# HJakeCunningham/ASVGP

Measured on AMD Instinct MI355X. Metric: Mpoints/s per ELBO+grad step, N=10M 1D Matern-3/2 M=2048, higher is better.
Workload: dtype f64

## Files before the change

### asvgp_amd/_lib.py

```python
import ctypes
import os

import torch

HERE = os.path.dirname(os.path.abspath(__file__))
LIB_PATH = os.path.join(HERE, "libasvgp_hip.so")

_c = ctypes
_P, _I, _L, _D, _Z = _c.c_void_p, _c.c_int, _c.c_int64, _c.c_double, _c.c_size_t

SIGNATURES = {
    "asvgp_version": (_I, []),
    "asvgp_last_error_string": (_c.c_char_p, []),
    "asvgp_status_name": (_c.c_char_p, [_I]),
    "asvgp_phi_workspace_bytes": (_Z, [_L, _I, _L]),
    "asvgp_create": (_I, [_c.POINTER(_P)]),
    "asvgp_destroy": (_I, [_P]),
    "asvgp_phi_accumulate_1d": (_I, [_P, _P, _P, _L, _L, _P, _L, _D, _I, _L, _P, _P, _Z, _P]),
    "asvgp_phi_weighted_workspace_bytes": (_Z, [_L, _I, _L]),
    "asvgp_phi_accumulate_1d_weighted": (_I, [_P, _P, _P, _P, _L, _L, _P, _L, _D, _I, _L, _P, _P, _P, _Z, _P]),
    "asvgp_set_weight_sums": (_I, [_P, _D, _D, _D]),
    "asvgp_phi_accumulate_kron2d_weighted": (_I, [_P, _P, _P, _L, _P, _L, _D, _L, _P, _L, _D, _L, _I, _P, _P, _P]),
    "asvgp_phi_accumulate_kron2d_sorted_weighted": (_I, [_P, _P, _P, _L, _P, _P, _L, _D, _L, _P, _L, _D, _L, _I, _P, _P, _P]),
    "asvgp_set_phi_algorithm": (_I, [_P, _I]),
    "asvgp_phi_last_algorithm": (_I, [_P]),
    "asvgp_set_phi_input_order": (_I, [_P, _I]),
    "asvgp_phi_last_input_order": (_I, [_P]),
    "asvgp_stream_probe": (_I, [_P, _P, _L, _P, _P]),
    "asvgp_debug_reload_env": (_I, []),
    "asvgp_set_deferred_forward_pass": (_I, [_P, _I]),
    "asvgp_prior_publish": (_I, [_P]),
    "asvgp_host_mantissa_bits": (_I, []),
    "asvgp_prior_interior_kuu_host": (_I, [_P, _I, _L, _I, _P, _P, _c.POINTER(_L), _c.POINTER(_L), _P]),
    "asvgp_result_mirror": (_I, [_P, _I, _c.POINTER(_P)]),
    "asvgp_result_mirror_read": (_I, [_P, _c.c_uint64, _P, _D]),
    "asvgp_elbo_grad_ahead_1d": (_I, [_P, _P, _P, _I, _L, _L, _I, _L, _P, _P, _P, _Z, _P]),
    "asvgp_elbo_publish_theta": (_I, [_P, _D, _D, _D]),
    "asvgp_elbo_grad_host_1d": (_I, [_P, _P, _P, _I, _D, _D, _D, _L, _L, _I, _L, _P, _P, _P, _Z, _P, _P, _D]),
    "asvgp_result_mirror_pending": (_c.c_uint64, [_P]),
    "asvgp_set_phi_workgroups": (_I, [_P, _I]),
    "asvgp_set_phi_deferred_reduce": (_I, [_P, _I]),
    "asvgp_phi_reduce_1d": (_I, [_P, _P]),
    "asvgp_phi_launch_plan_host": (_I, [_I, _I, _I, _I, _L, _L, _L, _I, _L, _D, _I, _I, _D, _D, _I, _P]),
    "asvgp_phi_index_1d": (_I, [_P, _L, _P, _L, _D, _P, _P]),
    "asvgp_phi_evaluate_1d": (_I, [_P, _L, _P, _L, _D, _I, _I, _P, _P, _P]),
    "asvgp_matern_coeffs": (_I, [_I, _D, _D, _c.POINTER(_D), _c.POINTER(_D), _c.POINTER(_I)]),
    "asvgp_kuu_assemble": (_I, [_P, _I, _c.POINTER(_D), _c.POINTER(_D), _L, _I, _P, _P, _P]),
    "asvgp_cholesky_band": (_I, [_P, _P, _L, _I, _P, _P]),
    "asvgp_inverse_from_cholesky_band": (_I, [_P, _P, _L, _I, _P]),
    "asvgp_solve_triang_mat": (_I, [_P, _P, _P, _L, _I, _L, _I, _P]),
    "asvgp_product_band_band": (_I, [_P, _P, _P, _L, _I, _I, _I, _I, _I, _I, _P]),
    "asvgp_transpose_band": (_I, [_P, _P, _L, _I, _I, _P]),
    "asvgp_symmetrise_band": (_I, [_P, _P, _L, _I, _P]),
    "asvgp_unpack_banded_matrix_to_dense": (_I, [_P, _P, _L, _I, _I, _P]),
    "asvgp_pack_dense_matrix_to_banded": (_I, [_P, _P, _L, _I, _I, _P]),
    "asvgp_band_trace_sym": (_I, [_P, _P, _L, _I, _P, _P]),
    "asvgp_cholesky_band_vjp": (_I, [_P, _P, _P, _P, _L, _I, _P]),
    "asvgp_inverse_from_cholesky_band_vjp": (_I, [_P, _P, _P, _P, _P, _L, _I, _P]),
    "asvgp_band_outer_product": (_I, [_P, _P, _L, _L, _I, _D, _P, _P]),
    "asvgp_band_launch_plan_host": (_I, [_I, _L, _I, _I, _I, _P]),
    "asvgp_elbo_workspace_bytes": (_Z, [_L, _I, _L]),
    "asvgp_set_band_algorithm": (_I, [_P, _I]),
    "asvgp_prior_plan_1d": (_I, [_P, _P, _I, _L, _I, _c.POINTER(_I)]),
    "asvgp_prior_table_doubles": (_Z, [_P, _I, _L, _I]),
    "asvgp_prior_forward_host": (_I, [_P, _I, _L, _I, _P, _P, _P, _Z, _P]),
    "asvgp_set_prior_forward": (_I, [_P, _I]),
    "asvgp_prior_forward_device": (_I, [_P, _P, _P, _P, _Z, _P]),
    "asvgp_prior_forward_stamps": (_I, [_P, _P, _P, _P, _P]),
    "asvgp_prior_plan_image_host": (_I, [_P, _I, _L, _I, _P, _P, _P, _P]),
    "asvgp_elbo_launch_plan_host": (_I, [_I, _I, _I, _I, _L, _I, _L, _I, _I, _I, _I, _I, _I, _I, _I, _I, _P]),
    "asvgp_elbo_grad_1d": (_I, [_P, _P, _P, _I, _D, _D, _D, _L, _L, _I, _L, _P, _P, _P, _Z, _P]),
    "asvgp_kuu_inverse_band_1d": (_I, [_P, _P, _I, _D, _D, _L, _I, _P, _P, _P, _P, _P, _P, _P, _Z, _P]),
    "asvgp_elbo_chain_sync": (_I, [_P, _I]),
    "asvgp_elbo_prior_chain_1d": (_I, [_P, _P, _I, _D, _D, _D, _L, _I, _L, _P, _P, _Z, _P]),
    "asvgp_elbo_data_chain_1d": (_I, [_P, _P, _P, _I, _D, _D, _D, _L, _L, _I, _L, _P, _P, _P, _Z, _P]),
    "asvgp_posterior_prepare_1d": (_I, [_P, _P, _P, _I, _D, _D, _D, _L, _I, _L, _P, _P, _P, _P, _Z, _P]),
    "asvgp_posterior_prepare_loo_1d": (_I, [_P, _P, _P, _I, _D, _D, _D, _L, _I, _L, _P, _P, _P, _P, _P, _Z, _P]),
    "asvgp_loo_workspace_bytes": (_Z, [_L, _I, _L]),
    "asvgp_loo_1d": (_I, [_P, _P, _P, _P, _L, _L, _P, _L, _D, _I, _L, _P, _P, _P, _D, _D, _P, _P, _P, _P, _P, _Z, _P]),
    "asvgp_score_workspace_bytes": (_Z, [_L, _I, _L]),
    "asvgp_score_1d": (_I, [_P, _P, _P, _P, _L, _L, _P, _L, _D, _I, _L, _P, _P, _D, _D, _P, _P, _P, _P, _P, _Z, _P]),
    "asvgp_weight_grad_workspace_bytes": (_Z, [_L, _I, _L, _L]),
    "asvgp_weight_grad_1d": (_I, [_P, _P, _P, _P, _L, _L, _P, _L, _D, _I, _L, _P, _P, _P, _D, _D, _P, _L, _P, _P, _P, _Z, _P]),
    "asvgp_predict_1d": (_I, [_P, _L, _P, _L, _D, _I, _L, _P, _P, _D, _L, _P, _P, _P]),
    "asvgp_predict_1d_h": (_I, [_P, _P, _L, _P, _L, _D, _I, _L, _P, _P, _D, _L, _P, _P, _P]),
    "asvgp_posterior_cov_workspace_bytes": (_Z, [_L, _I, _L]),
    "asvgp_posterior_cov_prepare_1d": (_I, [_P, _P, _P, _I, _D, _D, _D, _L, _I, _L, _P, _P, _P, _P, _P, _Z, _P]),
    "asvgp_predict_cov_1d": (_I, [_P, _P, _L, _P, _L, _P, _L, _D, _I, _L, _P, _I, _D, _D, _P, _L, _P]),
    "asvgp_predict_deriv_1d": (_I, [_P, _P, _L, _P, _L, _D, _I, _L, _P, _P, _I, _D, _D, _L, _P, _P, _P]),
    "asvgp_predict_cov_deriv_1d": (_I, [_P, _P, _L, _P, _L, _P, _L, _D, _I, _L, _P, _I, _D, _D, _I, _I, _P, _L, _P]),
    "asvgp_predict_grad_kron2d": (_I, [_P, _L, _P, _L, _D, _L, _P, _L, _D, _L, _I, _P, _P, _P, _P, _P, _L, _I, _L, _L, _L, _L,
                                       _I, _D, _D, _I, _D, _D, _P, _P, _P]),
    "asvgp_kron_dense_inverse": (_I, [_P, _P, _P, _L, _L, _I, _L, _L, _L, _L, _P, _P]),
    "asvgp_predict_cov_kron2d": (_I, [_P, _P, _L, _P, _L, _P, _L, _D, _L, _P, _L, _D, _L, _I, _P, _P, _P, _I, _D, _D, _I, _D, _D, _P, _L, _P]),
    "asvgp_predict_cov_additive": (_I, [_P, _P, _L, _P, _L, _I, _P, _c.POINTER(_L), _c.POINTER(_D), _c.POINTER(_L), _I,
                                         _c.POINTER(_I), _c.POINTER(_D), _c.POINTER(_D), _P, _P, _L, _P]),
    "asvgp_predict_components_additive": (_I, [_P, _P, _L, _I, _P, _c.POINTER(_L), _c.POINTER(_D), _c.POINTER(_L), _I, _c.POINTER(_I),
                                                _c.POINTER(_D), _c.POINTER(_D), _I, _P, _P, _P, _P, _P]),
    "asvgp_profile_enable": (_I, [_P, _I]),
    "asvgp_profile_read": (_I, [_P, _c.POINTER(_D), _c.POINTER(_L)]),
    "asvgp_kron_stats_doubles": (_Z, [_L, _L, _I]),
    "asvgp_phi_accumulate_kron2d": (_I, [_P, _P, _L, _P, _L, _D, _L, _P, _L, _D, _L, _I, _P, _P]),
    "asvgp_kron_evaluate_2d": (_I, [_P, _L, _P, _L, _D, _P, _L, _D, _L, _I, _P, _P, _P]),
    "asvgp_kron_assemble": (_I, [_P, _P, _P, _P, _P, _I, _L, _L, _D, _P, _P, _P]),
    "asvgp_blockband_cholesky": (_I, [_P, _L, _L, _P, _P, _P, _P]),
    "asvgp_blockband_backsolve": (_I, [_P, _L, _L, _P, _P]),
    "asvgp_predict_kron2d": (_I, [_P, _L, _P, _L, _D, _L, _P, _L, _D, _L, _I, _P, _P, _P, _P, _P, _P]),
    "asvgp_kron_cell_index": (_I, [_P, _L, _P, _L, _D, _P, _L, _D, _P, _P]),
    "asvgp_phi_accumulate_kron2d_sorted": (_I, [_P, _P, _L, _P, _P, _L, _D, _L, _P, _L, _D, _L, _I, _P, _P]),
    "asvgp_phi_accumulate_kron2d_sorted_f32": (_I, [_P, _P, _L, _P, _P, _L, _D, _L, _P, _L, _D, _L, _I, _P, _P]),
    "asvgp_kron_phi_launch_plan_host": (_I, [_I, _I, _I, _L, _L, _L, _L, _L, _I, _I, _L, _I, _P]),
    "asvgp_blockband_to_blocks": (_I, [_P, _L, _L, _L, _P, _P, _P]),
    "asvgp_kron_grad_terms": (_I, [_P, _P, _L, _P, _P, _P, _P, _P, _P, _P, _P, _P, _P, _I, _L, _L, _P, _P]),
    "asvgp_predict_kron2d_var": (_I, [_P, _L, _P, _L, _D, _P, _L, _D, _L, _I, _P, _P, _L, _P, _P]),
    "asvgp_kron_assemble_twisted": (_I, [_P, _P, _P, _P, _P, _I, _L, _L, _D, _L, _L, _L, _L, _L, _P, _P, _P, _P]),
    "asvgp_kron_grad_terms_twisted": (_I, [_P, _P, _L, _L, _L, _L, _L, _P, _P, _P, _P, _P, _P, _P, _P, _P, _P, _I, _L, _L, _P, _P]),
    "asvgp_predict_kron2d_var_twisted": (_I, [_P, _L, _P, _L, _D, _P, _L, _D, _L, _L, _I, _P, _P, _L, _L, _L, _L, _L, _P, _P]),
    "asvgp_phi_cross_workspace_bytes": (_Z, [_L, _L]),
    "asvgp_phi_cross_2d": (_I, [_P, _P, _L, _P, _L, _D, _L, _P, _L, _D, _L, _I, _P, _P, _Z, _P]),
}


class AsvgpError(RuntimeError):
    pass


_lib = None


def get_lib():
    global _lib
    if _lib is not None:
        return _lib
    if not os.path.exists(LIB_PATH):
        raise AsvgpError("HIP extension %s is missing: run `python -m asvgp_amd.build` (hipcc, gfx950). "
                         "asvgp_amd has no CPU fallback." % LIB_PATH)
    lib = ctypes.CDLL(LIB_PATH)
    for name, (res, args) in SIGNATURES.items():
        fn = getattr(lib, name, None)
        if fn is None:
            raise AsvgpError("libasvgp_hip.so does not export %s" % name)
        fn.restype = res
        fn.argtypes = args
    _lib = lib
    return lib


def check(status, what=""):
    if status != 0:
        lib = get_lib()
        raise AsvgpError("%s failed: %s (%s)" % (what or "asvgp call", lib.asvgp_status_name(status).decode(),
                                                  lib.asvgp_last_error_string().decode()))


class Handle:
    _defaults = {"band": 0, "phi": 0, "prior_forward": 0, "phi_order": 0}
    _live = None

    def __init__(self):
        import weakref
        lib = get_lib()
        h = _P()
        check(lib.asvgp_create(ctypes.byref(h)), "asvgp_create")
        self.ptr = h
        self._lib = lib
        self.band_algorithm = 0
        if Handle._live is None:
            Handle._live = weakref.WeakSet()
        Handle._live.add(self)
        if Handle._defaults["band"]:
            self.set_band_algorithm(Handle._defaults["band"])
        if Handle._defaults["phi"]:
            self.set_phi_algorithm(Handle._defaults["phi"])
        if Handle._defaults["prior_forward"]:
            self.set_prior_forward(Handle._defaults["prior_forward"])
        if Handle._defaults["phi_order"]:
            self.set_phi_input_order(Handle._defaults["phi_order"])

    def set_prior_forward(self, mode):
        check(self._lib.asvgp_set_prior_forward(self.ptr, int(mode)), "set_prior_forward")

    def prior_forward_device(self, coef, dcoef, n_doubles):
        import numpy as np
        coef = np.ascontiguousarray(coef, dtype=np.float64)
        dcoef = np.ascontiguousarray(dcoef, dtype=np.float64)
        tab = np.zeros(int(n_doubles), dtype=np.float64)
        check(self._lib.asvgp_prior_forward_device(self.ptr, coef.ctypes.data, dcoef.ctypes.data, tab.ctypes.data, tab.size, stream_ptr()),
              "prior_forward_device")
        return tab

    def set_band_algorithm(self, algo):
        check(self._lib.asvgp_set_band_algorithm(self.ptr, int(algo)), "set_band_algorithm")
        self.band_algorithm = int(algo)

    def set_phi_algorithm(self, algo):
        check(self._lib.asvgp_set_phi_algorithm(self.ptr, int(algo)), "set_phi_algorithm")

    def set_weight_sums(self, n_pos, sum_w, sum_log_w):
        if n_pos is None:
            n_pos, sum_w, sum_log_w = -1.0, 0.0, 0.0
        check(self._lib.asvgp_set_weight_sums(self.ptr, float(n_pos), float(sum_w), float(sum_log_w)), "set_weight_sums")

    def phi_last_algorithm(self):
        return int(self._lib.asvgp_phi_last_algorithm(self.ptr))

    def set_phi_input_order(self, order):
        check(self._lib.asvgp_set_phi_input_order(self.ptr, int(order)), "set_phi_input_order")

    def phi_last_input_order(self):
        return int(self._lib.asvgp_phi_last_input_order(self.ptr))

    def result_mirror(self, enable=True):
        import numpy as np
        ptr = _P()
        check(self._lib.asvgp_result_mirror(self.ptr, int(bool(enable)), ctypes.byref(ptr)), "result_mirror")
        if not enable or not ptr.value:
            self._mirror = None
            return None
        self._mirror = np.ctypeslib.as_array(ctypes.cast(ptr, ctypes.POINTER(_D)), shape=(16,))
        return self._mirror

    def set_deferred_forward_pass(self, on):
        check(self._lib.asvgp_set_deferred_forward_pass(self.ptr, int(on)), "set_deferred_forward_pass")
# ... 84 lines not shown
```

### asvgp_amd/csrc/bcr_mfma.hpp

```cpp
#pragma once
#include "bcr.hpp"
#include "prior_plan.hpp"

namespace asvgp {

constexpr int BM_THREADS = 1024;
constexpr int BM_B = 4;
constexpr int BM_GAT = 0, BM_GBT = 16, BM_DINV = 32, BM_SD = 48, BM_CAT = 64, BM_CBT = 80, BM_W = 96, BM_DG = 100, BM_REC = 104;

__host__ __device__ inline size_t bcr_mfma_ws_doubles(long nb) { return (size_t)nb * BM_REC + 64; }
__host__ __device__ inline size_t bcr_mfma_lds_doubles(long nb) {
  return (size_t)((nb + 1) / 2 + 1) * 32 + (size_t)nb * 4 + 96 + (size_t)(BM_THREADS / 64) * 4 * 40 + (size_t)(nb / 8 + 2) * 52;
}

__device__ __forceinline__ double bm_mfma(double a, double b, double c) { return __builtin_amdgcn_mfma_f64_4x4x4f64(a, b, c, 0, 0, 0); }

__device__ __forceinline__ double bm_chol_linv(const double (&d)[10], int hi, int lo, double& dprod, int& badj) {
  double l00, i0, l10, l20, l30, l11, i1, l21, l31, l22, i2, l32, l33, i3;
  Num<double>::sqrt_inv(d[0], l00, i0);
  badj = !(d[0] > 0.0) ? 1 : 0;
  l10 = d[1] * i0; l20 = d[3] * i0; l30 = d[6] * i0;
  double s = fma(-l10, l10, d[2]);
  badj = (!(s > 0.0) && !badj) ? 2 : badj;
  Num<double>::sqrt_inv(s, l11, i1);
  l21 = fma(-l20, l10, d[4]) * i1;
  l31 = fma(-l30, l10, d[7]) * i1;
  s = fma(-l21, l21, fma(-l20, l20, d[5]));
  badj = (!(s > 0.0) && !badj) ? 3 : badj;
  Num<double>::sqrt_inv(s, l22, i2);
  l32 = fma(-l31, l21, fma(-l30, l20, d[8])) * i2;
  s = fma(-l32, l32, fma(-l31, l31, fma(-l30, l30, d[9])));
  badj = (!(s > 0.0) && !badj) ? 4 : badj;
  Num<double>::sqrt_inv(s, l33, i3);
  dprod = (l00 * l11) * (l22 * l33);
  const double z0 = (lo == 0) ? i0 : 0.0;
  const double z1 = fma(-l10, z0, (lo == 1) ? 1.0 : 0.0) * i1;
  const double z2 = fma(-l21, z1, fma(-l20, z0, (lo == 2) ? 1.0 : 0.0)) * i2;
  const double z3 = fma(-l32, z2, fma(-l31, z1, fma(-l30, z0, (lo == 3) ? 1.0 : 0.0))) * i3;
  return hi == 0 ? z0 : (hi == 1 ? z1 : (hi == 2 ? z2 : z3));
}

template <typename Src> __device__ __forceinline__ auto bm_src_load(const Src& A, int dd, long col, long M, int) -> decltype(A.load_dc(dd, col, M)) {
  return A.load_dc(dd, col, M);
}
template <typename Src> __device__ __forceinline__ double bm_src_load(const Src& A, int dd, long col, long M, long) {
  return A.load((long)dd * M + col, true);
}
struct BmLog {
  double m; int e;
  __device__ __forceinline__ void mul(double p) {
    m *= p;
    const int hi = __double2hiint(m);
    e += ((hi >> 20) & 0x7ff) - 1023;
    m = __hiloint2double((hi & 0x800fffff) | 0x3ff00000, __double2loint(m));
  }
};

__device__ __forceinline__ unsigned long long bm_wave_xor(unsigned long long x) {
#pragma unroll
  for (int off = 32; off > 0; off >>= 1) x ^= (unsigned long long)__shfl_xor((long long)x, off, 64);
  return x;
}
__device__ __forceinline__ void bm_msg_send(double* box, int n, double v, unsigned long long tag, int lane) {
  unsigned long long* b = reinterpret_cast<unsigned long long*>(box);
  const unsigned long long w = lane < n ? (unsigned long long)__double_as_longlong(v) : 0ull;
  const unsigned long long x = bm_wave_xor(w) ^ tag;
  if (lane < n) __hip_atomic_store(b + lane, w, __ATOMIC_RELAXED, __HIP_MEMORY_SCOPE_AGENT);
  if (lane == n) __hip_atomic_store(b + n, x, __ATOMIC_RELAXED, __HIP_MEMORY_SCOPE_AGENT);
}
__device__ __forceinline__ bool bm_msg_recv(const double* box, int n, double& v, unsigned long long tag, int lane, long spin_limit) {
  const unsigned long long* b = reinterpret_cast<const unsigned long long*>(box);
  for (long spins = 0; spins <= spin_limit; ++spins) {
    const unsigned long long w = lane <= n ? __hip_atomic_load(b + lane, __ATOMIC_RELAXED, __HIP_MEMORY_SCOPE_AGENT) : 0ull;
    const unsigned long long x = bm_wave_xor(lane < n ? w : 0ull) ^ tag;
    const unsigned long long chk = (unsigned long long)__shfl((long long)w, n, 64);
    if (x == chk) { v = __longlong_as_double((long long)w); return true; }
    __builtin_amdgcn_s_sleep(1);
  }
  return false;
}

struct BmSplit {
  int half = -1;
  double* xchg = nullptr;
  long spin_limit = 0;
  int* gave_up = nullptr;
  unsigned long long tag = 0;
};
constexpr int BM_XCHG = 96;

template <typename Src>
__device__ __attribute__((always_inline)) void bcr_mfma_solve(Src A, const double* rhs, int M, double* ws, double* lds, double* Sband, double* x,
                                                              double* logdet, int* info, int rhs_stride = 1, double* stamps = nullptr,
                                                              BmSplit sp = BmSplit{}) {
  constexpr int B = BM_B;
  const int tid = threadIdx.x;
  const int lane = tid & 63, wv = __builtin_amdgcn_readfirstlane(tid >> 6);
  const int r = lane >> 4, q = (lane >> 2) & 3, c = lane & 3;
  const int e = r * 4 + c, et = c * 4 + r;
  const int hi = r > c ? r : c, lo = r > c ? c : r;
  const int nb = (M + B - 1) / B;
  const int nslot = (nb + 1) / 2;
  double* Dl = lds;
  double* El = lds + (size_t)(nslot + 1) * 16;
  double* xs = El + (size_t)(nslot + 1) * 16;
  double* red = xs + (size_t)nb * B;
  double* slab = red + 96 + (size_t)(wv * 4 + q) * 40;
  double* Fl = red + 96 + (size_t)(BM_THREADS / 64) * 4 * 40;
  double* Sl = lds;
  int levels = 0;
  while ((1 << levels) < nb) ++levels;
  const bool split = sp.half >= 0;
  const int top = levels - 1, ht = 1 << (top > 0 ? top : 0);
  double s_other = 0.0;
  int bad_other = 0x7fffffff;
  auto level_share = [&](int l, int ne, int& m0, int& ne_h) {
    m0 = 0; ne_h = ne;
    if (!split) return;
    if (l < top) {
      const int mL = ht >> (l + 1);
      if (sp.half == 0) ne_h = ne < mL ? ne : mL;
      else { m0 = mL; ne_h = ne > mL ? ne - mL : 0; }
    } else {
      ne_h = sp.half == 0 ? ne : 0;
    }
  };
  int bad = 0;
  BmLog ld{1.0, 0};
  unsigned long long t_prev = stamps ? __builtin_amdgcn_s_memtime() : 0ull;
  int nst = 0;
  auto stamp = [&]() {
    if (stamps && tid == 0) { const unsigned long long t = __builtin_amdgcn_s_memtime(); stamps[nst++] = (double)(t - t_prev); t_prev = t; }
  };
  auto rec = [&](int node) -> double* { return ws + (size_t)node * BM_REC; };
  auto bandD = [&](int n, int rr, int cc) -> double {
    const int col = n * B + cc, row = n * B + rr;
    const bool pad = row >= M;
    const double v = bm_src_load(A, rr - cc, pad ? 0 : col, (long)M, 0);
    return pad ? ((rr == cc) ? 1.0 : 0.0) : v;
  };
  auto bandE = [&](int n, int rr, int cc) -> double {
    if (rr > cc) return 0.0;
    const int col = n * B + cc, row = (n + 1) * B + rr;
    const bool pad = row >= M;
    const double v = bm_src_load(A, B + rr - cc, pad ? 0 : col, (long)M, 0);
    return pad ? 0.0 : v;
  };
  if ((nb & 1) && tid < 16 && !(split && sp.half == 0)) {
    const int rr = tid >> 2, cc = tid & 3;
    Dl[(size_t)((nb - 1) >> 1) * 16 + tid] = bandD(nb - 1, rr > cc ? rr : cc, rr > cc ? cc : rr);
  }
  if (split && sp.half == 0 && tid < 16) Dl[(size_t)(ht >> 1) * 16 + tid] = 0.0;
  for (int row = tid; row < nb * B; row += BM_THREADS) {
    const bool sep_left = split && sp.half == 0 && row >= ht * B && row < (ht + 1) * B;
    xs[row] = (row < M && !sep_left) ? rhs[(long)row * rhs_stride] : 0.0;
  }
  __syncthreads();
  stamp();

  constexpr int RMAXR = 4;
  for (int l = 0; l < levels; ++l) {
    const int h = 1 << l;
    const int ne = (nb > h) ? (nb - h + 2 * h - 1) / (2 * h) : 0;
    int m0, ne_h;
    level_share(l, ne, m0, ne_h);
    if (split && l == top) {
      if (sp.half == 1) {
        if (wv == 0) {
          const double v = lane < 16 ? Dl[(size_t)(ht >> 1) * 16 + lane] : (lane < 20 ? xs[ht * B + lane - 16] : 0.0);
          bm_msg_send(sp.xchg, 20, v, sp.tag | 1ull, lane);
        }
        const double mine = (r == 0 && c == 0) ? (log(ld.m) + (double)ld.e * 0.6931471805599453094) : 0.0;
        const double tot = wave_sum_dpp(mine);
        int bm = bad ? bad : 0x7fffffff;
#pragma unroll
        for (int off = 32; off > 0; off >>= 1) { const int o = __shfl_xor(bm, off, 64); bm = o < bm ? o : bm; }
        int* sbad = reinterpret_cast<int*>(red + 32);
        if (lane == 0) { red[wv] = tot; sbad[wv] = bm; }
        __syncthreads();
        if (wv == 0) {
          double sv = 0.0;
          int bmin = 0x7fffffff;
          for (int w2 = 0; w2 < BM_THREADS / 64; ++w2) { sv += red[w2]; bmin = sbad[w2] < bmin ? sbad[w2] : bmin; }
          bm_msg_send(sp.xchg + 24, 2, lane == 0 ? sv : (double)bmin, sp.tag | 2ull, lane);
        }
      } else {
        if (wv == 0) {
          double v = 0.0;
          if (!bm_msg_recv(sp.xchg, 20, v, sp.tag | 1ull, lane, sp.spin_limit)) { if (lane == 0) *sp.gave_up = 1; }
          else {
            if (lane < 16) Dl[(size_t)(ht >> 1) * 16 + lane] += v;
            else if (lane < 20) xs[ht * B + lane - 16] += v;
          }
        }
        __syncthreads();
        if (*sp.gave_up) return;
      }
      stamp();
    }
    double updb[RMAXR], ybu[RMAXR];
    int qv = q, ev = e;
    asm volatile("" : "+v"(qv), "+v"(ev));
    double sl[2][3];
    auto slab_loads = [&](int rd0) __attribute__((always_inline)) {
#pragma unroll
      for (int u = 0; u < 2; ++u) {
#pragma unroll
        for (int t3 = 0; t3 < 3; ++t3) {
          sl[u][t3] = 0.0;
          int m = (rd0 + u) * 64 + wv * 4 + qv;
          m = m0 + (m < ne_h ? m : ne_h - 1);
          const int kk = ev + 16 * t3, dd = kk >> 3, col = m * 2 * B + (kk & 7);
          const bool in = kk < 40 && col + dd < M;
          const double v = bm_src_load(A, in ? dd : 0, in ? col : 0, (long)M, 0);
          sl[u][t3] = in ? v : ((dd == 0) ? 1.0 : 0.0);
        }
      }
    };
#pragma unroll
    for (int rd = 0; rd < RMAXR; ++rd) {
      __builtin_amdgcn_sched_barrier(0);
      if (l == 0 && (rd & 1) == 0) slab_loads(rd);
      updb[rd] = 0.0; ybu[rd] = 0.0;
      if (rd * 64 + wv * 4 >= ne_h) continue;
      const int ml = rd * 64 + wv * 4 + q;
      const bool act = ml < ne_h;
      const int i = h + (m0 + (act ? ml : ne_h - 1)) * 2 * h, a = i - h, b = i + h;
      const bool hasb = b < nb;
      const int bsafe = hasb ? b : a;
      double d[10];
      double ea, eb, da;
      if (l == 0) {
#pragma unroll
        for (int t3 = 0; t3 < 3; ++t3) if (e + 16 * t3 < 40) slab[e + 16 * t3] = sl[rd & 1][t3];
        int kk = 0;
#pragma unroll
        for (int rr = 0; rr < 4; ++rr)
#pragma unroll
          for (int cc = 0; cc <= rr; ++cc) d[kk++] = slab[(rr - cc) * 8 + 4 + cc];
        ea = slab[(4 + lo - hi) * 8 + hi];
        ea = (r <= c) ? ea : 0.0;
        eb = slab[(4 + lo - hi) * 8 + 4 + hi];
        eb = (hasb && c <= r) ? eb : 0.0;
        da = slab[(hi - lo) * 8 + lo];
      } else {
        const double* Di = Dl + (size_t)(i >> 1) * 16;
        int kk = 0;
#pragma unroll
        for (int rr = 0; rr < 4; ++rr)
#pragma unroll
          for (int cc = 0; cc <= rr; ++cc) d[kk++] = Di[rr * 4 + cc];
        ea = El[(size_t)(a >> 1) * 16 + e];
        eb = El[(size_t)(i >> 1) * 16 + et];
        eb = hasb ? eb : 0.0;
        da = Dl[(size_t)(a >> 1) * 16 + e];
      }
      double yv = xs[i * B + r], ya = xs[a * B + r];
      yv = (c == 0) ? yv : 0.0;
      ya = (c == 0) ? ya : 0.0;
      (void)bsafe;
      double dprod;
      int badj;
      const double t = bm_chol_linv(d, hi, lo, dprod, badj);
      if (act && badj && !bad) bad = i * B + badj;
      const double linv = (r >= c) ? t : 0.0;
      const double linvT = (c >= r) ? t : 0.0;
      if (act) ld.mul(dprod);
      const double ua = bm_mfma(linvT, ea, 0.0);
      const double ub = bm_mfma(linvT, eb, 0.0);
      const double zz = bm_mfma(linvT, yv, 0.0);
      const double nua = -ua, nub = -ub;
      const double da_new = bm_mfma(nua, ua, da);
      const double e_new = bm_mfma(nub, ua, 0.0);
      const double ya_new = bm_mfma(nua, zz, ya);
      updb[rd] = bm_mfma(ub, ub, 0.0);
      ybu[rd] = bm_mfma(ub, zz, 0.0);
      updb[rd] = act ? updb[rd] : 0.0;
      ybu[rd] = act ? ybu[rd] : 0.0;
      const double gat = bm_mfma(ua, linv, 0.0);
      const double gbt = bm_mfma(ub, linv, 0.0);
      const double dinv = bm_mfma(linv, linv, 0.0);
      const double w = bm_mfma(linv, zz, 0.0);
      if (act) {
        if (l >= 3) {
          double* R = Fl + (size_t)(i >> 3) * 52;
          R[e] = gat; R[16 + e] = gbt; R[32 + e] = dinv;
          if (c == 0) R[48 + r] = w;
        } else {
          double* R = rec(i);
          R[BM_GAT + e] = gat; R[BM_GBT + e] = gbt; R[BM_DINV + e] = dinv;
          if (c == 0) R[BM_W + r] = w;
        }
        Dl[(size_t)(a >> 1) * 16 + e] = da_new;
        El[(size_t)(a >> 1) * 16 + e] = e_new;
        if (c == 0) xs[a * B + r] = ya_new;
      }
    }
    bcr_lds_barrier();
#pragma unroll
    for (int rd = 0; rd < RMAXR; ++rd) {
      if (rd * 64 + wv * 4 >= ne_h) continue;
      const int ml = rd * 64 + wv * 4 + q;
      const int i = h + (m0 + ml) * 2 * h, b = i + h;
      if (ml < ne_h && b < nb) {
        Dl[(size_t)(b >> 1) * 16 + e] -= updb[rd];
        if (c == 0) xs[b * B + r] -= ybu[rd];
      }
    }
    bcr_lds_barrier();
    stamp();
  }
  if (wv == 0 && !(split && sp.half == 1)) {
    const bool act = q == 0;
    double d[10];
    int kk = 0;
#pragma unroll
    for (int rr = 0; rr < 4; ++rr)
#pragma unroll
      for (int cc = 0; cc <= rr; ++cc) { const double v = Dl[rr * 4 + cc]; d[kk++] = act ? v : ((rr == cc) ? 1.0 : 0.0); }
    const double yv = (act && c == 0) ? xs[r] : 0.0;
    double dprod;
    int badj;
    const double t = bm_chol_linv(d, hi, lo, dprod, badj);
    if (act && badj && !bad) bad = badj;
    const double linv = (r >= c) ? t : 0.0, linvT = (c >= r) ? t : 0.0;
    if (act) ld.mul(dprod);
    const double s00 = bm_mfma(linv, linv, 0.0);
    const double zz = bm_mfma(linvT, yv, 0.0);
    const double x0 = bm_mfma(linv, zz, 0.0);
    if (act) {
      rec(0)[BM_SD + e] = s00;
      Sl[e] = s00;
      if (r >= c && r < M) Sband[(long)(r - c) * M + c] = s00;
      if (c == 0) xs[r] = x0;
    }
  }
  __syncthreads();
  stamp();
  unsigned long long lw = 0ull;
  for (int l = levels - 1; l >= 0; --l) {
    const int h = 1 << l;
    const int ne = (nb > h) ? (nb - h + 2 * h - 1) / (2 * h) : 0;
    int m0, ne_h;
    level_share(l, ne, m0, ne_h);
    if (split && sp.half == 0 && wv == BM_THREADS / 64 - 1) {
      if (l == top - 1 && lane <= 2)
        lw = __hip_atomic_load(reinterpret_cast<const unsigned long long*>(sp.xchg + 24) + lane, __ATOMIC_RELAXED, __HIP_MEMORY_SCOPE_AGENT);
      if (l == 2) {
        const unsigned long long x = bm_wave_xor(lane < 2 ? lw : 0ull) ^ (sp.tag | 2ull);
        const unsigned long long chk = (unsigned long long)__shfl((long long)lw, 2, 64);
        double v = __longlong_as_double((long long)lw);
        bool ok = x == chk;
        if (!ok) ok = bm_msg_recv(sp.xchg + 24, 2, v, sp.tag | 2ull, lane, sp.spin_limit);
        if (!ok) { if (lane == 0) *sp.gave_up = 1; }
        else if (lane < 2) red[48 + lane] = v;
      }
    }
#pragma unroll
    for (int rd = 0; rd < RMAXR; ++rd) {
      __builtin_amdgcn_sched_barrier(0);
      if (rd * 64 + wv * 4 >= ne_h) continue;
      const int ml = rd * 64 + wv * 4 + q;
      const bool act = ml < ne_h;
      const int i = h + (m0 + (act ? ml : ne_h - 1)) * 2 * h, a = i - h, b = i + h;
      const bool hasb = b < nb;
      const int bs = hasb ? b : a;
      const bool e_is_a = ((a / (2 * h)) & 1) != 0;
      double gat, gbt, dinv, w, saa, sbb, sba, sab;
      if (l >= 3) {
        const double* R = Fl + (size_t)(i >> 3) * 52;
        gat = R[e]; gbt = R[16 + e]; dinv = R[32 + e]; w = R[48 + r];
      } else {
        const double* R = rec(i);
        gat = R[BM_GAT + e]; gbt = R[BM_GBT + e]; dinv = R[BM_DINV + e]; w = R[BM_W + r];
      }
      if (l >= 1) {
        const double* Ra = Sl + (size_t)(a >> 2) * 48;
        const double* Rb = Sl + (size_t)(bs >> 2) * 48;
        saa = Ra[e];
        sbb = Rb[e];
        sba = e_is_a ? Ra[32 + e] : Rb[16 + et];
        sab = e_is_a ? Ra[32 + et] : Rb[16 + e];
      } else {
        const double* Ra = rec(a);
        const double* Rb = rec(bs);
        saa = Ra[BM_SD + e];
        sbb = Rb[BM_SD + e];
        sba = e_is_a ? Ra[BM_CBT + e] : Rb[BM_CAT + et];
        sab = e_is_a ? Ra[BM_CBT + et] : Rb[BM_CAT + e];
      }
      sbb = hasb ? sbb : 0.0; sba = hasb ? sba : 0.0; sab = hasb ? sab : 0.0;
      double xa = xs[a * B + r], xb = xs[bs * B + r];
      xa = (c == 0) ? xa : 0.0;
      xb = (hasb && c == 0) ? xb : 0.0;
      w = (c == 0) ? w : 0.0;
      double ncat = bm_mfma(saa, gat, 0.0);
      ncat = bm_mfma(sba, gbt, ncat);
      double ncbt = bm_mfma(sab, gat, 0.0);
      ncbt = bm_mfma(sbb, gbt, ncbt);
      double sii = bm_mfma(ncat, gat, dinv);
      sii = bm_mfma(ncbt, gbt, sii);
      double gx = bm_mfma(gat, xa, 0.0);
      gx = bm_mfma(gbt, xb, gx);
      if (act) {
        if (c == 0) xs[i * B + r] = w - gx;
        if (l >= 2) {
          double* Rw = Sl + (size_t)(i >> 2) * 48;
          Rw[e] = sii; Rw[16 + e] = -ncat; Rw[32 + e] = -ncbt;
        }
        if (l > 0) {
          double* Rw = rec(i);
          Rw[BM_SD + e] = sii; Rw[BM_CAT + e] = -ncat; Rw[BM_CBT + e] = -ncbt;
        }
        if (r >= c && i * B + r < M) Sband[(long)(r - c) * M + i * B + c] = sii;
        if (l == 0) {
          if (c <= r && i * B + c < M) Sband[(long)(B + c - r) * M + a * B + r] = -ncat;
          if (hasb && r <= c && b * B + r < M) Sband[(long)(B + r - c) * M + i * B + c] = -ncbt;
        }
      }
    }
    if (l == 1) __syncthreads(); else bcr_lds_barrier();
    if (split && l == top) {
      double* Rs = Sl + (size_t)(ht >> 2) * 48;
      if (sp.half == 0) {
        if (wv == 0) bm_msg_send(sp.xchg + 32, 52, lane < 48 ? Rs[lane < 48 ? lane : 0] : (lane < 52 ? xs[ht * B + lane - 48] : 0.0), sp.tag | 3ull, lane);
      } else {
        if (wv == 0) {
          double v = 0.0;
          if (!bm_msg_recv(sp.xchg + 32, 52, v, sp.tag | 3ull, lane, sp.spin_limit)) { if (lane == 0) *sp.gave_up = 1; }
          else if (lane < 48) {
            Rs[lane] = v;
            rec(ht)[BM_SD + lane] = v;
            if (lane < 16) {
              const int rr = lane >> 2, cc = lane & 3;
              if (rr >= cc && ht * B + rr < M) Sband[(long)(rr - cc) * M + ht * B + cc] = v;
            }
          } else if (lane < 52) {
            xs[ht * B + lane - 48] = v;
          }
        }
        __syncthreads();
        if (*sp.gave_up) return;
      }
    }
    stamp();
  }
  if (!(split && sp.half == 0))
    for (int col = M - B + tid; col < M; col += BM_THREADS)
      if (col >= 0)
#pragma unroll
        for (int dd = 1; dd <= B; ++dd)
          if (col + dd >= M) Sband[(long)dd * M + col] = 0.0;
  {
    const int row0 = (split && sp.half == 1) ? (ht + 1) * B : 0, row1 = (split && sp.half == 0) ? (ht + 1) * B : M;
    for (int row = row0 + tid; row < row1 && row < M; row += BM_THREADS) x[(long)row * rhs_stride] = xs[row];
  }
  if (!(split && sp.half == 1)) {
    const double mine = (r == 0 && c == 0) ? (log(ld.m) + (double)ld.e * 0.6931471805599453094) : 0.0;
    const double tot = wave_sum_dpp(mine);
    int bm = bad ? bad : 0x7fffffff;
#pragma unroll
    for (int off = 32; off > 0; off >>= 1) { const int o = __shfl_xor(bm, off, 64); bm = o < bm ? o : bm; }
    int* sbad = reinterpret_cast<int*>(red + 32);
    if (lane == 0) { red[wv] = tot; sbad[wv] = bm; }
    __syncthreads();
    if (split && tid == 0) { s_other = red[48]; bad_other = (int)red[49]; }
    if (tid == 0) {
      double s = 0.0;
      int bmin = 0x7fffffff;
      for (int w2 = 0; w2 < BM_THREADS / 64; ++w2) { s += red[w2]; bmin = sbad[w2] < bmin ? sbad[w2] : bmin; }
      s += s_other;
      bmin = bad_other < bmin ? bad_other : bmin;
      __hip_atomic_store(logdet + 0, 2.0 * s, __ATOMIC_RELAXED, __HIP_MEMORY_SCOPE_AGENT);
      __hip_atomic_store(logdet + 1, 0.0, __ATOMIC_RELAXED, __HIP_MEMORY_SCOPE_AGENT);
      __hip_atomic_store(info, (bmin == 0x7fffffff) ? 0 : bmin, __ATOMIC_RELAXED, __HIP_MEMORY_SCOPE_AGENT);
    }
  }
  stamp();
}


__host__ __device__ inline size_t bcr_mfma_pre_ws_doubles(long nb) { return (size_t)nb * 96 + 64; }
__host__ __device__ inline size_t bcr_mfma_pre_lds_doubles(long nb, int n_rec) {
  return PRIOR_TAB_HEADER + (size_t)2 * n_rec * prior_rec_fields(BM_B) + (size_t)(nb / 4 + 2) * 96 + (size_t)(nb + 1) / 2 + 64;
}

struct BmDual { double v, d; };
__device__ __forceinline__ BmDual bm_dmfma(BmDual x, BmDual y, BmDual c) {
  BmDual r;
  r.v = bm_mfma(x.v, y.v, c.v);
  r.d = bm_mfma(x.d, y.v, c.d);
  r.d = bm_mfma(x.v, y.d, r.d);
  return r;
}

__device__ __attribute__((always_inline)) void bcr_mfma_backward_pre(const double* __restrict__ tab, int n_rec, const int* __restrict__ node_rec, int M,
                                                                      double* ws, double* lds, double* Sv, double* Sd, double* logdet, int* info,
                                                                      unsigned long long* done_flag, unsigned long long seq,
                                                                      const unsigned long long* ready_flag = nullptr, long spin_limit = 0, int* gave_up = nullptr) {
  constexpr int B = BM_B, W = prior_rec_fields(B);
  const int tid = threadIdx.x;
  if (ready_flag) {
    if (tid == 0) {
      long spins = 0;
      while (__hip_atomic_load(ready_flag, __ATOMIC_RELAXED, __HIP_MEMORY_SCOPE_SYSTEM) < seq) {
        __builtin_amdgcn_s_sleep(8);
        if (++spins > spin_limit) { *gave_up = 1; break; }
      }
    }
    __syncthreads();
    if (*gave_up) return;
    __builtin_amdgcn_fence(__ATOMIC_ACQUIRE, "");
  }
  const int lane = tid & 63, wv = __builtin_amdgcn_readfirstlane(tid >> 6);
  const int r = lane >> 4, q = (lane >> 2) & 3, c = lane & 3;
  const int e = r * 4 + c, et = c * 4 + r;
  const int nb = (M + B - 1) / B;
  const int n_tab = PRIOR_TAB_HEADER + 2 * n_rec * W;
  double* tl = lds;
  double* Sl = lds + n_tab;
  int* nrl = reinterpret_cast<int*>(Sl + (size_t)(nb / 4 + 2) * 96);
  {
    const double2* src = reinterpret_cast<const double2*>(tab);
    double2* dst = reinterpret_cast<double2*>(tl);
    for (int i2 = tid; i2 < n_tab / 2; i2 += BM_THREADS) dst[i2] = src[i2];
    for (int i2 = tid; i2 < nb; i2 += BM_THREADS) nrl[i2] = node_rec[i2];
  }
  __syncthreads();
  if (done_flag && tid == 0) __hip_atomic_store(done_flag, seq, __ATOMIC_RELAXED, __HIP_MEMORY_SCOPE_SYSTEM);
  const double* tv = tl + PRIOR_TAB_HEADER;
  const double* td = tv + (size_t)n_rec * W;
  int levels = 0;
  while ((1 << levels) < nb) ++levels;
  if (tid < 16) {
    const int r0 = nrl[0];
    const double xv = tv[(size_t)r0 * W + prior_f_UA(B) + tid], xd = td[(size_t)r0 * W + prior_f_UA(B) + tid];
    Sl[tid] = xv; Sl[48 + tid] = xd;
    ws[tid] = xv; ws[48 + tid] = xd;
    const int rr = tid >> 2, cc = tid & 3;
    if (rr >= cc && rr < M) { Sv[(long)(rr - cc) * M + cc] = xv; Sd[(long)(rr - cc) * M + cc] = xd; }
  }
  __syncthreads();
  constexpr int RMAXR = 4;
  for (int l = levels - 1; l >= 0; --l) {
    const int h = 1 << l;
    const int ne = (nb > h) ? (nb - h + 2 * h - 1) / (2 * h) : 0;
#pragma unroll
    for (int rd = 0; rd < RMAXR; ++rd) {
      __builtin_amdgcn_sched_barrier(0);
      if (rd * 64 + wv * 4 >= ne) continue;
      const int m = rd * 64 + wv * 4 + q;
      const bool act = m < ne;
      const int i = h + (act ? m : ne - 1) * 2 * h, a = i - h, b = i + h;
      const bool hasb = b < nb;
      const int bs = hasb ? b : a;
      const bool e_is_a = ((a / (2 * h)) & 1) != 0;
      const int ri = nrl[i];
      const double* fv = tv + (size_t)ri * W;
      const double* fd = td + (size_t)ri * W;
      const BmDual gat{fv[prior_f_GAT(B) + e], fd[prior_f_GAT(B) + e]};
      const BmDual gbt{fv[prior_f_GBT(B) + e], fd[prior_f_GBT(B) + e]};
      const BmDual dinv{fv[prior_f_DINV(B) + e], fd[prior_f_DINV(B) + e]};
      BmDual saa, sbb, sba, sab;
      if (l >= 1) {
        const double* Ra = Sl + (size_t)(a >> 2) * 96;
        const double* Rb = Sl + (size_t)(bs >> 2) * 96;
        saa = BmDual{Ra[e], Ra[48 + e]};
        sbb = BmDual{Rb[e], Rb[48 + e]};
        sba = e_is_a ? BmDual{Ra[32 + e], Ra[80 + e]} : BmDual{Rb[16 + et], Rb[64 + et]};
        sab = e_is_a ? BmDual{Ra[32 + et], Ra[80 + et]} : BmDual{Rb[16 + e], Rb[64 + e]};
      } else {
        const double* Ga = ws + (size_t)a * 96;
        const double* Gb = ws + (size_t)bs * 96;
        saa = BmDual{Ga[e], Ga[48 + e]};
        sbb = BmDual{Gb[e], Gb[48 + e]};
        sba = e_is_a ? BmDual{Ga[32 + e], Ga[80 + e]} : BmDual{Gb[16 + et], Gb[64 + et]};
        sab = e_is_a ? BmDual{Ga[32 + et], Ga[80 + et]} : BmDual{Gb[16 + e], Gb[64 + e]};
      }
      if (!hasb) { sbb = BmDual{0.0, 0.0}; sba = sbb; sab = sbb; }
      const BmDual zero{0.0, 0.0};
      BmDual ncat = bm_dmfma(saa, gat, zero);
      ncat = bm_dmfma(sba, gbt, ncat);
      BmDual ncbt = bm_dmfma(sab, gat, zero);
      ncbt = bm_dmfma(sbb, gbt, ncbt);
      BmDual sii = bm_dmfma(ncat, gat, dinv);
      sii = bm_dmfma(ncbt, gbt, sii);
      if (act) {
        if (l >= 2) {
          double* Rw = Sl + (size_t)(i >> 2) * 96;
          Rw[e] = sii.v; Rw[16 + e] = -ncat.v; Rw[32 + e] = -ncbt.v;
          Rw[48 + e] = sii.d; Rw[64 + e] = -ncat.d; Rw[80 + e] = -ncbt.d;
        }
        if (l > 0) {
          double* Rw = ws + (size_t)i * 96;
          Rw[e] = sii.v; Rw[16 + e] = -ncat.v; Rw[32 + e] = -ncbt.v;
          Rw[48 + e] = sii.d; Rw[64 + e] = -ncat.d; Rw[80 + e] = -ncbt.d;
        }
        if (r >= c && i * B + r < M) { const long o = (long)(r - c) * M + i * B + c; Sv[o] = sii.v; Sd[o] = sii.d; }
        if (l == 0) {
          if (c <= r && i * B + c < M) { const long o = (long)(B + c - r) * M + a * B + r; Sv[o] = -ncat.v; Sd[o] = -ncat.d; }
          if (hasb && r <= c && b * B + r < M) { const long o = (long)(B + r - c) * M + i * B + c; Sv[o] = -ncbt.v; Sd[o] = -ncbt.d; }
        }
      }
    }
    if (l == 1) __syncthreads(); else bcr_lds_barrier();
  }
  for (int col = M - B + tid; col < M; col += BM_THREADS)
    if (col >= 0)
#pragma unroll
      for (int dd = 1; dd <= B; ++dd)
        if (col + dd >= M) { Sv[(long)dd * M + col] = 0.0; Sd[(long)dd * M + col] = 0.0; }
  if (tid == 0) {
    __hip_atomic_store(logdet + 0, tl[0], __ATOMIC_RELAXED, __HIP_MEMORY_SCOPE_AGENT);
    __hip_atomic_store(logdet + 1, tl[1], __ATOMIC_RELAXED, __HIP_MEMORY_SCOPE_AGENT);
    __hip_atomic_store(info, (int)tl[2], __ATOMIC_RELAXED, __HIP_MEMORY_SCOPE_AGENT);
  }
}

}
```

### asvgp_amd/csrc/elbo.hip

```cpp
#include <stdio.h>
#include <stdlib.h>
#include <time.h>
#include <string.h>

#include <type_traits>

#include "bcr_pre.hpp"
#include "bcr_mfma.hpp"
#include "handle.hpp"

namespace asvgp {


struct Ws {
  double *Kuu, *dK, *P, *LK, *dLK, *LP, *SK, *dSK, *SP, *c, *alpha, *logdets, *fin, *bcrK, *bcrP;
};
static size_t bcr_ws_chain(int planes, int k, bool big) {
  long ns = 1024;
  while ((long)planes * 2 * k * k * ns * 8 + 2 * ns * k * 8 + 1024 > 150 * 1024) ns >>= 1;
  if (big) ns *= 2;
  return (size_t)planes * (7 * k * k + k) * 2 * ns + (big ? (size_t)planes * k * k * ns : 0);
}
static size_t bcr_ws_K(int k, long M) {
  size_t a = bcr_ws_chain(2, k, false), b = bcr_ws_chain(2, k, true), c = bcr_pre_ws_doubles(k, (M + k - 1) / k);
  a = a > b ? a : b;
  return (a > c ? a : c) + 64;
}
static size_t bcr_ws_P(int k) { size_t a = bcr_ws_chain(1, k, false), b = bcr_ws_chain(1, k, true); return (a > b ? a : b) + 64; }
static size_t bcr_ws_total(long M, int k) { return bcr_ws_K(k, M) + bcr_ws_P(k); }
static size_t ws_doubles(long M, int k, long D) {
  return (size_t)9 * (k + 1) * M + (size_t)2 * M * D + 64 + 32 + bcr_ws_total(M, k);
}
static Ws carve(void* ws, long M, int k, long D) {
  double* p = static_cast<double*>(ws);
  size_t E = (size_t)(k + 1) * M;
  Ws w;
  w.Kuu = p; p += E; w.dK = p; p += E; w.P = p; p += E; w.LK = p; p += E; w.dLK = p; p += E;
  w.LP = p; p += E; w.SK = p; p += E; w.dSK = p; p += E; w.SP = p; p += E;
  w.c = p; p += (size_t)M * D; w.alpha = p; p += (size_t)M * D;
  w.logdets = p; p += 64;
  w.fin = p; p += 32;
  w.bcrK = p; p += bcr_ws_K(k, M);
  w.bcrP = p;
  return w;
}

template <int K> struct ElboLauncher {
  static int run(Handle* h, const double* stats, const double* S, int kind, double v, double l, double s, long N, long M, long D,
                 double* out, int* info, void* ws, hipStream_t st, int part);
};
template <int K> struct KuuInvLauncher {
  static int run(Handle* h, const double* S, int kind, double v, double l, long M, double* Kuu, double* dK, double* SK, double* dSK,
                 double* logdet2, int* info, void* ws, hipStream_t st);
};
template <int K> struct PostLauncher {
  static int run(Handle* h, const double* stats, const double* S, int kind, double v, double l, double s, long M, long D,
                 double* alpha, double* W, int* info, void* ws, hipStream_t st, double* Pinv = nullptr);
};
static size_t cov_ws_doubles(long M, int k) { return (size_t)4 * (k + 1) * M + (size_t)2 * M + 8; }
template <int K> struct PostCovLauncher {
  static int run(Handle* h, const double* stats, const double* S, int kind, double v, double l, double s, long M, long D,
                 double* alpha, double* W, double* Wd, int* info, void* ws, hipStream_t st);
};

constexpr int FIN_LDS_DOUBLES = 16 * 14 + 2;
constexpr size_t LDS_BYTES = 160 * 1024;
enum ChainPath { PATH_SWEEPS = 0, PATH_BCR, PATH_BCR_PRIOR, PATH_BCR_DATA, PATH_PLANNED_BCR, PATH_PLANNED_MFMA };
enum ChainForward { FWD_NONE = 0, FWD_HOST_INLINE, FWD_HOST_BEFORE, FWD_DEFERRED, FWD_WORKER, FWD_GPU, FWD_AHEAD };
struct ChainPlanIn {
  int algo;
  bool have_plan; int n_rec;
  bool interior;
  long M, D;
  int part;
  bool fused_fin;
  bool ahead_req, gpu_fwd, fwd_worker, defer_forward;
  bool no_split, plan_first;
};
struct ChainPlan {
  int status; char msg[160];
  int path;
  int part;
  bool nothing;
  bool big;
  size_t lds_bytes;
  int grid, n_helpers, split;
  int fwd;
  bool scale_alpha, scale_c;
};

template <int K, bool TANGENT>
static ChainPlan plan_chains(const ChainPlanIn& in) {
  ChainPlan p{};
  auto refuse = [&p](int status, const char* fmt, size_t bytes = 0) { p.status = status; snprintf(p.msg, sizeof(p.msg), fmt, bytes); return p; };
  const int algo = in.algo;
  const long M = in.M, nb = (M + K - 1) / K;
  if ((algo == 3 || algo == 4) && !in.have_plan) return refuse(ASVGP_ERR_BAD_ARG, "band algorithms 3 and 4 need asvgp_prior_plan_1d for this (M, k, kernel)");
  const bool planned0 = in.have_plan && (algo == 0 || algo == 3 || algo == 4);
  const size_t ldsK = sizeof(double) * (TANGENT ? bcr_lds_doubles<Dual, K, 0>(nb) : bcr_lds_doubles<double, K, 0>(nb));
  const size_t ldsP = sizeof(double) * bcr_lds_doubles<double, K, 1>(nb);
  p.lds_bytes = planned0 ? ldsP : (ldsK > ldsP ? ldsK : ldsP);
  bool fits = p.lds_bytes <= LDS_BYTES - 256;
  constexpr bool HAS_BIG = (K <= 5);
  if (HAS_BIG && !fits) {
    const size_t bK = sizeof(double) * (TANGENT ? bcr_lds_doubles<Dual, K, 0, true>(nb) : bcr_lds_doubles<double, K, 0, true>(nb));
    const size_t bP = sizeof(double) * bcr_lds_doubles<double, K, 1, true>(nb);
    const size_t bb = planned0 ? bP : (bK > bP ? bK : bP);
    if (bb <= LDS_BYTES - 256) { p.big = true; fits = true; p.lds_bytes = bb; }
  }
  const bool use_bcr = (algo == 2 || algo == 3 || algo == 4 || (algo == 0 && fits));
  const bool planned = planned0 && use_bcr;
  p.part = in.part;
  if (in.part != 0 && (!use_bcr || planned)) {
    if (in.part == 1) { p.nothing = true; return p; }
    p.part = 0;
  }
  p.scale_alpha = !TANGENT;
  const char* ahead_only = "launch-ahead exists for the matrix-core launch only (k = 4, D = 1, M <= 2048, planned prior chain)";
  if (planned) {
    bool mfma = false;
    size_t lds_mfma = 0;
    if constexpr (K == BM_B) {
      const size_t lb = sizeof(double) * bcr_mfma_lds_doubles(nb), lk = sizeof(double) * bcr_mfma_pre_lds_doubles(nb, in.n_rec);
      mfma = (algo == 0 || algo == 4) && in.D == 1 && nb <= 512 && TANGENT && in.fused_fin && lb <= LDS_BYTES && lk <= LDS_BYTES && in.interior;
      lds_mfma = lb > lk ? lb : lk;
    }
    if (algo == 4 && !mfma)
      return refuse(ASVGP_ERR_UNSUPPORTED, "band algorithm 4 (matrix-core chains) needs k = 4, D = 1, M <= 2048, Toeplitz static bands and the ELBO + gradient entry point");
    if (in.ahead_req && !mfma) return refuse(ASVGP_ERR_UNSUPPORTED, ahead_only);
    if (!mfma) {
      if (!fits) return refuse(ASVGP_ERR_LDS_CAPACITY, "BCR needs %zu B of LDS", p.lds_bytes);
      p.path = PATH_PLANNED_BCR;
      const size_t lds_pre = sizeof(double) * bcr_pre_lds_doubles(K, in.n_rec);
      if (lds_pre > p.lds_bytes) p.lds_bytes = lds_pre;
      p.n_helpers = (int)((M + 255) / 256 < 6 ? (M + 255) / 256 : 6);
      p.grid = 2 + p.n_helpers;
      p.fwd = in.gpu_fwd ? FWD_GPU : FWD_HOST_BEFORE;
      return p;
    }
    if (in.ahead_req && (in.gpu_fwd || in.plan_first)) return refuse(ASVGP_ERR_UNSUPPORTED, "launch-ahead needs the host forward pass (asvgp_set_prior_forward(h, 0))");
    p.path = PATH_PLANNED_MFMA;
    p.big = false;
    p.lds_bytes = lds_mfma > sizeof(double) * FIN_LDS_DOUBLES ? lds_mfma : sizeof(double) * FIN_LDS_DOUBLES;
    p.split = (nb >= 128 && !in.no_split) ? 1 : 0;
    p.grid = 2 + p.split;
    p.fwd = in.ahead_req ? FWD_AHEAD : in.gpu_fwd ? FWD_GPU : in.plan_first ? FWD_HOST_BEFORE : in.fwd_worker ? FWD_WORKER
          : in.defer_forward ? FWD_DEFERRED : FWD_HOST_INLINE;
    return p;
  }
  if (in.ahead_req) return refuse(ASVGP_ERR_UNSUPPORTED, ahead_only);
  if (!use_bcr) {
    p.path = PATH_SWEEPS; p.big = false; p.lds_bytes = 0; p.grid = 2; p.scale_alpha = p.scale_c = true;
    return p;
  }
  if (!fits) return refuse(ASVGP_ERR_LDS_CAPACITY, "BCR forced but needs %zu B of LDS", p.lds_bytes);
  p.path = p.part == 1 ? PATH_BCR_PRIOR : (p.part == 2 ? PATH_BCR_DATA : PATH_BCR);
  p.grid = p.part == 0 ? 2 : 1;
  if (p.part == 1) p.scale_alpha = false;
  return p;
}

template <class F>
static int for_bandwidth(int k, F&& f) {
  switch (k) {
    case 1: return f(std::integral_constant<int, 1>{});
    case 2: return f(std::integral_constant<int, 2>{});
    case 3: return f(std::integral_constant<int, 3>{});
    case 4: return f(std::integral_constant<int, 4>{});
    case 5: return f(std::integral_constant<int, 5>{});
    case 6: return f(std::integral_constant<int, 6>{});
  }
  return ASVGP_ERR_UNSUPPORTED;
}

#ifdef ASVGP_ELBO_ONLY_K
struct KuuCoefs2 { double c[ASVGP_MAX_KUU_TERMS]; double dc[ASVGP_MAX_KUU_TERMS]; int n; };

constexpr int KI_DKB = 8;
struct KuuInterior { double k[8]; long lo, hi; double bnd[2 * PRIOR_BND_DIAGS * PRIOR_BND]; double dk[8]; double dkb[2 * 5 * KI_DKB]; int dk_tab; };
struct ThetaBox {
  unsigned long long seq;
  double s, alpha_scale, v, l, N, Nw, cw;
  double k[8], dk[8];
  double bnd[2 * PRIOR_BND_DIAGS * PRIOR_BND];
  double dkb[2 * 5 * KI_DKB];
  double dc[ASVGP_MAX_KUU_TERMS];
};
typedef const __attribute__((address_space(3))) double* lds_cdouble_ptr;
struct BandSumToep {
  const double* A; double inv_s;
  lds_cdouble_ptr kl;
  lds_cdouble_ptr bnd;
  long lo, hi;
  __device__ __forceinline__ double load_dc(int dd, long col, long M) const {
#pragma clang fp contract(off)
    const double t2 = A[(long)dd * M + col] * inv_s;
    const bool left = col < lo, right = col >= hi;
    const long bi = left ? (long)dd * PRIOR_BND + col : (right ? (long)(PRIOR_BND_DIAGS + dd) * PRIOR_BND + (col - hi) : 0);
    const double bv = bnd[bi];
    const double kv = kl[dd];
    return t2 + ((left || right) ? bv : kv);
  }
};

static __global__ void elbo_prepare_kernel(const double* __restrict__ S, KuuCoefs2 cf, long E, const double* __restrict__ A,
                                    double s, double* __restrict__ Kuu, double* __restrict__ dK,
                                    double* __restrict__ P) {
#pragma clang fp contract(off)
  long e = (long)blockIdx.x * blockDim.x + threadIdx.x;
  if (e >= E) return;
  double acc = cf.c[0] * S[e];
  double dacc = cf.dc[0] * S[e];
  for (int t = 1; t < cf.n; ++t) {
    double sv = S[(long)t * E + e];
    acc = acc + cf.c[t] * sv;
    dacc = dacc + cf.dc[t] * sv;
  }
  Kuu[e] = acc;
  if (dK) dK[e] = dacc;
  if (P) P[e] = A[e] / s + acc;
}

template <int K, bool TANGENT, bool RHS>
__global__ __launch_bounds__(64) void elbo_factor_kernel(const double* Kuu, const double* dK, const double* P,
                                                         double* LK, double* dLK, double* LP, const double* b,
                                                         double* c, int M, int* info) {
  if (blockIdx.x == 0) {
    if (TANGENT) cholesky_sweep<Dual, K, false>(BandPtr<Dual>{Kuu, dK}, BandOut<Dual>{LK, dLK}, M, nullptr, nullptr, info);
    else cholesky_sweep<double, K, false>(BandPtr<double>{Kuu, nullptr}, BandOut<double>{LK, nullptr}, M, nullptr, nullptr, info);
  } else {
    cholesky_sweep<double, K, RHS>(BandPtr<double>{P, nullptr}, BandOut<double>{LP, nullptr}, M, b, c, info + 1);
  }
}

template <int K, bool TANGENT, bool RHS>
__global__ __launch_bounds__(64) void elbo_inverse_kernel(const double* LK, const double* dLK, const double* LP,
                                                          double* SK, double* dSK, double* SP, const double* c,
                                                          double* alpha, int M) {
  if (blockIdx.x == 0) {
    if (TANGENT) takahashi_sweep<Dual, K, false>(BandPtr<Dual>{LK, dLK}, BandOut<Dual>{SK, dSK}, M, nullptr, nullptr);
    else takahashi_sweep<double, K, false>(BandPtr<double>{LK, nullptr}, BandOut<double>{SK, nullptr}, M, nullptr, nullptr);
  } else {
    takahashi_sweep<double, K, RHS>(BandPtr<double>{LP, nullptr}, BandOut<double>{SP, nullptr}, M, c, alpha);
  }
}

template <int K>
__global__ __launch_bounds__(64) void elbo_trsv_kernel(const double* L, int M, const double* B, double* X, long D,
                                                       int trans, double scale) {
  const long d = blockIdx.x;
  if (trans) trsv_sweep<K, true>(L, M, B + d, X + d, D);
  else trsv_sweep<K, false>(L, M, B + d, X + d, D);
  (void)scale;
}

template <int K, bool BIG>
__device__ __forceinline__ void more_columns(const double* b, double* x, int D, int M, double* wsP, double* lds, int lds_doubles) {
  if (D <= 1) return;
  __syncthreads();
  const int nb = (M + K - 1) / K;
  int chunk = lds_doubles / (nb * K);
  if (chunk < 1) chunk = 1;
  for (int d0 = 1; d0 < D; d0 += chunk) bcr_solve_more<K, BIG>(b, x, D, d0, (D - d0 < chunk) ? D - d0 : chunk, M, wsP, lds);
}

template <int K, bool TANGENT, bool BIG>
__global__ __launch_bounds__(BCR_THREADS) void elbo_bcr_kernel(const double* Kuu, const double* dK, const double* P,
                                                               const double* b, int M, double* wsK, double* wsP,
                                                               double* SK, double* dSK, double* SP, double* x,
                                                               double* logdets, int* info, int do_stamps,
                                                               int first_chain, int D, int lds_doubles) {
  extern __shared__ double lds[];
  double* st = do_stamps ? logdets + 8 : nullptr;
  for (int rep = (do_stamps == 2) ? 0 : 1; rep < 2; ++rep) {
    if (blockIdx.x + first_chain == 0) {
      if (TANGENT) bcr_solve<Dual, K, 0, BandPtr<Dual>, BIG>(BandPtr<Dual>{Kuu, dK}, nullptr, M, wsK, lds, BandOut<Dual>{SK, dSK}, nullptr, logdets, info, st);
      else bcr_solve<double, K, 0, BandPtr<double>, BIG>(BandPtr<double>{Kuu, nullptr}, nullptr, M, wsK, lds, BandOut<double>{SK, nullptr}, nullptr, logdets, info, st);
    } else {
      bcr_solve<double, K, 1, BandPtr<double>, BIG>(BandPtr<double>{P, nullptr}, b, M, wsP, lds, BandOut<double>{SP, nullptr}, x, logdets + 2, info + 1, st ? st + 24 : nullptr, D);
      more_columns<K, BIG>(b, x, D, M, wsP, lds, lds_doubles);
    }
    __syncthreads();
  }
}

template <int K, bool BIG>
__global__ __launch_bounds__(BCR_THREADS) void elbo_bcr_prior_kernel(const double* Kuu, const double* dK, int M, double* wsK,
                                                                     double* SK, double* dSK, double* logdets, int* info,
                                                                     int do_stamps) {
  extern __shared__ double lds[];
  double* st = do_stamps ? logdets + 8 : nullptr;
  bcr_solve<Dual, K, 0, BandPtr<Dual>, BIG>(BandPtr<Dual>{Kuu, dK}, nullptr, M, wsK, lds, BandOut<Dual>{SK, dSK}, nullptr, logdets, info, st);
}

template <int K, bool BIG>
__global__ __launch_bounds__(BCR_THREADS) void elbo_bcr_data_kernel(const double* Kuu, const double* A, const double* b, int M,
                                                                    double* wsP, double* SP, double* x, double* logdets,
                                                                    int* info, int do_stamps, double s, int D, int lds_doubles) {
  extern __shared__ double lds[];
  double* st = do_stamps ? logdets + 8 : nullptr;
  bcr_solve<double, K, 1, BandSumP, BIG>(BandSumP{A, Kuu, 1.0 / s}, b, M, wsP, lds, BandOut<double>{SP, nullptr}, x, logdets + 2, info + 1,
                                         st ? st + 24 : nullptr, D);
  more_columns<K, BIG>(b, x, D, M, wsP, lds, lds_doubles);
}

template <int KT>
__device__ __forceinline__ double quad_col(const double* S, long M, long j, const double* x, long D, long d) {
  double xj = x[j * D + d];
  double a = S[j] * xj * xj;
#pragma unroll
  for (int r = 1; r <= KT; ++r) {
    long jr = (j + r < M) ? j + r : M - 1;
    double sv = (j + r < M) ? S[(long)r * M + j] : 0.0;
    a = fma(2.0 * sv * xj, x[jr * D + d], a);
  }
  return a;
}

struct ElboScalars { double v, l, s, N, Nw, cw; };

template <int KT>
__device__ __forceinline__ void elbo_finalize_body(
    int bid, int nblk, double* part_lds, const double* __restrict__ stats, const double* __restrict__ Kuu, const double* __restrict__ dK,
    const double* __restrict__ LK, const double* __restrict__ LP, const double* __restrict__ SK,
    const double* __restrict__ dSK, const double* __restrict__ SP, const double* __restrict__ c,
    const double* __restrict__ alpha, const double* __restrict__ logdets, long M, long D, ElboScalars th,
    double alpha_scale, double* __restrict__ gacc, unsigned* __restrict__ ticket, unsigned* __restrict__ rearm, double* __restrict__ out) {
  constexpr int k = KT;
  const double* A = stats;
  const double* b = stats + (long)(k + 1) * M;
  const double yy = stats[(long)(k + 1) * M + M * D];
  enum { LOGK, LOGP, TRKA, DTRKA, SKDK, SPDK, SKK, SPK, SPA, CC, AKA, ADKA, AAA, BA, NACC };
  double acc[NACC];
#pragma unroll
  for (int i = 0; i < NACC; ++i) acc[i] = 0.0;
  const long chunk = (M + nblk - 1) / nblk;
  const long j_end = ((long)(bid + 1) * chunk < M) ? (long)(bid + 1) * chunk : M;
  for (long j = (long)bid * chunk + threadIdx.x; j < j_end; j += blockDim.x) {
    if (!logdets) {
      double lk = LK[j], lp = LP[j];
      acc[LOGK] += log(lk * lk);
      acc[LOGP] += log(lp * lp);
    }
#pragma unroll
    for (int r = 0; r <= k; ++r) {
      long o = (long)r * M + j;
      double w = (r == 0) ? 1.0 : 2.0;
      double sk = SK[o], sp = SP[o], a = A[o], kk = Kuu[o], dk = dK[o];
      acc[TRKA] = fma(w * sk, a, acc[TRKA]);
      acc[DTRKA] = fma(w * dSK[o], a, acc[DTRKA]);
      acc[SKDK] = fma(w * sk, dk, acc[SKDK]);
      acc[SPDK] = fma(w * sp, dk, acc[SPDK]);
      acc[SKK] = fma(w * sk, kk, acc[SKK]);
      acc[SPK] = fma(w * sp, kk, acc[SPK]);
      acc[SPA] = fma(w * sp, a, acc[SPA]);
    }
    for (long d = 0; d < D; ++d) {
      if (!logdets) {
        double cv = c[j * D + d];
        acc[CC] = fma(cv, cv, acc[CC]);
      }
      acc[AKA] += quad_col<KT>(Kuu, M, j, alpha, D, d);
      acc[ADKA] += quad_col<KT>(dK, M, j, alpha, D, d);
      acc[AAA] += quad_col<KT>(A, M, j, alpha, D, d);
      acc[BA] = fma(b[j * D + d], alpha[j * D + d], acc[BA]);
    }
  }
  double (*part)[NACC] = reinterpret_cast<double (*)[NACC]>(part_lds);
  const int lane = threadIdx.x & 63, wv = threadIdx.x >> 6, nw = blockDim.x >> 6;
#pragma unroll
  for (int i = 0; i < NACC; ++i) {
    double v = wave_sum_dpp(acc[i]);
    if (lane == 0) part[wv][i] = v;
  }
  __syncthreads();
  double tot[NACC];
  if (threadIdx.x < 64) {
#pragma unroll
    for (int i = 0; i < NACC; ++i) tot[i] = wave_sum_dpp(lane < nw ? part[lane][i] : 0.0);
  }
  int* is_last_p = reinterpret_cast<int*>(part_lds + 16 * NACC);
#define is_last (*is_last_p)
  if (threadIdx.x == 0) {
#pragma unroll
    for (int i = 0; i < NACC; ++i)
      if (tot[i] != 0.0) __hip_atomic_fetch_add(gacc + i, tot[i], __ATOMIC_RELAXED, __HIP_MEMORY_SCOPE_AGENT);
    asm volatile("s_waitcnt vmcnt(0)" ::: "memory");
    unsigned t = __hip_atomic_fetch_add(ticket, 1u, __ATOMIC_RELAXED, __HIP_MEMORY_SCOPE_AGENT);
    is_last = (t == (unsigned)nblk - 1);
  }
  __syncthreads();
  if (!is_last) return;
  if (threadIdx.x == 0) {
#pragma unroll
    for (int i = 0; i < NACC; ++i) tot[i] = __hip_atomic_load(gacc + i, __ATOMIC_RELAXED, __HIP_MEMORY_SCOPE_AGENT);
#pragma unroll
    for (int i = 0; i < NACC; ++i) __hip_atomic_store(gacc + i, 0.0, __ATOMIC_RELAXED, __HIP_MEMORY_SCOPE_AGENT);
    __hip_atomic_store(ticket, 0u, __ATOMIC_RELAXED, __HIP_MEMORY_SCOPE_AGENT);
    if (rearm) __hip_atomic_store(rearm, 0u, __ATOMIC_RELAXED, __HIP_MEMORY_SCOPE_AGENT);
    const double v = th.v, s = th.s, N = th.N, Nw = th.Nw, Dd = (double)D;
    tot[AKA] *= alpha_scale * alpha_scale; tot[ADKA] *= alpha_scale * alpha_scale; tot[AAA] *= alpha_scale * alpha_scale;
    tot[BA] *= alpha_scale;
    if (logdets) {
      tot[LOGK] = logdets[0];
      tot[LOGP] = logdets[2];
      tot[CC] = tot[BA] / s;
    }
    const double two_pi = 6.283185307179586476925286766559;
    double elbo = -0.5 * N * Dd * log(two_pi * s);
    elbo -= 0.5 * Dd * tot[LOGP];
    elbo += 0.5 * Dd * tot[LOGK];
    elbo -= 0.5 * yy / s;
    elbo += 0.5 * tot[CC];
    elbo -= 0.5 * Nw * v / s;
    elbo += 0.5 * tot[TRKA] / s;
    if (th.cw != 0.0) elbo += th.cw;
    double d_l = 0.5 * (Dd * tot[SKDK] - Dd * tot[SPDK] - tot[ADKA] + tot[DTRKA] / s);
    double d_v = 0.5 * (-Dd * tot[SKK] / v + Dd * tot[SPK] / v + tot[AKA] / v + tot[TRKA] / (v * s)) - 0.5 * Nw / s;
    double s2 = s * s;
    double d_s = -0.5 * N * Dd / s + 0.5 * Dd * tot[SPA] / s2 + 0.5 * yy / s2 + 0.5 * tot[AAA] / s2 - tot[BA] / s2 +
                 0.5 * Nw * v / s2 - 0.5 * tot[TRKA] / s2;
    out[0] = elbo; out[1] = d_v; out[2] = d_l; out[3] = d_s;
    out[4] = tot[LOGK]; out[5] = tot[LOGP]; out[6] = tot[TRKA]; out[7] = tot[CC];
  }
#undef is_last
}

template <int KT>
__global__ __launch_bounds__(256) void elbo_finalize_kernel(
    const double* __restrict__ stats, const double* __restrict__ Kuu, const double* __restrict__ dK,
    const double* __restrict__ LK, const double* __restrict__ LP, const double* __restrict__ SK,
    const double* __restrict__ dSK, const double* __restrict__ SP, const double* __restrict__ c,
    const double* __restrict__ alpha, const double* __restrict__ logdets, long M, int k_rt, long D, ElboScalars th,
    double alpha_scale, double* __restrict__ gacc, unsigned* __restrict__ ticket, double* __restrict__ out) {
  __shared__ double part[FIN_LDS_DOUBLES];
  (void)k_rt;
  elbo_finalize_body<KT>((int)blockIdx.x, (int)gridDim.x, part, stats, Kuu, dK, LK, LP, SK, dSK, SP, c, alpha, logdets, M, D, th, alpha_scale,
                         gacc, ticket, nullptr, out);
}

struct FusedFin {
  const double* stats; ElboScalars th; double alpha_scale; double* gacc; unsigned* ticket; unsigned* arrived; unsigned* assembled; double* out;
  long D; int n_helpers; int finalize; int debug_no_assembly; int debug_stamps;
  double* mirror; unsigned long long mirror_seq;
  int split; double* xchg;
};
constexpr int FIN_GACC_PR = 21;
__device__ __forceinline__ void assemble_band_slice(const double* __restrict__ S, const double* __restrict__ coef, const double* __restrict__ dcoef, int n_terms,
                                                    long E, long e, double* __restrict__ Kuu, double* __restrict__ dK) {
#pragma clang fp contract(off)
  double sv[ASVGP_MAX_KUU_TERMS];
#pragma unroll
  for (int t = 0; t < ASVGP_MAX_KUU_TERMS; ++t) sv[t] = (t < n_terms) ? S[(long)t * E + e] : 0.0;
  double acc = coef[0] * sv[0], dacc = dcoef[0] * sv[0];
#pragma unroll
  for (int t = 1; t < ASVGP_MAX_KUU_TERMS; ++t)
    if (t < n_terms) { acc = acc + coef[t] * sv[t]; dacc = dacc + dcoef[t] * sv[t]; }
  Kuu[e] = acc;
  if (dK) dK[e] = dacc;
}
template <int K, bool BIG>
__global__ __launch_bounds__(BCR_THREADS) void elbo_chains_kernel(const double* S_static, KuuCoefs2 cf, double* Kuu, double* dK, const double* A, const double* b, int M,
                                                                  double* wsP, double* SP, double* x, double* logdets, int* info,
                                                                  double s, const double* tab, int n_rec, const int* node_rec,
                                                                  double* wsK, double* SK, double* dSK,
                                                                  unsigned long long* done_flag, unsigned long long seq, int D, int lds_doubles, FusedFin fin) {
  extern __shared__ double lds[];
  const long E = (long)(K + 1) * M;
  __shared__ int gave_up;
  if (threadIdx.x == 0) gave_up = 0;
  __syncthreads();
  if (blockIdx.x == 0) {
    if (threadIdx.x == 0) {
      long spins = 0;
      while (__hip_atomic_load(fin.assembled, __ATOMIC_RELAXED, __HIP_MEMORY_SCOPE_AGENT) < (unsigned)fin.n_helpers) {
        __builtin_amdgcn_s_sleep(2);
        if (++spins > (1L << 25)) { gave_up = 1; break; }
      }
      if (!gave_up) __hip_atomic_store(fin.assembled, 0u, __ATOMIC_RELAXED, __HIP_MEMORY_SCOPE_AGENT);
    }
    __syncthreads();
    if (gave_up) { if (threadIdx.x == 0) atomicExch(info + 1, -1); return; }
    __builtin_amdgcn_fence(__ATOMIC_ACQUIRE, "agent");
    bcr_solve<double, K, 1, BandSumP, BIG>(BandSumP{A, Kuu, 1.0 / s}, b, M, wsP, lds, BandOut<double>{SP, nullptr}, x, logdets + 2, info + 1, nullptr, D);
    more_columns<K, BIG>(b, x, D, M, wsP, lds, lds_doubles);
  } else if (blockIdx.x == 1) {
    bcr_backward_pre<K>(tab, n_rec, node_rec, M, wsK, lds, BandOut<Dual>{SK, dSK}, logdets, info, done_flag, seq);
  } else {
    for (long e = (long)(blockIdx.x - 2) * blockDim.x + threadIdx.x; e < E; e += (long)fin.n_helpers * blockDim.x)
      assemble_band_slice(S_static, cf.c, cf.dc, cf.n, E, e, Kuu, dK);
    __syncthreads();
    if (threadIdx.x == 0) {
      __threadfence();
      __hip_atomic_fetch_add(fin.assembled, 1u, __ATOMIC_RELEASE, __HIP_MEMORY_SCOPE_AGENT);
    }
  }
  if (!fin.finalize) return;
  if (blockIdx.x < 2) {
    __syncthreads();
    if (threadIdx.x == 0) {
      __threadfence();
      __hip_atomic_fetch_add(fin.arrived, 1u, __ATOMIC_RELEASE, __HIP_MEMORY_SCOPE_AGENT);
    }
    return;
  }
  if (threadIdx.x == 0) {
    long spins = 0;
    while (__hip_atomic_load(fin.arrived, __ATOMIC_RELAXED, __HIP_MEMORY_SCOPE_AGENT) < 2u) {
      __builtin_amdgcn_s_sleep(8);
      if (++spins > (1L << 25)) { gave_up = 1; break; }
    }
  }
  __syncthreads();
  if (gave_up) { if (threadIdx.x == 0) atomicExch(info + 1, -1); return; }
  __builtin_amdgcn_fence(__ATOMIC_ACQUIRE, "agent");
  elbo_finalize_body<K>((int)blockIdx.x - 2, fin.n_helpers, lds, fin.stats, Kuu, dK, nullptr, nullptr, SK, dSK, SP, nullptr, x, logdets, (long)M, fin.D,
                        fin.th, fin.alpha_scale, fin.gacc, fin.ticket, fin.arrived, fin.out);
}

template <int K>
__global__ __launch_bounds__(BM_THREADS) void elbo_chains_mfma_kernel(KuuInterior ki, const double* S_static, KuuCoefs2 cf, double* Kuu, double* dK, const double* A, const double* b, int M,
                                                                      double* wsP, double* SP, double* x, double* logdets, int* info,
                                                                      double s, const double* tab, int n_rec, const int* node_rec,
                                                                      double* wsK, double* SK, double* dSK,
                                                                      unsigned long long* done_flag, unsigned long long seq,
                                                                      const unsigned long long* ready_flag, long spin_limit, FusedFin fin, const ThetaBox* box) {
  extern __shared__ double lds[];
  static_assert(K == BM_B, "matrix-core chains: bandwidth 4");
  const long E = (long)(K + 1) * M;
  const unsigned long long t_start = fin.debug_stamps ? __builtin_amdgcn_s_memrealtime() : 0ull;
  auto rstamp = [&](int slot) {
    if (fin.debug_stamps && threadIdx.x == 0 && blockIdx.x <= 2)
      logdets[(slot < 4 ? 8 + 4 * (int)blockIdx.x : 24) + slot] = (slot == 0) ? (double)(t_start & 0xffffffffull) : (double)((__builtin_amdgcn_s_memrealtime() - t_start) & 0xffffffffull);
  };
  rstamp(0);
  __shared__ int gave_up, kuu_ok;
  __shared__ double kuu_pref[4];
  if (threadIdx.x == 0) { gave_up = 0; kuu_ok = 0; }
  __syncthreads();
  double s_v = s, asc_v = fin.alpha_scale;
  ElboScalars th_v = fin.th;
  if (box) {
    if (threadIdx.x == 0) {
      long spins = 0;
      for (;;) {
        const unsigned long long got = __hip_atomic_load(&box->seq, __ATOMIC_RELAXED, __HIP_MEMORY_SCOPE_SYSTEM);
        if (got == seq) break;
        if (got == ~0ull || ++spins > spin_limit) { gave_up = 1; break; }
        __builtin_amdgcn_s_sleep(2);
      }
    }
    __syncthreads();
    if (gave_up) { if (threadIdx.x == 0) atomicExch(info + 1, -1); return; }
    s_v = box->s; asc_v = box->alpha_scale;
    th_v.v = box->v; th_v.l = box->l; th_v.s = box->s; th_v.N = box->N; th_v.Nw = box->Nw; th_v.cw = box->cw;
  }
  const double* stats = fin.stats;
  enum { LOGK, LOGP, TRKA, DTRKA, SKDK, SPDK, SKK, SPK, SPA, CC, AKA, ADKA, AAA, BA, NACC };
  double acc[NACC];
#pragma unroll
  for (int i = 0; i < NACC; ++i) acc[i] = 0.0;
  const bool isP = blockIdx.x == 0 || (fin.split && blockIdx.x == 2);
  const bool isPR = fin.split && blockIdx.x == 2;
  __shared__ double kdl[16];
  __shared__ double bnd[2 * PRIOR_BND_DIAGS * PRIOR_BND], dkb[2 * 5 * KI_DKB];
  {
    if (isP) rstamp(1);
    if (threadIdx.x == 0) {
      if (box) {
#pragma unroll
        for (int i = 0; i < 5; ++i) { kdl[i] = box->k[i]; kdl[8 + i] = box->dk[i]; }
      } else {
        kdl[0] = ki.k[0]; kdl[1] = ki.k[1]; kdl[2] = ki.k[2]; kdl[3] = ki.k[3]; kdl[4] = ki.k[4];
        kdl[8] = ki.dk[0]; kdl[9] = ki.dk[1]; kdl[10] = ki.dk[2]; kdl[11] = ki.dk[3]; kdl[12] = ki.dk[4];
      }
    }
    {
      const double* bnd_g = box ? box->bnd : reinterpret_cast<const double*>((const char*)__builtin_amdgcn_kernarg_segment_ptr() + offsetof(KuuInterior, bnd));
      const double* dkb_g = box ? box->dkb : reinterpret_cast<const double*>((const char*)__builtin_amdgcn_kernarg_segment_ptr() + offsetof(KuuInterior, dkb));
      if (threadIdx.x < 2 * PRIOR_BND_DIAGS * PRIOR_BND) bnd[threadIdx.x] = bnd_g[threadIdx.x];
      else if (threadIdx.x < 2 * PRIOR_BND_DIAGS * PRIOR_BND + 2 * 5 * KI_DKB) dkb[threadIdx.x - 2 * PRIOR_BND_DIAGS * PRIOR_BND] = dkb_g[threadIdx.x - 2 * PRIOR_BND_DIAGS * PRIOR_BND];
    }
    __syncthreads();
  }
  if (isP) {
    BmSplit bsp;
    if (fin.split) { bsp.half = isPR ? 1 : 0; bsp.xchg = fin.xchg; bsp.spin_limit = spin_limit; bsp.gave_up = &gave_up; bsp.tag = seq << 8; }
    bcr_mfma_solve<BandSumToep>(BandSumToep{A, 1.0 / s_v, (lds_cdouble_ptr)kdl, (lds_cdouble_ptr)bnd, ki.lo, ki.hi}, b, M, wsP, lds, SP, x, logdets + 2, info + 1, 1,
                                fin.debug_stamps ? (isPR ? fin.xchg + 128 : logdets + 32) : (double*)nullptr, bsp);
    rstamp(3);
    __syncthreads();
    if (gave_up) { if (threadIdx.x == 0) atomicExch(info + 1, -1); return; }
    rstamp(4);
    if (fin.finalize) {
      const double* xs_l = lds + (size_t)2 * ((((M + K - 1) / K) + 1) / 2 + 1) * 16;
      static_assert(BM_THREADS == 1024, "two columns per thread");
      int nbl = (M + K - 1) / K, lv = 0;
      while ((1 << lv) < nbl) ++lv;
      const long jsep = (long)(1 << (lv > 0 ? lv - 1 : 0)) * K;
      const long j0 = isPR ? jsep : 0, j1 = (fin.split && !isPR) ? jsep : (long)M;
      unsigned long long kw = 0ull;
      const bool kuu_reader = !isPR && (threadIdx.x >> 6) == 1;
      if (kuu_reader && (threadIdx.x & 63) <= 4)
        kw = __hip_atomic_load(reinterpret_cast<const unsigned long long*>(fin.gacc + 8) + (threadIdx.x & 63), __ATOMIC_RELAXED, __HIP_MEMORY_SCOPE_AGENT);
      double sp[2][K + 1], av[2][K + 1], bj[2];
#pragma unroll
      for (int cI = 0; cI < 2; ++cI) {
        const long j = j0 + threadIdx.x + cI * BM_THREADS, jc = j < j1 ? j : j1 - 1;
#pragma unroll
        for (int r = 0; r <= K; ++r) { sp[cI][r] = SP[(long)r * M + jc]; av[cI][r] = stats[(long)r * M + jc]; }
        bj[cI] = stats[(long)(K + 1) * M + jc];
      }
#pragma unroll
      for (int cI = 0; cI < 2; ++cI) {
        const long j = j0 + threadIdx.x + cI * BM_THREADS;
        if (j >= j1) continue;
        const bool left = j < ki.lo, right = j >= ki.hi;
        const double xj = xs_l[j];
#pragma unroll
        for (int r = 0; r <= K; ++r) {
          const long o = (long)r * M + j;
          const double w2 = (r == 0) ? 1.0 : 2.0;
          double kv = kdl[r], dkv = kdl[8 + r];
          if (left || right) {
            kv = bnd[left ? (long)r * PRIOR_BND + j : (long)(PRIOR_BND_DIAGS + r) * PRIOR_BND + (j - ki.hi)];
            if (ki.dk_tab) {
              dkv = dkb[left ? (long)r * KI_DKB + j : (long)(5 + r) * KI_DKB + (j - ki.hi)];
            } else {
              dkv = 0.0;
              for (int t = 0; t < cf.n; ++t) dkv = fma(box ? box->dc[t] : cf.dc[t], S_static[(long)t * E + o], dkv);
            }
          }
          const double xx = (j + r < M) ? w2 * xj * xs_l[j + r] : 0.0;
          acc[SPDK] = fma(w2 * sp[cI][r], dkv, acc[SPDK]);
          acc[SPK] = fma(w2 * sp[cI][r], kv, acc[SPK]);
          acc[SPA] = fma(w2 * sp[cI][r], av[cI][r], acc[SPA]);
          acc[AKA] = fma(kv, xx, acc[AKA]);
          acc[ADKA] = fma(dkv, xx, acc[ADKA]);
          acc[AAA] = fma(av[cI][r], xx, acc[AAA]);
        }
        acc[BA] = fma(bj[cI], xj, acc[BA]);
      }
      if (kuu_reader) {
        const int ln = threadIdx.x & 63;
        const unsigned long long x = bm_wave_xor(ln < 4 ? kw : 0ull) ^ ((seq << 8) | 4ull);
        const unsigned long long chk = (unsigned long long)__shfl((long long)kw, 4, 64);
        if (x == chk) { if (ln < 4) kuu_pref[ln] = __longlong_as_double((long long)kw); if (ln == 0) kuu_ok = 1; }
      }
    }
  } else {
    if (fin.debug_no_assembly) {
      if (threadIdx.x == 0) { for (long sp_ = 0; sp_ < spin_limit; ++sp_) __builtin_amdgcn_s_sleep(8); atomicExch(info + 1, -1); }
      return;
    }
    bcr_mfma_backward_pre(tab, n_rec, node_rec, M, wsK, lds, SK, dSK, logdets, info, done_flag, seq, ready_flag,
                          spin_limit < (1L << 20) ? spin_limit : (1L << 20), &gave_up);
    if (gave_up) { if (threadIdx.x == 0) atomicExch(info + 1, -1); return; }
    rstamp(1);
    if (fin.finalize) {
      __syncthreads();
      double sk[2][K + 1], dsk[2][K + 1], av[2][K + 1];
#pragma unroll
      for (int cI = 0; cI < 2; ++cI) {
        const long j = (long)threadIdx.x + cI * BM_THREADS, jc = j < M ? j : M - 1;
#pragma unroll
        for (int r = 0; r <= K; ++r) { sk[cI][r] = SK[(long)r * M + jc]; dsk[cI][r] = dSK[(long)r * M + jc]; av[cI][r] = stats[(long)r * M + jc]; }
      }
#pragma unroll
      for (int cI = 0; cI < 2; ++cI) {
        const long j = (long)threadIdx.x + cI * BM_THREADS;
        if (j >= M) continue;
        const bool left = j < ki.lo, right = j >= ki.hi;
#pragma unroll
        for (int r = 0; r <= K; ++r) {
          const long o = (long)r * M + j;
          const double w2 = (r == 0) ? 1.0 : 2.0;
          double kv = kdl[r], dkv = kdl[8 + r];
          if (left || right) {
            kv = bnd[left ? (long)r * PRIOR_BND + j : (long)(PRIOR_BND_DIAGS + r) * PRIOR_BND + (j - ki.hi)];
            if (ki.dk_tab) {
              dkv = dkb[left ? (long)r * KI_DKB + j : (long)(5 + r) * KI_DKB + (j - ki.hi)];
            } else {
              dkv = 0.0;
              for (int t = 0; t < cf.n; ++t) dkv = fma(box ? box->dc[t] : cf.dc[t], S_static[(long)t * E + o], dkv);
            }
          }
          acc[TRKA] = fma(w2 * sk[cI][r], av[cI][r], acc[TRKA]);
          acc[DTRKA] = fma(w2 * dsk[cI][r], av[cI][r], acc[DTRKA]);
          acc[SKDK] = fma(w2 * sk[cI][r], dkv, acc[SKDK]);
          acc[SKK] = fma(w2 * sk[cI][r], kv, acc[SKK]);
        }
      }
    }
  }
  if (!fin.finalize) { rstamp(2); return; }
  if (isP) rstamp(5);
  double* part0 = lds;
  const int lane = threadIdx.x & 63;
  double mine[8];
  mine[0] = isP ? acc[SPDK] : acc[TRKA];
  mine[1] = isP ? acc[SPK] : acc[DTRKA];
  mine[2] = isP ? acc[SPA] : acc[SKDK];
  mine[3] = isP ? acc[AKA] : acc[SKK];
  mine[4] = acc[ADKA]; mine[5] = acc[AAA]; mine[6] = acc[BA]; mine[7] = 0.0;
  const int nmine = isP ? 7 : 4;
  __syncthreads();
  const bool b0 = (lane & 1) != 0, b1 = (lane & 2) != 0, b2 = (lane & 4) != 0;
  double s4[4], s2[2];
#pragma unroll
  for (int i = 0; i < 4; ++i) { const double keep = b0 ? mine[4 + i] : mine[i], send = b0 ? mine[i] : mine[4 + i]; s4[i] = keep + dpp_move_f64<0xB1>(send); }
#pragma unroll
  for (int i = 0; i < 2; ++i) { const double keep = b1 ? s4[2 + i] : s4[i], send = b1 ? s4[i] : s4[2 + i]; s2[i] = keep + dpp_move_f64<0x4E>(send); }
  double s1 = (b2 ? s2[1] : s2[0]) + dpp_xor4_f64(b2 ? s2[0] : s2[1], b2);
  s1 += dpp_move_f64<0x128>(s1); s1 += __shfl_xor(s1, 16, 64); s1 += __shfl_xor(s1, 32, 64);
  const int wv = threadIdx.x >> 6;
  if (lane < 8) part0[wv * 8 + lane] = s1;
  __syncthreads();
  if (threadIdx.x >= 64) return;
  double t2 = part0[(2 * (lane >> 3)) * 8 + (lane & 7)] + part0[(2 * (lane >> 3) + 1) * 8 + (lane & 7)];
  t2 += __shfl_xor(t2, 8, 64); t2 += __shfl_xor(t2, 16, 64); t2 += __shfl_xor(t2, 32, 64);
  double red[7];
  red[0] = __shfl(t2, 0, 64); red[1] = __shfl(t2, 4, 64); red[2] = __shfl(t2, 2, 64); red[3] = __shfl(t2, 6, 64);
  red[4] = __shfl(t2, 1, 64); red[5] = __shfl(t2, 5, 64); red[6] = __shfl(t2, 3, 64);
  (void)nmine;
  double tot[NACC];
#pragma unroll
  for (int i = 0; i < NACC; ++i) tot[i] = 0.0;
  if (isP && threadIdx.x == 0) rstamp(6);
  const unsigned long long mtag = seq << 8;
  double* box_kuu = fin.gacc + 8;
  double* box_pr = fin.gacc + FIN_GACC_PR;
  if (!isP || isPR) {
    double v = red[0];
#pragma unroll
    for (int i = 1; i < 7; ++i) v = (lane == i) ? red[i] : v;
    bm_msg_send(isPR ? box_pr : box_kuu, nmine, v, mtag | (isPR ? 5ull : 4ull), lane);
    if (threadIdx.x == 0) rstamp(2);
    return;
  }
  double kuu_v = 0.0, pr_v = 0.0;
  {
    bool ok = true;
    if (kuu_ok) kuu_v = lane < 4 ? kuu_pref[lane] : 0.0;
    else ok = bm_msg_recv(box_kuu, 4, kuu_v, mtag | 4ull, lane, spin_limit);
    if (ok && fin.split) ok = bm_msg_recv(box_pr, 7, pr_v, mtag | 5ull, lane, spin_limit);
    if (!ok) { if (lane == 0) atomicExch(info + 1, -1); return; }
  }
  {
    const int pidx[7] = {SPDK, SPK, SPA, AKA, ADKA, AAA, BA};
#pragma unroll
    for (int i = 0; i < 7; ++i) tot[pidx[i]] = red[i] + (fin.split ? __shfl(pr_v, i, 64) : 0.0);
  }
  tot[TRKA] = __shfl(kuu_v, 0, 64); tot[DTRKA] = __shfl(kuu_v, 1, 64); tot[SKDK] = __shfl(kuu_v, 2, 64); tot[SKK] = __shfl(kuu_v, 3, 64);
  if (threadIdx.x != 0) return;
#pragma unroll
  for (int i = 0; i < 14; ++i) __hip_atomic_store(fin.gacc + i, 0.0, __ATOMIC_RELAXED, __HIP_MEMORY_SCOPE_AGENT);
  {
    const double v = th_v.v, sn = th_v.s, N = th_v.N, Nw = th_v.Nw;
    const double yy = stats[(long)(K + 1) * M + M];
    const double asc = asc_v;
    tot[AKA] *= asc * asc; tot[ADKA] *= asc * asc; tot[AAA] *= asc * asc; tot[BA] *= asc;
    tot[LOGK] = __hip_atomic_load(logdets + 0, __ATOMIC_RELAXED, __HIP_MEMORY_SCOPE_AGENT);
    tot[LOGP] = __hip_atomic_load(logdets + 2, __ATOMIC_RELAXED, __HIP_MEMORY_SCOPE_AGENT);
    tot[CC] = tot[BA] / sn;
    const double two_pi = 6.283185307179586476925286766559;
    double elbo = -0.5 * N * log(two_pi * sn);
    elbo -= 0.5 * tot[LOGP];
    elbo += 0.5 * tot[LOGK];
    elbo -= 0.5 * yy / sn;
    elbo += 0.5 * tot[CC];
    elbo -= 0.5 * Nw * v / sn;
    elbo += 0.5 * tot[TRKA] / sn;
    if (th_v.cw != 0.0) elbo += th_v.cw;
    const double d_l = 0.5 * (tot[SKDK] - tot[SPDK] - tot[ADKA] + tot[DTRKA] / sn);
    const double d_v = 0.5 * (-tot[SKK] / v + tot[SPK] / v + tot[AKA] / v + tot[TRKA] / (v * sn)) - 0.5 * Nw / sn;
    const double s2 = sn * sn;
    const double d_s = -0.5 * N / sn + 0.5 * tot[SPA] / s2 + 0.5 * yy / s2 + 0.5 * tot[AAA] / s2 - tot[BA] / s2 + 0.5 * Nw * v / s2 - 0.5 * tot[TRKA] / s2;
    double* out = fin.out;
    out[0] = elbo; out[1] = d_v; out[2] = d_l; out[3] = d_s;
    out[4] = tot[LOGK]; out[5] = tot[LOGP]; out[6] = tot[TRKA]; out[7] = tot[CC];
    if (fin.mirror) {
      double* m = fin.mirror;
      const double mv[10] = {elbo, d_v, d_l, d_s, tot[LOGK], tot[LOGP], tot[TRKA], tot[CC],
                             (double)__hip_atomic_load(info, __ATOMIC_RELAXED, __HIP_MEMORY_SCOPE_AGENT),
                             (double)__hip_atomic_load(info + 1, __ATOMIC_RELAXED, __HIP_MEMORY_SCOPE_AGENT)};
      double sum = (double)fin.mirror_seq;
#pragma unroll
      for (int i = 0; i < 10; ++i) { __hip_atomic_store(m + i, mv[i], __ATOMIC_RELAXED, __HIP_MEMORY_SCOPE_SYSTEM); sum += mv[i]; }
      __hip_atomic_store(m + 11, sum, __ATOMIC_RELAXED, __HIP_MEMORY_SCOPE_SYSTEM);
      __hip_atomic_store(m + 10, (double)fin.mirror_seq, __ATOMIC_RELAXED, __HIP_MEMORY_SCOPE_SYSTEM);
    }
  }
  rstamp(2);
}

static __global__ void scale_sub_kernel(const double* __restrict__ a, const double* __restrict__ b, double* __restrict__ o,
                                 long n) {
  long i = (long)blockIdx.x * blockDim.x + threadIdx.x;
  if (i < n) o[i] = a[i] - b[i];
}
static __global__ void scale_kernel(double* __restrict__ x, double f, long n) {
  long i = (long)blockIdx.x * blockDim.x + threadIdx.x;
  if (i < n) x[i] = x[i] * f;
}

static double now_us() { timespec ts; clock_gettime(CLOCK_MONOTONIC, &ts); return ts.tv_sec * 1e6 + ts.tv_nsec * 1e-3; }

struct ChainCall {
  Handle* h; const double *S, *A, *b; KuuCoefs2 cf; int kind; double s; long M, D; Ws w; int* info; hipStream_t st; const FusedFin* fin;
  double t_enter;
};
static void scale_after(const ChainCall& c, const ChainPlan& p) {
  const long n = c.M * c.D;
  if (p.scale_c) hipLaunchKernelGGL(scale_kernel, dim3((unsigned)((n + 255) / 256)), dim3(256), 0, c.st, c.w.c, 1.0 / c.s, n);
  if (p.scale_alpha) hipLaunchKernelGGL(scale_kernel, dim3((unsigned)((n + 255) / 256)), dim3(256), 0, c.st, c.w.alpha, 1.0 / c.s, n);
}
static void set_pending_forward(Handle* h, const KuuCoefs2& cf, const TableSlot& slot) {
  for (int t = 0; t < ASVGP_MAX_KUU_TERMS; ++t) { h->fwd.coef[t] = cf.c[t]; h->fwd.dcoef[t] = cf.dc[t]; }
  h->fwd.tab = slot.tab; h->fwd.slot = slot.slot; h->fwd.seq = slot.seq;
}
static FusedFin chain_fin(const ChainCall& c, const ChainPlan& p) {
  FusedFin ff{};
  if (c.fin) { ff = *c.fin; ff.finalize = 1; }
  ff.n_helpers = p.n_helpers;
  ff.split = p.split;
  ff.xchg = p.split ? c.w.LP : nullptr;
  ff.assembled = reinterpret_cast<unsigned*>(c.w.fin + 20);
  ff.debug_no_assembly = debug_env().no_assembly;
  ff.debug_stamps = debug_env().chain_stamps;
  return ff;
}
static void interior_dkuu(const PriorPlan* plan, const double* dc, double* dk, double* dkb) {
  double bnd2[2 * PRIOR_BND_DIAGS * PRIOR_BND];
  long lo2 = 0, hi2 = 0;
  prior_plan_interior_kuu(plan, dc, dk, &lo2, &hi2, bnd2);
  for (int sd = 0; sd < 2; ++sd)
    for (int d = 0; d <= BM_B; ++d)
      for (int cI = 0; cI < KI_DKB; ++cI)
        dkb[(sd * 5 + d) * KI_DKB + cI] = bnd2[(size_t)(sd * PRIOR_BND_DIAGS + d) * PRIOR_BND + cI];
}
static int grant_lds(const void* kern, size_t lds_bytes) {
  const hipError_t e = hipFuncSetAttribute(kern, hipFuncAttributeMaxDynamicSharedMemorySize, (int)lds_bytes);
  if (e == hipSuccess) return ASVGP_OK;
  set_error("hipFuncSetAttribute: %s", hipGetErrorString(e));
  return ASVGP_ERR_LDS_CAPACITY;
}

template <int K>
static int launch_planned_mfma(const ChainCall& c, const ChainPlan& p) {
  Handle* h = c.h;
  const Ws& w = c.w;
  const int n_rec = prior_plan_nrec(h->plan);
  const bool host_times = debug_env().host_times != 0;
  KuuInterior ki;
  prior_plan_interior_kuu(h->plan, c.cf.c, ki.k, &ki.lo, &ki.hi, ki.bnd);
  interior_dkuu(h->plan, c.cf.dc, ki.dk, ki.dkb);
  ki.dk_tab = (ki.lo <= KI_DKB && c.M - ki.hi <= KI_DKB) ? 1 : 0;
  const double t_acq0 = host_times ? now_us() : 0.0;
  TableSlot slot(h);
  const double t_acq1 = host_times ? now_us() : 0.0;
  const double* tab_k = h->tab_dev + (size_t)slot.slot * h->slot_doubles;
  const unsigned long long* ready = h->ready_dev + slot.slot;
  if (p.fwd == FWD_GPU) {
    double* t = nullptr;
    const int rc = handle_prior_dd_forward(h, c.cf.c, c.cf.dc, slot.slot, c.st, &t, nullptr, slot.seq, &ready);
    if (rc) return rc;
    tab_k = t;
  }
  FusedFin ff = chain_fin(c, p);
  const long spin_limit = debug_env().spin_limit;
  auto kern = elbo_chains_mfma_kernel<K>;
  static size_t lds_granted[16] = {0};
  size_t& granted = lds_granted[h->device & 15];
  if (p.lds_bytes > granted) {
    const int rc = grant_lds(reinterpret_cast<const void*>(kern), p.lds_bytes);
    if (rc) return rc;
    granted = p.lds_bytes;
  }
  const double t0 = host_times ? now_us() : 0.0;
  const ThetaBox* box_k = nullptr;
  if (p.fwd == FWD_HOST_BEFORE) {
    (void)prior_plan_eval(h->plan, c.cf.c, c.cf.dc, slot.tab);
    ready = nullptr;
  } else if (p.fwd == FWD_AHEAD) {
    static_assert(sizeof(ThetaBox) <= BOX_BYTES, "theta box");
    if (!h->box_host) {
      if (hipHostMalloc(&h->box_host, BOX_BYTES * TAB_SLOTS, hipHostMallocMapped | hipHostMallocPortable | hipHostMallocCoherent) != hipSuccess ||
          hipHostGetDevicePointer(&h->box_dev, h->box_host, 0) != hipSuccess) {
        if (h->box_host) { (void)hipHostFree(h->box_host); h->box_host = nullptr; }
        set_error("launch-ahead: pinned allocation failed: %s", hipGetErrorString(hipGetLastError()));
        return ASVGP_ERR_HIP;
      }
      memset(h->box_host, 0, BOX_BYTES * TAB_SLOTS);
    }
    ThetaBox* bh = reinterpret_cast<ThetaBox*>(static_cast<char*>(h->box_host) + (size_t)slot.slot * BOX_BYTES);
    __atomic_store_n(&bh->seq, 0ull, __ATOMIC_RELEASE);
    box_k = reinterpret_cast<const ThetaBox*>(static_cast<const char*>(h->box_dev) + (size_t)slot.slot * BOX_BYTES);
  }
  if (h->mirror_dev) { ff.mirror = h->mirror_dev; ff.mirror_seq = ++h->mirror_seq; h->mirror_pending = ff.mirror_seq; }
  if (p.fwd == FWD_WORKER) {
    set_pending_forward(h, c.cf, slot);
    handle_post_forward(h);
  }
  hipLaunchKernelGGL(kern, dim3(p.grid), dim3(BM_THREADS), p.lds_bytes, c.st, ki, c.S, c.cf, w.Kuu, w.dK, c.A, c.b, (int)c.M, w.bcrP, w.SP, w.alpha,
                     w.logdets, c.info, c.s, tab_k, n_rec, h->node_rec_dev, w.bcrK, w.SK, w.dSK, h->done_dev + slot.slot, slot.seq, ready, spin_limit, ff,
                     box_k);
  switch (p.fwd) {
    case FWD_AHEAD: {
      const int rc = slot.launched(check_launch("elbo chains (matrix cores, launched ahead of theta)"));
      if (rc == ASVGP_OK) h->ahead = Handle::PendingAhead{true, slot.slot, slot.seq, slot.tab, c.kind, ff.th.N, ff.th.Nw, ff.th.cw};
      return rc;
    }
    case FWD_GPU: return slot.launched(check_launch("elbo chains (matrix cores, forward pass on the GPU)"));
    case FWD_WORKER: return slot.launched(check_launch("elbo chains (matrix cores, forward pass on the worker thread)"));
    case FWD_DEFERRED:
      h->fwd.valid = true;
      set_pending_forward(h, c.cf, slot);
      return slot.launched(check_launch("elbo chains (matrix cores, forward pass deferred)"));
    default: break;
  }
  const double t1 = host_times ? now_us() : 0.0;
  if (p.fwd == FWD_HOST_INLINE) (void)prior_plan_eval(h->plan, c.cf.c, c.cf.dc, slot.tab);
  if (host_times) {
    static double acc_launch = 0.0, acc_plan = 0.0, acc_pre = 0.0, acc_acq = 0.0, acc_a = 0.0;
    static long calls = 0;
    const bool plan_first = p.fwd == FWD_HOST_BEFORE;
    const double t2 = now_us();
    acc_acq += t_acq1 - t_acq0; acc_a += t_acq0 - c.t_enter;
    acc_pre += t0 - c.t_enter; acc_launch += t1 - t0; acc_plan += t2 - t1;
    if (++calls % 200 == 0) {
      fprintf(stderr, "[entry -> acquire %.1f us, table acquire %.1f us] ", acc_a / 200, acc_acq / 200);
      fprintf(stderr, "[asvgp host times, mean of 200 calls] entry -> launch call %.1f us | launch call (%s) %.1f us | %s %.1f us\n", acc_pre / 200,
              plan_first ? "forward pass + hipLaunchKernel" : "hipLaunchKernel", acc_launch / 200, plan_first ? "-" : "forward pass", acc_plan / 200);
      acc_a = acc_acq = acc_launch = acc_plan = acc_pre = 0.0;
    }
  }
  __atomic_store_n(h->ready_host + slot.slot, slot.seq, __ATOMIC_RELEASE);
  return slot.launched(check_launch("elbo chains (planned prior)"));
}

template <int K, bool TANGENT>
static int launch_planned_bcr(const ChainCall& c, const ChainPlan& p) {
  Handle* h = c.h;
  const Ws& w = c.w;
  constexpr bool HAS_BIG = (K <= 5);
  const int n_rec = prior_plan_nrec(h->plan);
  TableSlot slot(h);
  const double* tab_k = h->tab_dev + (size_t)slot.slot * h->slot_doubles;
  if (p.fwd == FWD_GPU) {
    double* t = nullptr;
    const int rc = handle_prior_dd_forward(h, c.cf.c, c.cf.dc, slot.slot, c.st, &t);
    if (rc) return rc;
    tab_k = t;
  } else {
    (void)prior_plan_eval(h->plan, c.cf.c, c.cf.dc, slot.tab);
    __atomic_store_n(h->ready_host + slot.slot, slot.seq, __ATOMIC_RELEASE);
  }
  const FusedFin ff = chain_fin(c, p);
  auto kern = p.big ? elbo_chains_kernel<K, HAS_BIG> : elbo_chains_kernel<K, false>;
  const int rc = grant_lds(reinterpret_cast<const void*>(kern), p.lds_bytes);
  if (rc) return rc;
  hipLaunchKernelGGL(kern, dim3(p.grid), dim3(BCR_THREADS), p.lds_bytes, c.st, c.S, c.cf, w.Kuu, TANGENT ? w.dK : (double*)nullptr, c.A, c.b,
                     (int)c.M, w.bcrP, w.SP, w.alpha, w.logdets, c.info, c.s, tab_k, n_rec, h->node_rec_dev, w.bcrK, w.SK, w.dSK,
                     h->done_dev + slot.slot, slot.seq, (int)c.D, (int)(p.lds_bytes / sizeof(double)), ff);
  scale_after(c, p);
  return slot.launched(check_launch("elbo chains (planned prior)"));
}

template <int K, bool TANGENT>
static int launch_bcr(const ChainCall& c, const ChainPlan& p) {
  const Ws& w = c.w;
  constexpr bool HAS_BIG = (K <= 5);
  const long E = (long)(K + 1) * c.M;
  hipLaunchKernelGGL(elbo_prepare_kernel, dim3((unsigned)((E + 255) / 256)), dim3(256), 0, c.st, c.S, c.cf, E, c.A, c.s, w.Kuu, w.dK, w.P);
  auto kern = p.big ? elbo_bcr_kernel<K, TANGENT, HAS_BIG> : elbo_bcr_kernel<K, TANGENT, false>;
  const int rc = grant_lds(reinterpret_cast<const void*>(kern), p.lds_bytes);
  if (rc) return rc;
  hipLaunchKernelGGL(kern, dim3(p.grid), dim3(BCR_THREADS), p.lds_bytes, c.st, w.Kuu, w.dK, w.P, c.b, (int)c.M, w.bcrK, w.bcrP, w.SK, w.dSK, w.SP,
                     w.alpha, w.logdets, c.info, debug_env().bcr_stamps, 0, (int)c.D, (int)(p.lds_bytes / sizeof(double)));
  scale_after(c, p);
  return check_launch("elbo chains");
}
template <int K>
static int launch_bcr_prior(const ChainCall& c, const ChainPlan& p) {
  Handle* h = c.h;
  const Ws& w = c.w;
  constexpr bool HAS_BIG = (K <= 5);
  const long E = (long)(K + 1) * c.M;
  hipLaunchKernelGGL(elbo_prepare_kernel, dim3((unsigned)((E + 255) / 256)), dim3(256), 0, c.st, c.S, c.cf, E, c.A, c.s, w.Kuu, w.dK, (double*)nullptr);
  if (h->sync_on) (void)hipEventRecord(h->evK, c.st);
  auto kern = p.big ? elbo_bcr_prior_kernel<K, HAS_BIG> : elbo_bcr_prior_kernel<K, false>;
  const int rc = grant_lds(reinterpret_cast<const void*>(kern), p.lds_bytes);
  if (rc) return rc;
  hipLaunchKernelGGL(kern, dim3(p.grid), dim3(BCR_THREADS), p.lds_bytes, c.st, w.Kuu, w.dK, (int)c.M, w.bcrK, w.SK, w.dSK, w.logdets, c.info,
                     debug_env().bcr_stamps);
  if (h->sync_on) (void)hipEventRecord(h->evP, c.st);
  return check_launch("elbo prior chain");
}
template <int K>
static int launch_bcr_data(const ChainCall& c, const ChainPlan& p) {
  Handle* h = c.h;
  const Ws& w = c.w;
  constexpr bool HAS_BIG = (K <= 5);
  if (h->sync_on) (void)hipStreamWaitEvent(c.st, h->evK, 0);
  auto kern = p.big ? elbo_bcr_data_kernel<K, HAS_BIG> : elbo_bcr_data_kernel<K, false>;
  const int rc = grant_lds(reinterpret_cast<const void*>(kern), p.lds_bytes);
  if (rc) return rc;
  hipLaunchKernelGGL(kern, dim3(p.grid), dim3(BCR_THREADS), p.lds_bytes, c.st, w.Kuu, c.A, c.b, (int)c.M, w.bcrP, w.SP, w.alpha, w.logdets, c.info,
                     debug_env().bcr_stamps, c.s, (int)c.D, (int)(p.lds_bytes / sizeof(double)));
  scale_after(c, p);
  return check_launch("elbo chains");
}

template <int K, bool TANGENT>
static int launch_sweeps(const ChainCall& c, const ChainPlan& p) {
  const Ws& w = c.w;
  const long E = (long)(K + 1) * c.M, D = c.D;
  const int M = (int)c.M;
  hipLaunchKernelGGL(elbo_prepare_kernel, dim3((unsigned)((E + 255) / 256)), dim3(256), 0, c.st, c.S, c.cf, E, c.A, c.s, w.Kuu, w.dK, w.P);
  if (D == 1) {
    hipLaunchKernelGGL((elbo_factor_kernel<K, TANGENT, true>), dim3(p.grid), dim3(64), 0, c.st, w.Kuu, w.dK, w.P, w.LK, w.dLK, w.LP, c.b, w.c, M, c.info);
    hipLaunchKernelGGL((elbo_inverse_kernel<K, TANGENT, true>), dim3(p.grid), dim3(64), 0, c.st, w.LK, w.dLK, w.LP, w.SK, w.dSK, w.SP, w.c, w.alpha, M);
  } else {
    hipLaunchKernelGGL((elbo_factor_kernel<K, TANGENT, false>), dim3(p.grid), dim3(64), 0, c.st, w.Kuu, w.dK, w.P, w.LK, w.dLK, w.LP, c.b, w.c, M, c.info);
    hipLaunchKernelGGL(elbo_trsv_kernel<K>, dim3((unsigned)D), dim3(64), 0, c.st, w.LP, M, c.b, w.c, D, 0, 1.0);
    hipLaunchKernelGGL((elbo_inverse_kernel<K, TANGENT, false>), dim3(p.grid), dim3(64), 0, c.st, w.LK, w.dLK, w.LP, w.SK, w.dSK, w.SP, w.c, w.alpha, M);
    hipLaunchKernelGGL(elbo_trsv_kernel<K>, dim3((unsigned)D), dim3(64), 0, c.st, w.LP, M, w.c, w.alpha, D, 1, 1.0);
  }
  scale_after(c, p);
  return check_launch("elbo chains");
}

template <int K, bool TANGENT>
static int run_chains(Handle* h, const double* stats, const double* S, int kind, double v, double l, double s, long M, long D,
                      Ws w, int* info, hipStream_t st, ChainPlan& p, int part = 0, const FusedFin* fin = nullptr) {
  ChainCall c{h, S, stats, stats ? stats + (long)(K + 1) * M : nullptr, {}, kind, s, M, D, w, info, st, fin, debug_env().host_times ? now_us() : 0.0};
  for (int t = 0; t < ASVGP_MAX_KUU_TERMS; ++t) c.cf.c[t] = c.cf.dc[t] = 0.0;
  const int rc = asvgp_matern_coeffs(kind, v, l, c.cf.c, c.cf.dc, &c.cf.n);
  if (rc) return rc;
  const bool have_plan = h->plan && prior_plan_M(h->plan) == M && prior_plan_k(h->plan) == K && prior_plan_terms(h->plan) == c.cf.n;
  p = plan_chains<K, TANGENT>(ChainPlanIn{h->band_algo, have_plan, have_plan ? prior_plan_nrec(h->plan) : 0, have_plan && prior_plan_interior(h->plan),
                                          M, D, part, fin != nullptr, h->ahead_req, h->prior_forward_gpu, h->fwd_worker, h->defer_forward,
                                          debug_env().no_split != 0, debug_env().plan_first != 0});
  if (p.status) { set_error("%s", p.msg); return p.status; }
  if (p.nothing) return ASVGP_OK;
  switch (p.path) {
    case PATH_PLANNED_MFMA: if constexpr (K == BM_B) return launch_planned_mfma<K>(c, p); break;
    case PATH_PLANNED_BCR: return launch_planned_bcr<K, TANGENT>(c, p);
    case PATH_BCR: return launch_bcr<K, TANGENT>(c, p);
    case PATH_BCR_PRIOR: if constexpr (TANGENT) return launch_bcr_prior<K>(c, p); break;
    case PATH_BCR_DATA: return launch_bcr_data<K>(c, p);
    case PATH_SWEEPS: return launch_sweeps<K, TANGENT>(c, p);
  }
  set_error("elbo chains: no launcher for this plan in this unit");
  return ASVGP_ERR_UNSUPPORTED;
}

template <int K>
int ElboLauncher<K>::run(Handle* h, const double* stats, const double* S, int kind, double v, double l, double s, long N, long M, long D,
                         double* out, int* info, void* ws, hipStream_t st, int part) {
  {
    Ws w = carve(ws, M, K, D);
    ChainPlan p;
    h->mirror_pending = 0;
    ElboScalars th{v, l, s, (double)N, (double)N, 0.0};
    if (h->w_set) { th.N = h->w_npos; th.Nw = h->w_sum; th.cw = 0.5 * (double)D * h->w_sumlog; }
    const int fin_blocks = (int)((M + 255) / 256 < 64 ? (M + 255) / 256 : 64);
    static_assert(BCR_THREADS == 256, "the fused finalize shares the chain kernel's workgroup size");
    const FusedFin ff{stats, th, 1.0 / s, w.fin, reinterpret_cast<unsigned*>(w.fin + 16), reinterpret_cast<unsigned*>(w.fin + 18), nullptr, out, D, 0, 0};
    int rc = run_chains<K, true>(h, stats, S, kind, v, l, s, M, D, w, info, st, p, part, part == 1 ? nullptr : &ff);
    if (rc || (part == 1)) return rc;
    if (p.path == PATH_PLANNED_BCR || p.path == PATH_PLANNED_MFMA) return check_launch("elbo_grad_1d (fused)");
    const bool bcr = p.path != PATH_SWEEPS;
    if (h->sync_on && p.path == PATH_BCR_DATA && h->evP) (void)hipStreamWaitEvent(st, h->evP, 0);
    hipLaunchKernelGGL(elbo_finalize_kernel<K>, dim3(fin_blocks), dim3(256), 0, st, stats, w.Kuu, w.dK, w.LK, w.LP, w.SK,
                       w.dSK, w.SP, w.c, w.alpha, bcr ? w.logdets : (const double*)nullptr, M, K, D, th,
                       bcr ? 1.0 / s : 1.0, w.fin, reinterpret_cast<unsigned*>(w.fin + 16), out);
    return check_launch("elbo_grad_1d");
  }
}
template <int K>
int PostLauncher<K>::run(Handle* h, const double* stats, const double* S, int kind, double v, double l, double s, long M, long D,
                         double* alpha, double* W, int* info, void* ws, hipStream_t st, double* Pinv) {
  {
    Ws w = carve(ws, M, K, D);
    ChainPlan p;
    int rc = run_chains<K, false>(h, stats, S, kind, v, l, s, M, D, w, info, st, p);
    if (rc) return rc;
    long E = (long)(K + 1) * M;
    hipLaunchKernelGGL(scale_sub_kernel, dim3((unsigned)((E + 255) / 256)), dim3(256), 0, st, w.SP, w.SK, W, E);
    hipError_t e = hipMemcpyAsync(alpha, w.alpha, sizeof(double) * M * D, hipMemcpyDeviceToDevice, st);
    if (e == hipSuccess && Pinv) e = hipMemcpyAsync(Pinv, w.SP, sizeof(double) * E, hipMemcpyDeviceToDevice, st);
    if (e != hipSuccess) { set_error("hipMemcpyAsync: %s", hipGetErrorString(e)); return ASVGP_ERR_HIP; }
    return check_launch(Pinv ? "posterior_prepare_loo_1d" : "posterior_prepare_1d");
  }
}

#if !defined(ASVGP_ELBO_PART) || ASVGP_ELBO_PART == 2
static __global__ void cov_recip_kernel(const double* __restrict__ LK, const double* __restrict__ LP, long M, double* __restrict__ rK,
                                        double* __restrict__ rP, const int* __restrict__ finfo, int* __restrict__ info) {
  const long j = (long)blockIdx.x * blockDim.x + threadIdx.x;
  if (j < M) { rK[j] = 1.0 / LK[j]; rP[j] = 1.0 / LP[j]; }
  if (j < 2 && info[j] == 0 && finfo[j] != 0) info[j] = finfo[j];
}

constexpr int COV_CH = 64;
template <int K>
__global__ __launch_bounds__(64) void cov_rows_kernel(const double* __restrict__ LK, const double* __restrict__ LP, const double* __restrict__ rK,
                                                      const double* __restrict__ rP, const double* __restrict__ SK, const double* __restrict__ SP,
                                                      const double* __restrict__ Wb, int M, double* __restrict__ Wd) {
  constexpr int NV = 2 * K + 2;
  __shared__ double tab[COV_CH][NV];
  const int lane = threadIdx.x;
  const int i0 = blockIdx.x * COV_CH;
  const int i = i0 + lane;
  const bool live = i < M;
  const int jtop = (i0 + COV_CH - 1 < M - 1) ? i0 + COV_CH - 1 : M - 1;
  double wk[K], wp[K];
#pragma unroll
  for (int l = 0; l < K; ++l) wk[l] = wp[l] = 0.0;
  double nxt[NV];
  auto fetch = [&](int jhi) {
    const int j = jhi - lane;
    if (j >= 0) {
#pragma unroll
      for (int l = 1; l <= K; ++l) { nxt[l - 1] = LK[(long)l * M + j]; nxt[K + l - 1] = LP[(long)l * M + j]; }
      nxt[2 * K] = rK[j];
      nxt[2 * K + 1] = rP[j];
    }
  };
  fetch(jtop);
  for (int jhi = jtop; jhi >= 0; jhi -= COV_CH) {
#pragma unroll
    for (int v = 0; v < NV; ++v) tab[lane][v] = nxt[v];
    __syncthreads();
    if (jhi - COV_CH >= 0) fetch(jhi - COV_CH);
    const int nj = jhi + 1 < COV_CH ? jhi + 1 : COV_CH;
    for (int c = 0; c < nj; ++c) {
      const int j = jhi - c;
      const int d = i - j;
      double sk = 0.0, sp = 0.0;
      if (live && d > K) {
        double ak = 0.0, ap = 0.0;
#pragma unroll
        for (int l = K; l >= 1; --l) { ak = fma(tab[c][l - 1], wk[l - 1], ak); ap = fma(tab[c][K + l - 1], wp[l - 1], ap); }
        sk = -ak * tab[c][2 * K];
        sp = -ap * tab[c][2 * K + 1];
        Wd[(long)j * M + i] = sp - sk;
      } else if (live && d >= 0) {
        sk = SK[(long)d * M + j];
        sp = SP[(long)d * M + j];
        Wd[(long)j * M + i] = Wb[(long)d * M + j];
      }
#pragma unroll
      for (int l = K - 1; l >= 1; --l) { wk[l] = wk[l - 1]; wp[l] = wp[l - 1]; }
      wk[0] = sk;
      wp[0] = sp;
    }
    __syncthreads();
  }
}

static __global__ __launch_bounds__(256) void cov_mirror_kernel(double* __restrict__ Wd, int M) {
  const int bi = blockIdx.y, bj = blockIdx.x;
  if (bj > bi) return;
  __shared__ double t[64][65];
  const int tx = threadIdx.x & 63, ty = threadIdx.x >> 6;
  for (int r = ty; r < 64; r += 4) {
    const int j = bj * 64 + r, i = bi * 64 + tx;
    if (i < M && j <= i) t[r][tx] = Wd[(long)j * M + i];
  }
  __syncthreads();
  for (int r = ty; r < 64; r += 4) {
    const int i = bi * 64 + r, j = bj * 64 + tx;
    if (i < M && j < i) Wd[(long)i * M + j] = t[tx][r];
  }
}

template <int K>
int PostCovLauncher<K>::run(Handle* h, const double* stats, const double* S, int kind, double v, double l, double s, long M, long D,
                            double* alpha, double* W, double* Wd, int* info, void* ws, hipStream_t st) {
  int rc = PostLauncher<K>::run(h, stats, S, kind, v, l, s, M, D, alpha, W, info, ws, st);
  if (rc) return rc;
  const Ws w = carve(ws, M, K, D);
  const long E = (long)(K + 1) * M;
  double* c = static_cast<double*>(ws) + ws_doubles(M, K, D);
  double *Kb = c, *Pb = c + E, *LKb = c + 2 * E, *LPb = c + 3 * E, *rK = c + 4 * E, *rP = rK + M;
  int* finfo = reinterpret_cast<int*>(rP + M);
  KuuCoefs2 cf;
  for (int t = 0; t < ASVGP_MAX_KUU_TERMS; ++t) cf.c[t] = cf.dc[t] = 0.0;
  rc = asvgp_matern_coeffs(kind, v, l, cf.c, cf.dc, &cf.n);
  if (rc) return rc;
  hipLaunchKernelGGL(elbo_prepare_kernel, dim3((unsigned)((E + 255) / 256)), dim3(256), 0, st, S, cf, E, stats, s, Kb, (double*)nullptr, Pb);
  rc = asvgp_cholesky_band(Kb, LKb, M, K, finfo, st);
  if (rc) return rc;
  rc = asvgp_cholesky_band(Pb, LPb, M, K, finfo + 1, st);
// ... 169 lines not shown
    if (m[10] == want) {
      double r[12];
      for (int i = 0; i < 12; ++i) r[i] = m[i];
      double sum = want;
      for (int i = 0; i < 10; ++i) sum += r[i];
      if (r[10] == want && (sum == r[11] || r[11] != r[11])) {
        for (int i = 0; i < 10; ++i) result10[i] = r[i];
        return ASVGP_OK;
      }
    }
    __builtin_ia32_pause();
    if ((spins & 1023) == 1023) {
      struct timespec t1;
      clock_gettime(CLOCK_MONOTONIC, &t1);
      if ((double)(t1.tv_sec - t0.tv_sec) + 1e-9 * (double)(t1.tv_nsec - t0.tv_nsec) > timeout_seconds) return 1;
    }
  }
}
extern "C" int asvgp_elbo_grad_ahead_1d(asvgp_handle_t handle, const double* stats, const double* static_bands, int kind, int64_t N, int64_t M,
                                        int k, int64_t D, double* out, int* info, void* workspace, size_t workspace_bytes, asvgp_stream_t stream) {
  Handle* h = as_handle(handle);
  if (h->ahead.valid) { set_error("elbo_grad_ahead_1d: the previous launch still waits for its theta (asvgp_elbo_publish_theta)"); return ASVGP_ERR_BAD_ARG; }
  if (!h->mirror_host) { const double* p = nullptr; const int rcm = asvgp_result_mirror(handle, 1, &p); if (rcm) return rcm; }
  h->ahead_req = true;
  const int rc = asvgp_elbo_grad_1d(handle, stats, static_bands, kind, 1.0, 1.0, 1.0, N, M, k, D, out, info, workspace, workspace_bytes, stream);
  h->ahead_req = false;
  return rc;
}
extern "C" int asvgp_elbo_publish_theta(asvgp_handle_t handle, double variance, double lengthscale, double noise_variance) {
  if (!(variance > 0.0) || !(lengthscale > 0.0) || !(noise_variance > 0.0)) { set_error("elbo_publish_theta: bad argument"); return ASVGP_ERR_BAD_ARG; }
  return elbo_publish_theta(as_handle(handle), variance, lengthscale, noise_variance, false);
}
extern "C" int asvgp_elbo_grad_host_1d(asvgp_handle_t handle, const double* stats, const double* static_bands, int kind, double variance,
                                       double lengthscale, double noise_variance, int64_t N, int64_t M, int k, int64_t D,
                                       double* out, int* info, void* workspace, size_t workspace_bytes, asvgp_stream_t stream,
                                       double* result10, double timeout_seconds) {
  Handle* h = as_handle(handle);
  if (!h->mirror_host) { const double* p = nullptr; const int rcm = asvgp_result_mirror(handle, 1, &p); if (rcm) return rcm; }
  const int rc = asvgp_elbo_grad_1d(handle, stats, static_bands, kind, variance, lengthscale, noise_variance, N, M, k, D, out, info, workspace,
                                    workspace_bytes, stream);
  if (rc) return rc;
  return asvgp_result_mirror_read(handle, h->mirror_pending, result10, timeout_seconds);
}

extern "C" int asvgp_elbo_prior_chain_1d(asvgp_handle_t handle, const double* static_bands, int kind, double variance, double lengthscale,
                                         double noise_variance, int64_t M, int k, int64_t D, int* info, void* workspace,
                                         size_t workspace_bytes, asvgp_stream_t stream) {
  int rc = elbo_args_ok(static_bands, static_bands, static_bands, M, k, D, variance, lengthscale, noise_variance, workspace,
                        workspace_bytes, info, "elbo_prior_chain_1d");
  if (rc) return rc;
  Handle* h = as_handle(handle);
  hipStream_t st = as_stream(stream);
  return for_bandwidth(k, [&](auto kk) {
    return ElboLauncher<decltype(kk)::value>::run(h, nullptr, static_bands, kind, variance, lengthscale, noise_variance, 0, (long)M, (long)D, nullptr, info, workspace, st, 1);
  });
}

extern "C" int asvgp_elbo_data_chain_1d(asvgp_handle_t handle, const double* stats, const double* static_bands, int kind, double variance,
                                        double lengthscale, double noise_variance, int64_t N, int64_t M, int k, int64_t D,
                                        double* out, int* info, void* workspace, size_t workspace_bytes,
                                        asvgp_stream_t stream) {
  int rc = elbo_args_ok(stats, static_bands, out, M, k, D, variance, lengthscale, noise_variance, workspace,
                        workspace_bytes, info, "elbo_data_chain_1d");
  if (rc) return rc;
  Handle* h = as_handle(handle);
  { const int rcf = handle_flush_phi_reduce(h, stats, as_stream(stream)); if (rcf) return rcf; }
  hipStream_t st = as_stream(stream);
  return for_bandwidth(k, [&](auto kk) {
    return ElboLauncher<decltype(kk)::value>::run(h, stats, static_bands, kind, variance, lengthscale, noise_variance, (long)N, (long)M, (long)D, out, info, workspace, st, 2);
  });
}

extern "C" int asvgp_kuu_inverse_band_1d(asvgp_handle_t handle, const double* static_bands, int kind, double variance, double lengthscale,
                                         int64_t M, int k, double* Kuu, double* dKuu_dl, double* S, double* dS_dl, double* logdet2, int* info,
                                         void* workspace, size_t workspace_bytes, asvgp_stream_t stream) {
  if (!static_bands || !Kuu || !dKuu_dl || !S || !dS_dl || !logdet2 || !info || M < 1 || !(variance > 0.0) || !(lengthscale > 0.0)) {
    set_error("kuu_inverse_band_1d: bad argument");
    return ASVGP_ERR_BAD_ARG;
  }
  if (k < 1 || k > ASVGP_MAX_ORDER) { set_error("kuu_inverse_band_1d: bandwidth %d outside 1..%d", k, (int)ASVGP_MAX_ORDER); return ASVGP_ERR_UNSUPPORTED; }
  if (!workspace || workspace_bytes < asvgp_elbo_workspace_bytes(M, k, 1)) { set_error("kuu_inverse_band_1d: workspace too small"); return ASVGP_ERR_WORKSPACE; }
  Handle* h = as_handle(handle);
  hipStream_t st = as_stream(stream);
  return for_bandwidth(k, [&](auto kk) {
    return KuuInvLauncher<decltype(kk)::value>::run(h, static_bands, kind, variance, lengthscale, (long)M, Kuu, dKuu_dl, S, dS_dl, logdet2, info, workspace, st);
  });
}

extern "C" int asvgp_posterior_prepare_1d(asvgp_handle_t handle, const double* stats, const double* static_bands, int kind, double variance,
                                          double lengthscale, double noise_variance, int64_t M, int k, int64_t D,
                                          double* alpha, double* W, int* info, void* workspace, size_t workspace_bytes,
                                          asvgp_stream_t stream) {
  int rc = elbo_args_ok(stats, static_bands, alpha, M, k, D, variance, lengthscale, noise_variance, workspace,
                        workspace_bytes, info, "posterior_prepare_1d");
  if (rc) return rc;
  if (!W) { set_error("posterior_prepare_1d: bad argument"); return ASVGP_ERR_BAD_ARG; }
  Handle* h = as_handle(handle);
  { const int rcf = handle_flush_phi_reduce(h, stats, as_stream(stream)); if (rcf) return rcf; }
  hipStream_t st = as_stream(stream);
  return for_bandwidth(k, [&](auto kk) {
    return PostLauncher<decltype(kk)::value>::run(h, stats, static_bands, kind, variance, lengthscale, noise_variance, (long)M, (long)D, alpha, W, info, workspace, st);
  });
}

extern "C" int asvgp_posterior_prepare_loo_1d(asvgp_handle_t handle, const double* stats, const double* static_bands, int kind, double variance,
                                              double lengthscale, double noise_variance, int64_t M, int k, int64_t D,
                                              double* alpha, double* W, double* Pinv_band, int* info, void* workspace, size_t workspace_bytes,
                                              asvgp_stream_t stream) {
  int rc = elbo_args_ok(stats, static_bands, alpha, M, k, D, variance, lengthscale, noise_variance, workspace,
                        workspace_bytes, info, "posterior_prepare_loo_1d");
  if (rc) return rc;
  if (!W || !Pinv_band) { set_error("posterior_prepare_loo_1d: bad argument"); return ASVGP_ERR_BAD_ARG; }
  Handle* h = as_handle(handle);
  { const int rcf = handle_flush_phi_reduce(h, stats, as_stream(stream)); if (rcf) return rcf; }
  hipStream_t st = as_stream(stream);
  return for_bandwidth(k, [&](auto kk) {
    return PostLauncher<decltype(kk)::value>::run(h, stats, static_bands, kind, variance, lengthscale, noise_variance, (long)M, (long)D, alpha, W, info, workspace, st, Pinv_band);
  });
}

extern "C" size_t asvgp_posterior_cov_workspace_bytes(int64_t M, int k, int64_t D) {
  if (M < 1 || k < 1 || k > ASVGP_MAX_ORDER || D < 1) return 0;
  return sizeof(double) * (ws_doubles(M, k, D) + cov_ws_doubles(M, k));
}

extern "C" int asvgp_posterior_cov_prepare_1d(asvgp_handle_t handle, const double* stats, const double* static_bands, int kind, double variance,
                                              double lengthscale, double noise_variance, int64_t M, int k, int64_t D,
                                              double* alpha, double* W, double* W_dense, int* info, void* workspace, size_t workspace_bytes,
                                              asvgp_stream_t stream) {
  int rc = elbo_args_ok(stats, static_bands, alpha, M, k, D, variance, lengthscale, noise_variance, workspace,
                        workspace_bytes, info, "posterior_cov_prepare_1d");
  if (rc) return rc;
  if (!W || !W_dense) { set_error("posterior_cov_prepare_1d: bad argument"); return ASVGP_ERR_BAD_ARG; }
  if (workspace_bytes < asvgp_posterior_cov_workspace_bytes(M, k, D)) {
    set_error("posterior_cov_prepare_1d: workspace too small (asvgp_posterior_cov_workspace_bytes)");
    return ASVGP_ERR_WORKSPACE;
  }
  Handle* h = as_handle(handle);
  { const int rcf = handle_flush_phi_reduce(h, stats, as_stream(stream)); if (rcf) return rcf; }
  hipStream_t st = as_stream(stream);
  return for_bandwidth(k, [&](auto kk) {
    return PostCovLauncher<decltype(kk)::value>::run(h, stats, static_bands, kind, variance, lengthscale, noise_variance, (long)M, (long)D, alpha, W, W_dense, info, workspace, st);
  });
}

extern "C" int asvgp_elbo_launch_plan_host(int band_algorithm, int have_plan, int n_rec, int interior, int64_t M, int k, int64_t D, int part, int tangent,
                                           int fused_finalize, int ahead, int prior_forward_gpu, int forward_worker, int defer_forward, int no_split,
                                           int plan_first, int64_t* plan12_host) {
  if (!plan12_host || M < 1 || D < 1 || part < 0 || part > 2 || band_algorithm < 0 || band_algorithm > 4) {
    set_error("elbo_launch_plan_host: bad argument");
    return ASVGP_ERR_BAD_ARG;
  }
  const ChainPlanIn in{band_algorithm, have_plan != 0, n_rec, interior != 0, (long)M, (long)D, part, fused_finalize != 0, ahead != 0,
                       prior_forward_gpu != 0, forward_worker != 0, defer_forward != 0, no_split != 0, plan_first != 0};
  ChainPlan p{};
  p.status = ASVGP_ERR_UNSUPPORTED;
  snprintf(p.msg, sizeof(p.msg), "elbo_launch_plan_host: bandwidth %d outside 1..%d", k, (int)ASVGP_MAX_ORDER);
  (void)for_bandwidth(k, [&](auto kk) {
    p = tangent ? plan_chains<decltype(kk)::value, true>(in) : plan_chains<decltype(kk)::value, false>(in);
    return 0;
  });
  const int64_t f[12] = {p.status, p.path, p.part, p.nothing, p.big, (int64_t)p.lds_bytes, p.grid, p.n_helpers, p.split, p.fwd, p.scale_alpha, p.scale_c};
  for (int i = 0; i < 12; ++i) plan12_host[i] = f[i];
  if (p.status) set_error("%s", p.msg);
  return p.status;
}

#endif
```

### asvgp_amd/csrc/handle.hip

```cpp
#include <sched.h>
#include <stdlib.h>
#include <string.h>
#include <time.h>

#include <condition_variable>
#include <mutex>
#include <thread>
#include <vector>

#include "handle.hpp"

namespace asvgp {

static DebugEnv g_dbg;
static std::once_flag g_dbg_once;
static void debug_env_load() {
  g_dbg.no_assembly = getenv("ASVGP_DEBUG_NO_ASSEMBLY") ? 1 : 0;
  g_dbg.chain_stamps = getenv("ASVGP_CHAIN_STAMPS") ? 1 : 0;
  g_dbg.spin_limit = getenv("ASVGP_SPIN_LIMIT") ? atol(getenv("ASVGP_SPIN_LIMIT")) : (1L << 25);
  g_dbg.host_times = getenv("ASVGP_HOST_TIMES") ? 1 : 0;
  g_dbg.plan_first = getenv("ASVGP_PLAN_FIRST") ? 1 : 0;
  g_dbg.bcr_stamps = getenv("ASVGP_BCR_STAMPS") ? atoi(getenv("ASVGP_BCR_STAMPS")) : 0;
  g_dbg.no_split = getenv("ASVGP_NO_SPLIT") ? atoi(getenv("ASVGP_NO_SPLIT")) : 0;
}
const DebugEnv& debug_env() {
  std::call_once(g_dbg_once, debug_env_load);
  return g_dbg;
}

static Handle* g_default = nullptr;
static std::mutex g_default_mu;

Handle* as_handle(asvgp_handle_t h) {
  if (h) return reinterpret_cast<Handle*>(h);
  std::lock_guard<std::mutex> lk(g_default_mu);
  if (!g_default) {
    g_default = new Handle;
    (void)hipGetDevice(&g_default->device);
  }
  return g_default;
}

static void handle_quiesce(Handle* h) {
  if (h->ahead.valid) (void)elbo_publish_theta(h, 1.0, 1.0, 1.0, true);
  handle_publish_forward(h);
  bool need_sync = false;
  struct timespec t0;
  clock_gettime(CLOCK_MONOTONIC, &t0);
  auto expired = [&]() { struct timespec t1; clock_gettime(CLOCK_MONOTONIC, &t1); return (t1.tv_sec - t0.tv_sec) > 2; };
  if (h->done_host && h->seq > 0) {
    volatile unsigned long long* flag = h->done_host + (h->seq % TAB_SLOTS);
    while (*flag < h->seq) { sched_yield(); if (expired()) { need_sync = true; break; } }
  }
  if (!need_sync && h->mirror_host && h->mirror_pending) {
    volatile double* m = h->mirror_host + 10;
    while (*m != (double)h->mirror_pending) { sched_yield(); if (expired()) { need_sync = true; break; } }
  }
  if (need_sync) (void)hipDeviceSynchronize();
}

static void plan_release(Handle* h) {
  handle_quiesce(h);
  if (h->plan) { prior_plan_destroy(h->plan); h->plan = nullptr; }
  handle_prior_dd_release(h);
  if (h->node_rec_dev) { (void)hipFree(h->node_rec_dev); h->node_rec_dev = nullptr; }
  if (h->tab_host) { (void)hipHostFree(h->tab_host); h->tab_host = nullptr; h->tab_dev = nullptr; }
  if (h->done_host) { (void)hipHostFree(h->done_host); h->done_host = nullptr; h->done_dev = nullptr; }
  if (h->ready_host) { (void)hipHostFree(h->ready_host); h->ready_host = nullptr; h->ready_dev = nullptr; }
  h->slot_doubles = 0;
}

static void worker_wait_idle(Handle* h) {
  while (__atomic_load_n(&h->wstate, __ATOMIC_ACQUIRE) == 1) sched_yield();
}
struct WorkerPark {
  std::mutex mu;
  std::condition_variable cv;
  int parked = 0;
};
static WorkerPark* park_of(Handle* h) { return static_cast<WorkerPark*>(h->worker_park); }
static void worker_main(Handle* h) {
  long idle = 0;
  WorkerPark* pk = park_of(h);
  for (;;) {
    const int st = __atomic_load_n(&h->wstate, __ATOMIC_ACQUIRE);
    if (st == 2) return;
    if (st == 1) {
      if (h->plan) (void)prior_plan_eval(h->plan, h->fwd.coef, h->fwd.dcoef, h->fwd.tab);
      __atomic_store_n(h->ready_host + h->fwd.slot, h->fwd.seq, __ATOMIC_RELEASE);
      __atomic_store_n(&h->wstate, 0, __ATOMIC_RELEASE);
      idle = 0;
    } else if (++idle > 200000) {
      std::unique_lock<std::mutex> lk(pk->mu);
      pk->parked = 1;
      pk->cv.wait(lk, [&] { return __atomic_load_n(&h->wstate, __ATOMIC_ACQUIRE) != 0; });
      pk->parked = 0;
      idle = 0;
    } else {
      __builtin_ia32_pause();
    }
  }
}
static void worker_signal(Handle* h, int state) {
  WorkerPark* pk = park_of(h);
  __atomic_store_n(&h->wstate, state, __ATOMIC_SEQ_CST);
  bool wake;
  { std::lock_guard<std::mutex> lk(pk->mu); wake = pk->parked != 0; }
  if (wake) pk->cv.notify_one();
}
void handle_post_forward(Handle* h) {
  if (!h->worker) {
    h->worker_park = new WorkerPark;
    h->worker = new std::thread(worker_main, h);
  }
  worker_signal(h, 1);
}
static void worker_stop(Handle* h) {
  if (!h->worker) return;
  worker_wait_idle(h);
  worker_signal(h, 2);
  std::thread* t = static_cast<std::thread*>(h->worker);
  t->join();
  delete t;
  delete park_of(h);
  h->worker_park = nullptr;
  h->worker = nullptr;
  h->wstate = 0;
}

void handle_publish_forward(Handle* h) {
  if (h->worker) worker_wait_idle(h);
  if (!h->fwd.valid) return;
  h->fwd.valid = false;
  if (h->plan) (void)prior_plan_eval(h->plan, h->fwd.coef, h->fwd.dcoef, h->fwd.tab);
  __atomic_store_n(h->ready_host + h->fwd.slot, h->fwd.seq, __ATOMIC_RELEASE);
}

double* handle_table_acquire(Handle* h, unsigned long long* seq_out, int* slot_out) {
  handle_publish_forward(h);
  const unsigned long long seq = ++h->seq;
  const int slot = (int)(seq % TAB_SLOTS);
  if (seq > TAB_SLOTS) {
    const unsigned long long need = seq - TAB_SLOTS;
    volatile unsigned long long* flag = h->done_host + slot;
    struct timespec t0;
    clock_gettime(CLOCK_MONOTONIC, &t0);
    while (*flag < need) {
      sched_yield();
      struct timespec t1;
      clock_gettime(CLOCK_MONOTONIC, &t1);
      if ((t1.tv_sec - t0.tv_sec) > 2) { (void)hipDeviceSynchronize(); break; }
    }
  }
  *seq_out = seq;
  *slot_out = slot;
  return h->tab_host + (size_t)slot * h->slot_doubles;
}

bool handle_mesh_is_linspace(Handle* h, const double* mesh_dev, long n_mesh, hipStream_t st, double* step_out, double* first_out, double* last_out) {
  for (int i = 0; i < h->n_mesh_seen; ++i)
    if (h->mesh_seen[i].ptr == mesh_dev && h->mesh_seen[i].n == n_mesh) {
      *step_out = h->mesh_seen[i].step;
      if (first_out) *first_out = h->mesh_seen[i].first;
      if (last_out) *last_out = h->mesh_seen[i].last;
      return h->mesh_seen[i].regular != 0;
    }
  std::vector<double> m((size_t)n_mesh);
  bool regular = false;
  double step = 0.0, first = 0.0, last = 0.0;
  if (n_mesh >= 2 && hipMemcpyAsync(m.data(), mesh_dev, sizeof(double) * (size_t)n_mesh, hipMemcpyDeviceToHost, st) == hipSuccess &&
      hipStreamSynchronize(st) == hipSuccess) {
    const double m0 = m[0];
    first = m0; last = m[n_mesh - 1];
    step = (m[n_mesh - 1] - m0) / (double)(n_mesh - 1);
    regular = step > 0.0 && step == step;
    for (long i = 0; i < n_mesh - 1 && regular; ++i) {
// ... 271 lines not shown
```

### asvgp_amd/csrc/handle.hpp

```cpp
#pragma once
#include "asvgp_common.hpp"
#include "prior_plan.hpp"

namespace asvgp {

constexpr int PROF_RING = 1024;
constexpr int TAB_SLOTS = 16;

struct Handle {
  unsigned magic = 0x41535647u;
  int device = 0;
  int phi_algo = 0, phi_blocks = 0;
  int phi_last = 0;
  bool phi_defer = false;
  struct PendingReduce { const double* partials; int G, M, K; double* stats; bool valid; const int* ranges; } pend = {nullptr, 0, 0, 0, nullptr, false, nullptr};
  int band_algo = 0;
  bool sync_on = false;
  hipEvent_t evK = nullptr, evP = nullptr;
  bool prof_on = false, prof_made = false;
  int prof_every = 1;
  long prof_calls = 0, prof_n = 0;
  hipEvent_t prof_ev[PROF_RING][2];
  PriorPlan* plan = nullptr;
  int* node_rec_dev = nullptr;
  double* tab_host = nullptr;
  double* tab_dev = nullptr;
  unsigned long long* done_host = nullptr;
  unsigned long long* done_dev = nullptr;
  unsigned long long* ready_host = nullptr;
  unsigned long long* ready_dev = nullptr;
  size_t slot_doubles = 0;
  unsigned long long seq = 0;
  int plan_terms = 0;
  bool defer_forward = false;
  bool fwd_worker = false;
  void* worker = nullptr;
  void* worker_park = nullptr;
  int wstate = 0;
  struct PendingForward { bool valid; double coef[ASVGP_MAX_KUU_TERMS], dcoef[ASVGP_MAX_KUU_TERMS]; double* tab; int slot; unsigned long long seq; } fwd = {false, {0}, {0}, nullptr, 0, 0};
  bool prior_forward_gpu = false;
  int* dd_img_i = nullptr;
  int dd_n_img = 0;
  double* dd_img_d = nullptr;
  double* dd_tab = nullptr;
  hipStream_t dd_stream = nullptr;
  unsigned long long* dd_ready = nullptr;
  double* mirror_host = nullptr;
  double* mirror_dev = nullptr;
  unsigned long long mirror_seq = 0;
  unsigned long long mirror_pending = 0;
  struct MeshSeen { const double* ptr; long n; int regular; double step, first, last; };
  MeshSeen mesh_seen[8];
  int n_mesh_seen = 0;
  int phi_order = 0;
  struct OrderSeen { const double* ptr; long n; int series; };
  OrderSeen order_seen[8];
  int n_order_seen = 0;
  int* order_dev = nullptr;
  int phi_last_series = 0;
  bool ahead_req = false;
  void* box_host = nullptr;
  void* box_dev = nullptr;
  struct PendingAhead { bool valid; int slot; unsigned long long seq; double* tab; int kind; double N, Nw, cw; } ahead = {false, 0, 0, nullptr, 0, 0.0, 0.0, 0.0};
  bool w_set = false;
  double w_npos = 0.0, w_sum = 0.0, w_sumlog = 0.0;
};
constexpr size_t BOX_BYTES = 4096;

struct DebugEnv { int no_assembly; int chain_stamps; long spin_limit; int host_times; int plan_first; int bcr_stamps; int no_split; };
const DebugEnv& debug_env();

Handle* as_handle(asvgp_handle_t h);

bool handle_mesh_is_linspace(Handle* h, const double* mesh_dev, long n_mesh, hipStream_t st, double* step_out, double* first_out, double* last_out);

int handle_flush_phi_reduce(Handle* h, const double* stats, hipStream_t st);

void handle_publish_forward(Handle* h);
void handle_post_forward(Handle* h);

int handle_prior_dd_prepare(Handle* h);
void handle_prior_dd_release(Handle* h);
int handle_prior_dd_forward(Handle* h, const double* coef, const double* dcoef, int slot, hipStream_t st, double** tab_out, unsigned long long* stamps = nullptr,
                            unsigned long long seq = 0, const unsigned long long** ready_out = nullptr);

int elbo_publish_theta(Handle* h, double v, double l, double s, bool withdraw);

double* handle_table_acquire(Handle* h, unsigned long long* seq_out, int* slot_out);
struct TableSlot {
  Handle* h; unsigned long long seq = 0; int slot = 0; double* tab; bool owned = true;
  explicit TableSlot(Handle* hh) : h(hh) { tab = handle_table_acquire(h, &seq, &slot); }
  TableSlot(const TableSlot&) = delete;
  TableSlot& operator=(const TableSlot&) = delete;
  int launched(int rc) { if (rc == ASVGP_OK) owned = false; return rc; }
  ~TableSlot() {
    if (!owned) return;
    __atomic_store_n(h->ready_host + slot, seq, __ATOMIC_RELEASE);
    __atomic_store_n(h->done_host + slot, seq, __ATOMIC_RELEASE);
  }
};

}
```

### asvgp_amd/csrc/phi_launch.hpp

```cpp
#pragma once
#include <type_traits>

namespace asvgp {

constexpr size_t PHI_LDS_MAX = 160 * 1024;

struct PhiGrid { int G; long ppb; };
static PhiGrid phi_grid(long N, int blocks, long unit, long round) {
  const long nblk = (N + unit - 1) / unit;
  const long gmax = (blocks > 0 && blocks < PHI_MAX_BLOCKS) ? blocks : PHI_MAX_BLOCKS;
  const int G = (int)(nblk < 1 ? 1 : (nblk > gmax ? gmax : nblk));
  return PhiGrid{G, ((N + G - 1) / G + round - 1) / round * round};
}

static int phi_s0(long ppb) {
  int lg = 1;
  for (long c = 2; c < ppb; c <<= 1) ++lg;
  return 62 - lg < 50 ? 62 - lg : 50;
}

static int phi_max_cols(int K, long n_mesh, bool fx) {
  long avail = (long)PHI_LDS_BUDGET - (long)n_mesh * 8 - 16 * 8;
  if (avail <= 0) return 0;
  return (int)(avail / (8 * (K + 2 + (fx ? 1 : 0))));
}
static size_t phi_band_lds_bytes(int K, bool fx, int ncols, long n_mesh) { return sizeof(double) * ((size_t)(K + 2 + (fx ? 1 : 0)) * ncols + n_mesh + 16); }

static int phi_reduce_split(int G) { return G >= 64 ? 16 : (G >= 8 ? 4 : 1); }
static void enqueue_phi_reduce(hipStream_t st, const double* partials, int G, int ncols, int K, int cell0, long M, long D, int dcol, int do_band,
                               double* stats, const int* ranges) {
  const int E1 = (K + 2) * ncols + 1;
  hipLaunchKernelGGL(phi_reduce_kernel, dim3((E1 + 255) / 256, phi_reduce_split(G)), dim3(256), 0, st, partials, G, ncols, K, cell0, M, D, dcol, do_band, stats, ranges);
}

template <class Kern, class... Args>
static int phi_launch(Handle* h, hipStream_t st, Kern kern, int G, int threads, size_t lds_bytes, Args... args) {
  hipError_t e = hipFuncSetAttribute(reinterpret_cast<const void*>(kern), hipFuncAttributeMaxDynamicSharedMemorySize, (int)lds_bytes);
  if (e != hipSuccess) { set_error("hipFuncSetAttribute(%zu B LDS): %s", lds_bytes, hipGetErrorString(e)); return ASVGP_ERR_LDS_CAPACITY; }
  const bool prof = h->prof_on && h->prof_n < PROF_RING && (h->prof_calls++ % h->prof_every == 0);
  if (prof) (void)hipEventRecord(h->prof_ev[h->prof_n][0], st);
  hipLaunchKernelGGL(kern, dim3((unsigned)G), dim3(threads), lds_bytes, st, args...);
  if (prof) { (void)hipEventRecord(h->prof_ev[h->prof_n][1], st); ++h->prof_n; }
  return ASVGP_OK;
}

template <class F>
static int for_phi_order(int order, F&& f) {
  switch (order) {
    case 1: return f(std::integral_constant<int, 1>{});
    case 2: return f(std::integral_constant<int, 2>{});
    case 3: return f(std::integral_constant<int, 3>{});
    case 4: return f(std::integral_constant<int, 4>{});
    case 5: return f(std::integral_constant<int, 5>{});
    case 6: return f(std::integral_constant<int, 6>{});
  }
  return ASVGP_ERR_UNSUPPORTED;
}

enum PhiNeed { PHI_NEED_NOTHING = 0, PHI_NEED_MESH, PHI_NEED_ORDER };
struct PhiInputs {
  long N, D, M, n_mesh; double delta;
  bool weighted;
  int algo, blocks; bool defer;
  bool aligned16;
  int mesh_regular; double mesh_first, mesh_last, mesh_step;
  int series;
};
struct PhiPlan {
  int status; char msg[256];
  int need;
  int kernel;
  int series;
  int shape;
  size_t lds_bytes;
  int G; long ppb;
  int s0;
  int cells_per_chunk, chunks;
  int launches, reduces, reduce_y;
  bool defer;
  bool asked_mesh, asked_order;
};

static double phi_knot_margin(const PhiInputs& in) {
  const double amax = fabs(in.mesh_first) > fabs(in.mesh_last) ? fabs(in.mesh_first) : fabs(in.mesh_last);
  return 16.0 * 2.220446049250313e-16 * amax / in.delta + 1e-12;
}

template <int K>
static PhiPlan plan_phi(const PhiInputs& in) {
  PhiPlan p{};
  p.s0 = -1;
  auto refuse = [&p](int status, const char* fmt, auto... a) { p.status = status; snprintf(p.msg, sizeof(p.msg), fmt, a...); return p; };
  auto ask = [&p](int fact) { p.need = fact; return p; };
  auto whole = [&](int kernel, int series, int shape, size_t lds, PhiGrid g, bool fixed_point, bool may_defer) {
    p.kernel = kernel; p.series = series; p.shape = shape; p.lds_bytes = lds; p.G = g.G; p.ppb = g.ppb;
    if (fixed_point) p.s0 = phi_s0(g.ppb);
    p.cells_per_chunk = (int)in.n_mesh - 1; p.chunks = 1; p.launches = 1;
    p.defer = may_defer && in.defer;
    p.reduces = p.defer ? 0 : 1; p.reduce_y = phi_reduce_split(g.G);
    return p;
  };
  const int algo = in.algo;
  const int ncells = (int)in.n_mesh - 1;
  const char* entry = in.weighted ? "phi_accumulate_1d_weighted" : "phi_accumulate_1d";
  if (in.weighted && (algo == 3 || algo == 5))
    return refuse(ASVGP_ERR_UNSUPPORTED, "%s: phi algorithm %d accumulates in fixed point, whose scales are bounds on the unweighted products - it has no weighted form (0 or 1)", entry, algo);
  const bool streams = in.D == 1 && in.aligned16;

  if (algo == 0 || algo == 6) {
    bool applies = streams && in.N >= 2 && in.M <= PS_NCELL;
    if (applies) {
      if (in.mesh_regular < 0) return ask(PHI_NEED_MESH);
      p.asked_mesh = true;
      applies = in.mesh_regular != 0 && phi_knot_margin(in) < 0.125;
    }
    if (applies && !in.weighted) {
      if (in.series < 0) return ask(PHI_NEED_ORDER);
      p.asked_order = true;
    }
    if (applies) {
      constexpr int TP = ps_tile_points<K>(), TPS = TP < 4 ? TP : 4, TPW = psw_tile_points<K>();
      static_assert(psw_lds_bytes<K, TPW>() <= PHI_LDS_MAX && ps_epilogue_bytes<K>() <= PHI_LDS_MAX, "weighted register-moment kernel: LDS plan exceeds 160 KB");
      struct { int kernel, series, tp; size_t lds; bool tried; } inst[3] = {
          {16, 0, TPW, psw_lds_bytes<K, TPW>(), in.weighted},
          {6, 1, TPS, ps_lds_bytes<K, TPS, 1>(), !in.weighted && in.series > 0},
          {6, 0, TP, ps_lds_bytes<K, TP, 0>(), !in.weighted}};
      for (const auto& i : inst) {
        if (!i.tried) continue;
        const size_t lds = i.lds > ps_epilogue_bytes<K>() ? i.lds : ps_epilogue_bytes<K>();
        const PhiGrid g = phi_grid(in.N, in.blocks, (long)i.tp * PS_THREADS, i.series ? 128 : 2);
        if (lds > PHI_LDS_MAX || g.ppb > 0x3fffffffL) continue;
        return whole(i.kernel, i.series, i.tp, lds, g, false, !in.weighted);
      }
    }
    if (algo == 6)
      return in.weighted ? refuse(ASVGP_ERR_UNSUPPORTED, "%s: phi algorithm 6 (register moments) needs D == 1, N >= 2, M <= 2048, 16-byte aligned x / y / w and a mesh that is an exact linspace", entry)
                         : refuse(ASVGP_ERR_UNSUPPORTED, "%s", "phi algorithm 6 (tile sort) needs D == 1, N >= 2, M <= 2048, 16-byte aligned x / y and a mesh that is an exact linspace");
  }

  if (!in.weighted && (algo == 0 || algo == 5)) {
    if (streams && in.N >= 1) {
      if (in.mesh_regular < 0) return ask(PHI_NEED_MESH);
      p.asked_mesh = true;
      const size_t lds[3] = {mq_lds_bytes<K, 512>(in.M), mq_lds_bytes<K, 1024>(in.M), mq_lds_bytes<K, 2048>(in.M)};
      for (int i = 0; i < 3; ++i)
        if (ncells <= (512 << i) && lds[i] <= PHI_LDS_BUDGET)
          return whole(5, 0, 512 << i, lds[i], phi_grid(in.N, in.blocks, 2 * MQ_THREADS, 2 * MQ_THREADS), true, true);
    }
    if (algo == 5) return refuse(ASVGP_ERR_UNSUPPORTED, "%s", "phi algorithm 5 (centred moments) needs D == 1, 16-byte aligned x / y and M small enough for the LDS split");
  }

  const bool fx = !in.weighted && algo != 1;
  const int maxc = phi_max_cols(K, in.n_mesh, fx);
  if (maxc < 2 * K + 2) return refuse(ASVGP_ERR_LDS_CAPACITY, "%s: mesh table (%ld knots) leaves no LDS for the band", entry, in.n_mesh);
  p.kernel = in.weighted ? 11 : (fx ? 3 : 1);
  p.cells_per_chunk = (in.M <= maxc) ? ncells : (maxc - K);
  p.chunks = (ncells + p.cells_per_chunk - 1) / p.cells_per_chunk;
  p.lds_bytes = phi_band_lds_bytes(K, fx, p.cells_per_chunk + K, in.n_mesh);
  const PhiGrid g = in.weighted ? phi_grid(in.N, in.blocks, PW_THREADS, 64) : phi_grid(in.N, in.blocks, 2 * PHI_THREADS, 2 * PHI_THREADS);
  p.G = g.G; p.ppb = g.ppb;
  if (fx) p.s0 = phi_s0(g.ppb);
  p.launches = p.reduces = (int)(p.chunks * in.D);
  p.reduce_y = phi_reduce_split(g.G);
  return p;
}

static bool handle_phi_is_series(Handle* h, const double* x, long N, double m0, double inv_delta, long n_mesh, hipStream_t st) {
  if (h->phi_order == 1) return false;
  if (h->phi_order == 2) return true;
  for (int i = 0; i < h->n_order_seen; ++i)
    if (h->order_seen[i].ptr == x && h->order_seen[i].n == N) return h->order_seen[i].series != 0;
  int series = 0;
  const int nprobe = 512;
  if (N >= 128L * nprobe) {
    if (!h->order_dev && hipMalloc(&h->order_dev, sizeof(int)) != hipSuccess) h->order_dev = nullptr;
    int cnt = 0;
    if (h->order_dev && hipMemsetAsync(h->order_dev, 0, sizeof(int), st) == hipSuccess) {
      hipLaunchKernelGGL(phi_order_probe_kernel, dim3(nprobe), dim3(64), 0, st, x, N, N / nprobe, nprobe, m0, inv_delta, (int)n_mesh, h->order_dev);
      if (hipMemcpyAsync(&cnt, h->order_dev, sizeof(int), hipMemcpyDeviceToHost, st) == hipSuccess && hipStreamSynchronize(st) == hipSuccess)
        series = cnt * 10 >= nprobe * 9 ? 1 : 0;
    }
  }
  if (h->n_order_seen < 8) h->order_seen[h->n_order_seen++] = Handle::OrderSeen{x, N, series};
  return series != 0;
}

struct PhiCall {
  PhiInputs in;
  const double* x; const double* y; const double* w; const double* mesh;
  double* stats; double* wstats;
  double* ws;
// ... 199 lines not shown
```

### include/asvgp_hip.h

```cpp
#ifndef ASVGP_HIP_H
#define ASVGP_HIP_H

#include <stddef.h>
#include <stdint.h>

#ifdef __cplusplus
extern "C" {
#endif

typedef void* asvgp_stream_t;
typedef struct asvgp_handle_s* asvgp_handle_t;

typedef enum {
  ASVGP_OK = 0,
  ASVGP_ERR_BAD_ARG = -1,
  ASVGP_ERR_UNSUPPORTED = -2,
  ASVGP_ERR_LDS_CAPACITY = -3,
  ASVGP_ERR_WORKSPACE = -4,
  ASVGP_ERR_HIP = -5
} asvgp_status;

enum { ASVGP_MATERN12 = 0, ASVGP_MATERN32 = 1, ASVGP_MATERN52 = 2 };
enum { ASVGP_MAX_ORDER = 6, ASVGP_MAX_BANDWIDTH = 8, ASVGP_MAX_KUU_TERMS = 9 };

int asvgp_version(void);
const char* asvgp_last_error_string(void);
const char* asvgp_status_name(int status);

int asvgp_create(asvgp_handle_t* handle_out);
int asvgp_destroy(asvgp_handle_t handle);

size_t asvgp_phi_workspace_bytes(int64_t M, int order, int64_t D);
int asvgp_phi_accumulate_1d(asvgp_handle_t handle, const double* x, const double* y, int64_t N, int64_t D,
                            const double* mesh, int64_t n_mesh, double delta, int order, int64_t M,
                            double* stats, void* workspace, size_t workspace_bytes, asvgp_stream_t stream);

int asvgp_set_phi_algorithm(asvgp_handle_t handle, int algo);
int asvgp_prior_interior_kuu_host(const double* static_bands_host, int n_terms, int64_t M, int k, const double* coef_host,
                                  double* kuu_diag8, int64_t* lo, int64_t* hi, double* bnd256);
int asvgp_host_mantissa_bits(void);
int asvgp_debug_reload_env(void);
int asvgp_set_deferred_forward_pass(asvgp_handle_t handle, int on);
int asvgp_prior_publish(asvgp_handle_t handle);
int asvgp_result_mirror(asvgp_handle_t handle, int enable, const double** host_ptr);
uint64_t asvgp_result_mirror_pending(asvgp_handle_t handle);
int asvgp_result_mirror_read(asvgp_handle_t handle, uint64_t token, double* result10, double timeout_seconds);
int asvgp_elbo_grad_ahead_1d(asvgp_handle_t handle, const double* stats, const double* static_bands, int kind, int64_t N, int64_t M, int k,
                             int64_t D, double* out, int* info, void* workspace, size_t workspace_bytes, asvgp_stream_t stream);
int asvgp_elbo_publish_theta(asvgp_handle_t handle, double variance, double lengthscale, double noise_variance);
int asvgp_elbo_grad_host_1d(asvgp_handle_t handle, const double* stats, const double* static_bands, int kind, double variance,
                            double lengthscale, double noise_variance, int64_t N, int64_t M, int k, int64_t D,
                            double* out, int* info, void* workspace, size_t workspace_bytes, asvgp_stream_t stream,
                            double* result10, double timeout_seconds);
int asvgp_phi_last_algorithm(asvgp_handle_t handle);
int asvgp_set_phi_input_order(asvgp_handle_t handle, int order);
int asvgp_phi_last_input_order(asvgp_handle_t handle);
int asvgp_stream_probe(const double* x, const double* y, int64_t N, double* sink, asvgp_stream_t stream);
int asvgp_set_phi_workgroups(asvgp_handle_t handle, int n);
int asvgp_set_phi_deferred_reduce(asvgp_handle_t handle, int on);
int asvgp_phi_reduce_1d(asvgp_handle_t handle, asvgp_stream_t stream);
int asvgp_phi_launch_plan_host(int phi_algorithm, int phi_workgroups, int deferred_reduce, int weighted, int64_t N, int64_t D, int64_t M, int order,
                               int64_t n_mesh, double delta, int aligned16, int mesh_regular, double mesh_first, double mesh_last, int series,
                               int64_t* plan16_host);

size_t asvgp_phi_weighted_workspace_bytes(int64_t M, int order, int64_t D);
int asvgp_phi_accumulate_1d_weighted(asvgp_handle_t handle, const double* x, const double* y, const double* w, int64_t N, int64_t D,
                                     const double* mesh, int64_t n_mesh, double delta, int order, int64_t M, double* stats,
                                     double* wstats, void* workspace, size_t workspace_bytes, asvgp_stream_t stream);
int asvgp_set_weight_sums(asvgp_handle_t handle, double n_pos, double sum_w, double sum_log_w);

int asvgp_phi_index_1d(const double* x, int64_t N, const double* mesh, int64_t n_mesh, double delta,
                       int64_t* idx, asvgp_stream_t stream);

int asvgp_phi_evaluate_1d(const double* x, int64_t N, const double* mesh, int64_t n_mesh, double delta,
                          int order, int deriv, int64_t* rows, double* data, asvgp_stream_t stream);

int asvgp_matern_coeffs(int kind, double variance, double lengthscale, double* coef_host, double* dcoef_dl_host,
                        int* n_terms_host);
int asvgp_kuu_assemble(const double* static_bands, int n_terms, const double* coef_host,
                       const double* dcoef_dl_host, int64_t M, int k, double* Kuu, double* dKuu_dl,
                       asvgp_stream_t stream);

int asvgp_cholesky_band(const double* K, double* L, int64_t M, int k, int* info, asvgp_stream_t stream);
int asvgp_inverse_from_cholesky_band(const double* L, double* S, int64_t M, int k, asvgp_stream_t stream);
int asvgp_solve_triang_mat(const double* L, const double* B, double* X, int64_t M, int k, int64_t D,
                           int transpose_left, asvgp_stream_t stream);
int asvgp_product_band_band(const double* left, const double* right, double* out, int64_t M,
                            int left_lower, int left_upper, int right_lower, int right_upper,
                            int result_lower, int result_upper, asvgp_stream_t stream);
int asvgp_transpose_band(const double* in, double* out, int64_t M, int lower, int upper, asvgp_stream_t stream);
int asvgp_symmetrise_band(const double* in, double* out, int64_t M, int lower, asvgp_stream_t stream);
int asvgp_unpack_banded_matrix_to_dense(const double* band, double* dense, int64_t M, int lower, int upper,
                                        asvgp_stream_t stream);
int asvgp_pack_dense_matrix_to_banded(const double* dense, double* band, int64_t M, int lower, int upper,
                                      asvgp_stream_t stream);
int asvgp_band_trace_sym(const double* S, const double* A, int64_t M, int k, double* out, asvgp_stream_t stream);

int asvgp_cholesky_band_vjp(const double* L, const double* Lbar, double* Kbar, double* work, int64_t M, int k, asvgp_stream_t stream);
int asvgp_inverse_from_cholesky_band_vjp(const double* L, const double* S, const double* Sbar, double* Lbar, double* work, int64_t M,
                                         int k, asvgp_stream_t stream);
int asvgp_band_outer_product(const double* U, const double* V, int64_t M, int64_t D, int k, double sign, double* out, asvgp_stream_t stream);
int asvgp_band_launch_plan_host(int op, int64_t M, int k, int lds, int seg_blocks, int64_t* plan8);

size_t asvgp_elbo_workspace_bytes(int64_t M, int k, int64_t D);
int asvgp_set_band_algorithm(asvgp_handle_t handle, int algo);
int asvgp_prior_plan_1d(asvgp_handle_t handle, const double* static_bands_host, int n_terms, int64_t M, int k, int* planned);
size_t asvgp_prior_table_doubles(const double* static_bands_host, int n_terms, int64_t M, int k);
int asvgp_prior_forward_host(const double* static_bands_host, int n_terms, int64_t M, int k, const double* coef_host,
                             const double* dcoef_dl_host, double* table_host, size_t table_doubles, int* node_rec_host);
int asvgp_set_prior_forward(asvgp_handle_t handle, int mode);
int asvgp_prior_forward_device(asvgp_handle_t handle, const double* coef_host, const double* dcoef_dl_host, double* table_host,
                               size_t table_doubles, void* stream);
int asvgp_prior_plan_image_host(const double* static_bands_host, int n_terms, int64_t M, int k, int* ints, size_t* n_ints,
                                double* doubles, size_t* n_doubles);
int asvgp_elbo_launch_plan_host(int band_algorithm, int have_plan, int n_rec, int interior, int64_t M, int k, int64_t D, int part, int tangent,
                                int fused_finalize, int ahead, int prior_forward_gpu, int forward_worker, int defer_forward, int no_split,
                                int plan_first, int64_t* plan12_host);
int asvgp_prior_forward_stamps(asvgp_handle_t handle, const double* coef_host, const double* dcoef_dl_host, uint64_t* out64, void* stream);
int asvgp_elbo_grad_1d(asvgp_handle_t handle, const double* stats, const double* static_bands, int kind, double variance,
                       double lengthscale, double noise_variance, int64_t N, int64_t M, int k, int64_t D,
                       double* out, int* info, void* workspace, size_t workspace_bytes, asvgp_stream_t stream);

int asvgp_kuu_inverse_band_1d(asvgp_handle_t handle, const double* static_bands, int kind, double variance, double lengthscale,
                              int64_t M, int k, double* Kuu, double* dKuu_dl, double* S, double* dS_dl, double* logdet2, int* info,
                              void* workspace, size_t workspace_bytes, asvgp_stream_t stream);

int asvgp_elbo_chain_sync(asvgp_handle_t handle, int enable);
int asvgp_elbo_prior_chain_1d(asvgp_handle_t handle, const double* static_bands, int kind, double variance, double lengthscale,
                              double noise_variance, int64_t M, int k, int64_t D, int* info, void* workspace,
                              size_t workspace_bytes, asvgp_stream_t stream);
int asvgp_elbo_data_chain_1d(asvgp_handle_t handle, const double* stats, const double* static_bands, int kind, double variance,
                             double lengthscale, double noise_variance, int64_t N, int64_t M, int k, int64_t D,
                             double* out, int* info, void* workspace, size_t workspace_bytes, asvgp_stream_t stream);

int asvgp_posterior_prepare_1d(asvgp_handle_t handle, const double* stats, const double* static_bands, int kind, double variance,
                               double lengthscale, double noise_variance, int64_t M, int k, int64_t D,
                               double* alpha, double* W, int* info, void* workspace, size_t workspace_bytes,
                               asvgp_stream_t stream);
int asvgp_predict_1d(const double* xnew, int64_t n, const double* mesh, int64_t n_mesh, double delta, int order,
                     int64_t M, const double* alpha, const double* W, double variance, int64_t D, double* mean,
                     double* var, asvgp_stream_t stream);
int asvgp_predict_1d_h(asvgp_handle_t handle, const double* xnew, int64_t n, const double* mesh, int64_t n_mesh, double delta, int order,
                       int64_t M, const double* alpha, const double* W, double variance, int64_t D, double* mean,
                       double* var, asvgp_stream_t stream);

size_t asvgp_posterior_cov_workspace_bytes(int64_t M, int k, int64_t D);
int asvgp_posterior_cov_prepare_1d(asvgp_handle_t handle, const double* stats, const double* static_bands, int kind, double variance,
                                   double lengthscale, double noise_variance, int64_t M, int k, int64_t D,
                                   double* alpha, double* W, double* W_dense, int* info, void* workspace, size_t workspace_bytes,
                                   asvgp_stream_t stream);
int asvgp_predict_cov_1d(asvgp_handle_t handle, const double* x1, int64_t n1, const double* x2, int64_t n2, const double* mesh,
                         int64_t n_mesh, double delta, int order, int64_t M, const double* W_dense, int kind, double variance,
                         double lengthscale, double* cov, int64_t ldc, asvgp_stream_t stream);

int asvgp_predict_deriv_1d(asvgp_handle_t handle, const double* xnew, int64_t n, const double* mesh, int64_t n_mesh, double delta,
                           int order, int64_t M, const double* alpha, const double* W, int kind, double variance, double lengthscale,
                           int64_t D, double* mean, double* var, asvgp_stream_t stream);
int asvgp_predict_cov_deriv_1d(asvgp_handle_t handle, const double* x1, int64_t n1, const double* x2, int64_t n2, const double* mesh,
                               int64_t n_mesh, double delta, int order, int64_t M, const double* W_dense, int kind, double variance,
                               double lengthscale, int p, int q, double* cov, int64_t ldc, asvgp_stream_t stream);

int asvgp_posterior_prepare_loo_1d(asvgp_handle_t handle, const double* stats, const double* static_bands, int kind, double variance,
                                   double lengthscale, double noise_variance, int64_t M, int k, int64_t D,
                                   double* alpha, double* W, double* Pinv_band, int* info, void* workspace, size_t workspace_bytes,
                                   asvgp_stream_t stream);
size_t asvgp_loo_workspace_bytes(int64_t M, int order, int64_t D);
int asvgp_loo_1d(asvgp_handle_t handle, const double* x, const double* y, const double* w, int64_t N, int64_t D, const double* mesh,
                 int64_t n_mesh, double delta, int order, int64_t M, const double* alpha, const double* W, const double* Pinv_band,
                 double variance, double noise_variance, double* mean, double* var, double* logdens, double* scores,
                 void* workspace, size_t workspace_bytes, asvgp_stream_t stream);

size_t asvgp_score_workspace_bytes(int64_t M, int order, int64_t D);
int asvgp_score_1d(asvgp_handle_t handle, const double* x, const double* y, const double* w, int64_t N, int64_t D, const double* mesh,
                   int64_t n_mesh, double delta, int order, int64_t M, const double* alpha, const double* W, double variance,
                   double noise_variance, double* mean, double* var, double* logdens, double* scores, void* workspace,
                   size_t workspace_bytes, asvgp_stream_t stream);

size_t asvgp_weight_grad_workspace_bytes(int64_t M, int order, int64_t D, int64_t G);
int asvgp_weight_grad_1d(asvgp_handle_t handle, const double* x, const double* y, const double* w, int64_t N, int64_t D,
                         const double* mesh, int64_t n_mesh, double delta, int order, int64_t M, const double* alpha, const double* W,
                         const double* Pinv_band, double variance, double noise_variance, const int32_t* groups, int64_t G, double* grad,
                         double* gsum, void* workspace, size_t workspace_bytes, asvgp_stream_t stream);

size_t asvgp_kron_stats_doubles(int64_t m1, int64_t m2, int k);
int asvgp_phi_accumulate_kron2d(const double* X, const double* y, int64_t N, const double* mesh1, int64_t n_mesh1,
                                double delta1, int64_t m1, const double* mesh2, int64_t n_mesh2, double delta2,
                                int64_t m2, int order, double* stats, asvgp_stream_t stream);
int asvgp_kron_evaluate_2d(const double* X, int64_t N, const double* mesh1, int64_t n_mesh1, double delta1,
                           const double* mesh2, int64_t n_mesh2, double delta2, int64_t m2, int order, int64_t* rows,
                           double* data, asvgp_stream_t stream);
int asvgp_kron_assemble(const double* K1, const double* K2, const double* S1, const double* S2, const double* Ablk, int k,
                        int64_t m1, int64_t m2, double noise_variance, double* Pb, double* trace_out,
                        asvgp_stream_t stream);
int asvgp_blockband_cholesky(double* Pb, int64_t M, int64_t bw, double* rhs, double* logdet, int* info,
                             asvgp_stream_t stream);
int asvgp_blockband_backsolve(const double* Lb, int64_t M, int64_t bw, double* x, asvgp_stream_t stream);
int asvgp_predict_kron2d(const double* Xnew, int64_t n, const double* mesh1, int64_t n_mesh1, double delta1, int64_t m1,
                         const double* mesh2, int64_t n_mesh2, double delta2, int64_t m2, int order, const double* alpha,
                         const double* S1, const double* S2, double* mean, double* qk, asvgp_stream_t stream);

int asvgp_kron_cell_index(const double* X, int64_t N, const double* mesh1, int64_t n_mesh1, double delta1,
                          const double* mesh2, int64_t n_mesh2, double delta2, int* cell, asvgp_stream_t stream);
int asvgp_phi_accumulate_kron2d_sorted(const double* Xs, const double* ys, int64_t N, const int64_t* cell_start,
                                       const double* mesh1, int64_t n_mesh1, double delta1, int64_t m1,
                                       const double* mesh2, int64_t n_mesh2, double delta2, int64_t m2, int order,
                                       double* stats, asvgp_stream_t stream);
int asvgp_phi_accumulate_kron2d_sorted_f32(const float* Xs, const float* ys, int64_t N, const int64_t* cell_start,
                                           const double* mesh1, int64_t n_mesh1, double delta1, int64_t m1,
                                           const double* mesh2, int64_t n_mesh2, double delta2, int64_t m2, int order,
                                           double* stats, asvgp_stream_t stream);
int asvgp_phi_accumulate_kron2d_weighted(const double* X, const double* y, const double* w, int64_t N, const double* mesh1, int64_t n_mesh1,
                                         double delta1, int64_t m1, const double* mesh2, int64_t n_mesh2, double delta2,
                                         int64_t m2, int order, double* stats, double* wstats, asvgp_stream_t stream);
int asvgp_phi_accumulate_kron2d_sorted_weighted(const double* Xs, const double* ys, const double* ws, int64_t N, const int64_t* cell_start,
                                                const double* mesh1, int64_t n_mesh1, double delta1, int64_t m1,
                                                const double* mesh2, int64_t n_mesh2, double delta2, int64_t m2, int order,
                                                double* stats, double* wstats, asvgp_stream_t stream);
int asvgp_kron_phi_launch_plan_host(int sorted, int weighted, int f32, int64_t N, int64_t m1, int64_t m2, int64_t n_mesh1, int64_t n_mesh2,
                                    int order, int atomics, int64_t grid, int staging, int64_t* plan12);

int asvgp_blockband_to_blocks(const double* Lb, int64_t M, int64_t bw, int64_t Bb, double* diag, double* sub,
                              asvgp_stream_t stream);
int asvgp_kron_grad_terms(const double* SigD, const double* SigS, int64_t Bb, const double* alpha, const double* Ablk,
                          const double* K1, const double* K2, const double* dK1, const double* dK2, const double* S1,
                          const double* S2, const double* Z1, const double* Z2, int k, int64_t m1, int64_t m2,
                          double* out11, asvgp_stream_t stream);
int asvgp_predict_kron2d_var(const double* Xnew, int64_t n, const double* mesh1, int64_t n_mesh1, double delta1,
                             const double* mesh2, int64_t n_mesh2, double delta2, int64_t m2, int order,
                             const double* SigD, const double* SigS, int64_t Bb, double* qp, asvgp_stream_t stream);
int asvgp_kron_assemble_twisted(const double* K1, const double* K2, const double* S1, const double* S2, const double* Ablk, int k,
                                int64_t m1, int64_t m2, double noise_variance, int64_t Bb, int64_t nb, int64_t top_end, int64_t padt,
                                int64_t padb, double* Pt, double* Pr, double* trace_out, asvgp_stream_t stream);
int asvgp_kron_grad_terms_twisted(const double* SigD, const double* SigS, int64_t Bb, int64_t nb, int64_t top_end, int64_t padt,
                                  int64_t padb, const double* alpha, const double* Ablk, const double* K1, const double* K2,
                                  const double* dK1, const double* dK2, const double* S1, const double* S2, const double* Z1,
                                  const double* Z2, int k, int64_t m1, int64_t m2, double* out11, asvgp_stream_t stream);
int asvgp_predict_kron2d_var_twisted(const double* Xnew, int64_t n, const double* mesh1, int64_t n_mesh1, double delta1,
                                     const double* mesh2, int64_t n_mesh2, double delta2, int64_t m1, int64_t m2, int order,
                                     const double* SigD, const double* SigS, int64_t Bb, int64_t nb, int64_t top_end, int64_t padt,
                                     int64_t padb, double* qp, asvgp_stream_t stream);
int asvgp_predict_grad_kron2d(const double* X, int64_t n, const double* mesh1, int64_t n_mesh1, double delta1, int64_t m1,
                              const double* mesh2, int64_t n_mesh2, double delta2, int64_t m2, int order, const double* alpha,
                              const double* S1, const double* S2, const double* SigD, const double* SigS, int64_t Bb, int twisted,
                              int64_t nb, int64_t top_end, int64_t padt, int64_t padb, int kind1, double variance1,
                              double lengthscale1, int kind2, double variance2, double lengthscale2, double* mean2, double* cov3,
                              asvgp_stream_t stream);

int asvgp_kron_dense_inverse(const double* G, const double* SigD, const double* SigS, int64_t M, int64_t Bb, int twisted, int64_t nb,
                             int64_t top_end, int64_t padt, int64_t padb, double* Sigma, asvgp_stream_t stream);
int asvgp_predict_cov_kron2d(asvgp_handle_t handle, const double* x1, int64_t n1, const double* x2, int64_t n2, const double* mesh1,
                             int64_t n_mesh1, double delta1, int64_t m1, const double* mesh2, int64_t n_mesh2, double delta2, int64_t m2,
                             int order, const double* Sigma, const double* K1inv, const double* K2inv, int kind1, double variance1,
                             double lengthscale1, int kind2, double variance2, double lengthscale2, double* cov, int64_t ldc,
                             asvgp_stream_t stream);

size_t asvgp_phi_cross_workspace_bytes(int64_t m_i, int64_t m_j);
int asvgp_phi_cross_2d(const double* x_i, const double* x_j, int64_t N, const double* mesh_i, int64_t n_mesh_i,
                       double delta_i, int64_t m_i, const double* mesh_j, int64_t n_mesh_j, double delta_j, int64_t m_j,
                       int order, double* out, void* workspace, size_t workspace_bytes, asvgp_stream_t stream);

enum { ASVGP_ADDITIVE_COV_MAX_D = 16 };
int asvgp_predict_cov_additive(asvgp_handle_t handle, const double* x1, int64_t n1, const double* x2, int64_t n2, int d,
                               const double* meshes, const int64_t* n_mesh, const double* delta, const int64_t* m, int order,
                               const int* kind, const double* variance, const double* lengthscale, const double* W, double* cov,
                               int64_t ldc, asvgp_stream_t stream);

int asvgp_predict_components_additive(asvgp_handle_t handle, const double* X, int64_t n, int d, const double* meshes,
                                      const int64_t* n_mesh, const double* delta, const int64_t* m, int order, const int* kind,
                                      const double* variance, const double* lengthscale, int deriv, const double* alpha,
                                      const double* W, double* mean, double* cov, asvgp_stream_t stream);
// ... 9 lines not shown
```

Before: 139,300.

## Pre-split first BCR levels of P-chain solve across many workgroups

Adds a wide pre-pass kernel that runs the first three block cyclic reduction levels of the banded solve across multiple 256-thread workgroups, each handling 32 blocks and writing survivor blocks, logdet and error info to a workspace. The main single-workgroup solver then starts at a later level, merging boundary contributions from adjacent groups. This moves the early, most parallel levels off the serial single-CU critical path at the cost of an extra kernel launch and a global round trip. It also caches hipFuncSetAttribute LDS grants so the attribute call is not repeated on every phi launch.

```diff
diff --git a/asvgp_amd/_lib.py b/asvgp_amd/_lib.py
--- a/asvgp_amd/_lib.py
+++ b/asvgp_amd/_lib.py
@@ -69,6 +69,7 @@
     "asvgp_prior_forward_stamps": (_I, [_P, _P, _P, _P, _P]),
     "asvgp_prior_plan_image_host": (_I, [_P, _I, _L, _I, _P, _P, _P, _P]),
     "asvgp_elbo_launch_plan_host": (_I, [_I, _I, _I, _I, _L, _I, _L, _I, _I, _I, _I, _I, _I, _I, _I, _I, _P]),
+    "asvgp_elbo_presplit_plan_host": (_I, [_I, _I, _I, _I, _L, _I, _L, _I, _I, _I, _I, _I, _I, _I, _I, _I, _I, _P]),
     "asvgp_elbo_grad_1d": (_I, [_P, _P, _P, _I, _D, _D, _D, _L, _L, _I, _L, _P, _P, _P, _Z, _P]),
     "asvgp_kuu_inverse_band_1d": (_I, [_P, _P, _I, _D, _D, _L, _I, _P, _P, _P, _P, _P, _P, _P, _Z, _P]),
     "asvgp_elbo_chain_sync": (_I, [_P, _I]),
diff --git a/asvgp_amd/csrc/bcr_mfma.hpp b/asvgp_amd/csrc/bcr_mfma.hpp
--- a/asvgp_amd/csrc/bcr_mfma.hpp
+++ b/asvgp_amd/csrc/bcr_mfma.hpp
@@ -89,10 +89,92 @@
 };
 constexpr int BM_XCHG = 96;
 
+constexpr int BMW_THREADS = 256, BMW_BLOCKS = 32, BMW_LEVELS = 3, BMW_MAX_WG = 16;
+constexpr int BMW_SURV = 36, BMW_LEFT = 4 * BMW_SURV, BMW_LOGDET = BMW_LEFT + 20, BMW_BAD = BMW_LOGDET + 1, BMW_WG = 192;
+__host__ __device__ inline size_t bcr_mfma_wide_ws_doubles() { return (size_t)BMW_MAX_WG * BMW_WG; }
+__host__ __device__ inline size_t bcr_mfma_wide_lds_doubles() {
+  return (size_t)2 * (BMW_BLOCKS / 2 + 1) * 16 + (size_t)(BMW_BLOCKS + 1) * BM_B + (size_t)(BMW_THREADS / 64) * 4 * 40 + 16;
+}
+
+struct BmLane { int r, q, c, e, et, hi, lo; };
+
+__device__ __forceinline__ void bm_forward_node(int l, int i, int a, int node0, bool act, bool hasb, const BmLane& g, double* Dl, double* El, double* xs,
+                                                double* slab, const double (&sl)[3], double* Fl, double* wsrec, int& bad, BmLog& ld, double& updb,
+                                                double& ybu) {
+  constexpr int B = BM_B;
+  const int r = g.r, c = g.c, e = g.e, et = g.et, hi = g.hi, lo = g.lo;
+  double d[10];
+  double ea, eb, da;
+  if (l == 0) {
+#pragma unroll
+    for (int t3 = 0; t3 < 3; ++t3) if (e + 16 * t3 < 40) slab[e + 16 * t3] = sl[t3];
+    int kk = 0;
+#pragma unroll
+    for (int rr = 0; rr < 4; ++rr)
+#pragma unroll
+      for (int cc = 0; cc <= rr; ++cc) d[kk++] = slab[(rr - cc) * 8 + 4 + cc];
+    ea = slab[(4 + lo - hi) * 8 + hi];
+    ea = (r <= c) ? ea : 0.0;
+    eb = slab[(4 + lo - hi) * 8 + 4 + hi];
+    eb = (hasb && c <= r) ? eb : 0.0;
+    da = slab[(hi - lo) * 8 + lo];
+  } else {
+    const double* Di = Dl + (size_t)(i >> 1) * 16;
+    int kk = 0;
+#pragma unroll
+    for (int rr = 0; rr < 4; ++rr)
+#pragma unroll
+      for (int cc = 0; cc <= rr; ++cc) d[kk++] = Di[rr * 4 + cc];
+    ea = El[(size_t)(a >> 1) * 16 + e];
+    eb = El[(size_t)(i >> 1) * 16 + et];
+    eb = hasb ? eb : 0.0;
+    da = Dl[(size_t)(a >> 1) * 16 + e];
+  }
+  double yv = xs[i * B + r], ya = xs[a * B + r];
+  yv = (c == 0) ? yv : 0.0;
+  ya = (c == 0) ? ya : 0.0;
+  double dprod;
+  int badj;
+  const double t = bm_chol_linv(d, hi, lo, dprod, badj);
+  if (act && badj && !bad) bad = (node0 + i) * B + badj;
+  const double linv = (r >= c) ? t : 0.0;
+  const double linvT = (c >= r) ? t : 0.0;
+  if (act) ld.mul(dprod);
+  const double ua = bm_mfma(linvT, ea, 0.0);
+  const double ub = bm_mfma(linvT, eb, 0.0);
+  const double zz = bm_mfma(linvT, yv, 0.0);
+  const double nua = -ua, nub = -ub;
+  const double da_new = bm_mfma(nua, ua, da);
+  const double e_new = bm_mfma(nub, ua, 0.0);
+  const double ya_new = bm_mfma(nua, zz, ya);
+  updb = bm_mfma(ub, ub, 0.0);
+  ybu = bm_mfma(ub, zz, 0.0);
+  updb = act ? updb : 0.0;
+  ybu = act ? ybu : 0.0;
+  const double gat = bm_mfma(ua, linv, 0.0);
+  const double gbt = bm_mfma(ub, linv, 0.0);
+  const double dinv = bm_mfma(linv, linv, 0.0);
+  const double w = bm_mfma(linv, zz, 0.0);
+  if (act) {
+    if (l >= 3) {
+      double* R = Fl + (size_t)(i >> 3) * 52;
+      R[e] = gat; R[16 + e] = gbt; R[32 + e] = dinv;
+      if (c == 0) R[48 + r] = w;
+    } else {
+      double* R = wsrec + (size_t)i * BM_REC;
+      R[BM_GAT + e] = gat; R[BM_GBT + e] = gbt; R[BM_DINV + e] = dinv;
+      if (c == 0) R[BM_W + r] = w;
+    }
+    Dl[(size_t)(a >> 1) * 16 + e] = da_new;
+    El[(size_t)(a >> 1) * 16 + e] = e_new;
+    if (c == 0) xs[a * B + r] = ya_new;
+  }
+}
+
 template <typename Src>
 __device__ __attribute__((always_inline)) void bcr_mfma_solve(Src A, const double* rhs, int M, double* ws, double* lds, double* Sband, double* x,
                                                               double* logdet, int* info, int rhs_stride = 1, double* stamps = nullptr,
-                                                              BmSplit sp = BmSplit{}) {
+                                                              BmSplit sp = BmSplit{}, int first_level = 0, const double* pre = nullptr) {
   constexpr int B = BM_B;
   const int tid = threadIdx.x;
   const int lane = tid & 63, wv = __builtin_amdgcn_readfirstlane(tid >> 6);
@@ -146,20 +228,42 @@
     const double v = bm_src_load(A, B + rr - cc, pad ? 0 : col, (long)M, 0);
     return pad ? 0.0 : v;
   };
-  if ((nb & 1) && tid < 16 && !(split && sp.half == 0)) {
-    const int rr = tid >> 2, cc = tid & 3;
-    Dl[(size_t)((nb - 1) >> 1) * 16 + tid] = bandD(nb - 1, rr > cc ? rr : cc, rr > cc ? cc : rr);
-  }
-  if (split && sp.half == 0 && tid < 16) Dl[(size_t)(ht >> 1) * 16 + tid] = 0.0;
-  for (int row = tid; row < nb * B; row += BM_THREADS) {
-    const bool sep_left = split && sp.half == 0 && row >= ht * B && row < (ht + 1) * B;
-    xs[row] = (row < M && !sep_left) ? rhs[(long)row * rhs_stride] : 0.0;
+  if (first_level > 0) {
+    const int nsurv = (nb + 7) >> 3;
+    for (int idx = tid; idx < nsurv * BMW_SURV; idx += BM_THREADS) {
+      const int j = idx / BMW_SURV, k2 = idx - j * BMW_SURV, n = j * 8, w2 = j >> 2;
+      const bool is_e = k2 >= 16 && k2 < 32;
+      const bool two = (j & 3) == 0 && w2 > 0 && !is_e;
+      const double vr = pre[(size_t)w2 * BMW_WG + (j & 3) * BMW_SURV + k2];
+      const double vl = pre[(size_t)(two ? w2 - 1 : 0) * BMW_WG + BMW_LEFT + (k2 < 16 ? k2 : (is_e ? 0 : k2 - 16))];
+      const bool sep = split && n == ht;
+      const double v = two ? ((sep && sp.half == 0) ? vl : ((sep && sp.half == 1) ? vr : vr + vl)) : vr;
+      if (k2 < 16) Dl[(size_t)(n >> 1) * 16 + k2] = v;
+      else if (is_e) El[(size_t)(n >> 1) * 16 + k2 - 16] = v;
+      else xs[n * B + k2 - 32] = v;
+    }
+    for (int row = tid; row < nb * B; row += BM_THREADS)
+      if ((row >> 2) & 7) xs[row] = 0.0;
+    if (tid >= BM_THREADS - 64 && lane < (nb + BMW_BLOCKS - 1) / BMW_BLOCKS) {
+      red[50 + lane] = pre[(size_t)lane * BMW_WG + BMW_LOGDET];
+      red[66 + lane] = pre[(size_t)lane * BMW_WG + BMW_BAD];
+    }
+  } else {
+    if ((nb & 1) && tid < 16 && !(split && sp.half == 0)) {
+      const int rr = tid >> 2, cc = tid & 3;
+      Dl[(size_t)((nb - 1) >> 1) * 16 + tid] = bandD(nb - 1, rr > cc ? rr : cc, rr > cc ? cc : rr);
+    }
+    if (split && sp.half == 0 && tid < 16) Dl[(size_t)(ht >> 1) * 16 + tid] = 0.0;
+    for (int row = tid; row < nb * B; row += BM_THREADS) {
+      const bool sep_left = split && sp.half == 0 && row >= ht * B && row < (ht + 1) * B;
+      xs[row] = (row < M && !sep_left) ? rhs[(long)row * rhs_stride] : 0.0;
+    }
   }
   __syncthreads();
   stamp();
 
   constexpr int RMAXR = 4;
-  for (int l = 0; l < levels; ++l) {
+  for (int l = first_level; l < levels; ++l) {
     const int h = 1 << l;
     const int ne = (nb > h) ? (nb - h + 2 * h - 1) / (2 * h) : 0;
     int m0, ne_h;
@@ -227,74 +331,7 @@
       const bool act = ml < ne_h;
       const int i = h + (m0 + (act ? ml : ne_h - 1)) * 2 * h, a = i - h, b = i + h;
       const bool hasb = b < nb;
-      const int bsafe = hasb ? b : a;
-      double d[10];
-      double ea, eb, da;
-      if (l == 0) {
-#pragma unroll
-        for (int t3 = 0; t3 < 3; ++t3) if (e + 16 * t3 < 40) slab[e + 16 * t3] = sl[rd & 1][t3];
-        int kk = 0;
-#pragma unroll
-        for (int rr = 0; rr < 4; ++rr)
-#pragma unroll
-          for (int cc = 0; cc <= rr; ++cc) d[kk++] = slab[(rr - cc) * 8 + 4 + cc];
-        ea = slab[(4 + lo - hi) * 8 + hi];
-        ea = (r <= c) ? ea : 0.0;
-        eb = slab[(4 + lo - hi) * 8 + 4 + hi];
-        eb = (hasb && c <= r) ? eb : 0.0;
-        da = slab[(hi - lo) * 8 + lo];
-      } else {
-        const double* Di = Dl + (size_t)(i >> 1) * 16;
-        int kk = 0;
-#pragma unroll
-        for (int rr = 0; rr < 4; ++rr)
-#pragma unroll
-          for (int cc = 0; cc <= rr; ++cc) d[kk++] = Di[rr * 4 + cc];
-        ea = El[(size_t)(a >> 1) * 16 + e];
-        eb = El[(size_t)(i >> 1) * 16 + et];
-        eb = hasb ? eb : 0.0;
-        da = Dl[(size_t)(a >> 1) * 16 + e];
-      }
-      double yv = xs[i * B + r], ya = xs[a * B + r];
-      yv = (c == 0) ? yv : 0.0;
-      ya = (c == 0) ? ya : 0.0;
-      (void)bsafe;
-      double dprod;
-      int badj;
-      const double t = bm_chol_linv(d, hi, lo, dprod, badj);
-      if (act && badj && !bad) bad = i * B + badj;
-      const double linv = (r >= c) ? t : 0.0;
-      const double linvT = (c >= r) ? t : 0.0;
-      if (act) ld.mul(dprod);
-      const double ua = bm_mfma(linvT, ea, 0.0);
-      const double ub = bm_mfma(linvT, eb, 0.0);
-      const double zz = bm_mfma(linvT, yv, 0.0);
-      const double nua = -ua, nub = -ub;
-      const double da_new = bm_mfma(nua, ua, da);
-      const double e_new = bm_mfma(nub, ua, 0.0);
-      const double ya_new = bm_mfma(nua, zz, ya);
-      updb[rd] = bm_mfma(ub, ub, 0.0);
-      ybu[rd] = bm_mfma(ub, zz, 0.0);
-      updb[rd] = act ? updb[rd] : 0.0;
-      ybu[rd] = act ? ybu[rd] : 0.0;
-      const double gat = bm_mfma(ua, linv, 0.0);
-      const double gbt = bm_mfma(ub, linv, 0.0);
-      const double dinv = bm_mfma(linv, linv, 0.0);
-      const double w = bm_mfma(linv, zz, 0.0);
-      if (act) {
-        if (l >= 3) {
-          double* R = Fl + (size_t)(i >> 3) * 52;
-          R[e] = gat; R[16 + e] = gbt; R[32 + e] = dinv;
-          if (c == 0) R[48 + r] = w;
-        } else {
-          double* R = rec(i);
-          R[BM_GAT + e] = gat; R[BM_GBT + e] = gbt; R[BM_DINV + e] = dinv;
-          if (c == 0) R[BM_W + r] = w;
-        }
-        Dl[(size_t)(a >> 1) * 16 + e] = da_new;
-        El[(size_t)(a >> 1) * 16 + e] = e_new;
-        if (c == 0) xs[a * B + r] = ya_new;
-      }
+      bm_forward_node(l, i, a, 0, act, hasb, BmLane{r, q, c, e, et, hi, lo}, Dl, El, xs, slab, sl[rd & 1], Fl, ws, bad, ld, updb[rd], ybu[rd]);
     }
     bcr_lds_barrier();
 #pragma unroll
@@ -471,6 +508,8 @@
       for (int w2 = 0; w2 < BM_THREADS / 64; ++w2) { s += red[w2]; bmin = sbad[w2] < bmin ? sbad[w2] : bmin; }
       s += s_other;
       bmin = bad_other < bmin ? bad_other : bmin;
+      if (first_level > 0)
+        for (int w2 = 0; w2 < (nb + BMW_BLOCKS - 1) / BMW_BLOCKS; ++w2) { s += red[50 + w2]; bmin = (int)red[66 + w2] < bmin ? (int)red[66 + w2] : bmin; }
       __hip_atomic_store(logdet + 0, 2.0 * s, __ATOMIC_RELAXED, __HIP_MEMORY_SCOPE_AGENT);
       __hip_atomic_store(logdet + 1, 0.0, __ATOMIC_RELAXED, __HIP_MEMORY_SCOPE_AGENT);
       __hip_atomic_store(info, (bmin == 0x7fffffff) ? 0 : bmin, __ATOMIC_RELAXED, __HIP_MEMORY_SCOPE_AGENT);
@@ -479,6 +518,105 @@
   stamp();
 }
 
+
+template <typename Src>
+__device__ __attribute__((always_inline)) void bcr_mfma_wide(Src A, const double* rhs, int M, int w, double* ws, double* pre, double* lds, int rhs_stride = 1,
+                                                             double* stamps = nullptr) {
+  constexpr int B = BM_B;
+  const int tid = threadIdx.x;
+  const int lane = tid & 63, wv = __builtin_amdgcn_readfirstlane(tid >> 6);
+  const int r = lane >> 4, q = (lane >> 2) & 3, c = lane & 3;
+  const int e = r * 4 + c, et = c * 4 + r;
+  const int hi = r > c ? r : c, lo = r > c ? c : r;
+  const int nb = (M + B - 1) / B;
+  const int base = w * BMW_BLOCKS;
+  constexpr int NSLOT = BMW_BLOCKS / 2 + 1;
+  double* Dl = lds;
+  double* El = Dl + NSLOT * 16;
+  double* xs = El + NSLOT * 16;
+  double* slab = xs + (BMW_BLOCKS + 1) * B + (size_t)(wv * 4 + q) * 40;
+  double* red = xs + (BMW_BLOCKS + 1) * B + (size_t)(BMW_THREADS / 64) * 4 * 40;
+  unsigned long long t_prev = stamps ? __builtin_amdgcn_s_memtime() : 0ull;
+  int nst = 0;
+  auto stamp = [&]() {
+    if (stamps && tid == 0) { const unsigned long long t = __builtin_amdgcn_s_memtime(); stamps[nst++] = (double)(t - t_prev); t_prev = t; }
+  };
+  for (int k2 = tid; k2 < 2 * NSLOT * 16; k2 += BMW_THREADS) Dl[k2] = 0.0;
+  if (tid < (BMW_BLOCKS + 1) * B) {
+    const long row = (long)base * B + tid;
+    xs[tid] = (tid < BMW_BLOCKS * B && row < M) ? rhs[(row < M ? row : 0) * rhs_stride] : 0.0;
+  }
+  __syncthreads();
+  if ((nb & 1) && nb - 1 >= base && nb - 1 < base + BMW_BLOCKS && tid < 16) {
+    const int rr = tid >> 2, cc = tid & 3, rh = rr > cc ? rr : cc, cl = rr > cc ? cc : rr;
+    const int col = (nb - 1) * B + cl, row = (nb - 1) * B + rh;
+    const bool pad = row >= M;
+    const double v = bm_src_load(A, rh - cl, pad ? 0 : col, (long)M, 0);
+    Dl[(size_t)((nb - 1 - base) >> 1) * 16 + tid] = pad ? ((rh == cl) ? 1.0 : 0.0) : v;
+  }
+  __syncthreads();
+  stamp();
+  int bad = 0;
+  BmLog ld{1.0, 0};
+  for (int l = 0; l < BMW_LEVELS; ++l) {
+    const int h = 1 << l;
+    const int ne = (nb > h) ? (nb - h + 2 * h - 1) / (2 * h) : 0;
+    const int per = (BMW_BLOCKS / 2) >> l, m0 = w * per;
+    const int ne_h = ne - m0 < per ? (ne - m0 > 0 ? ne - m0 : 0) : per;
+    double updb = 0.0, ybu = 0.0;
+    const bool work = wv * 4 < ne_h;
+    const int ml = wv * 4 + q;
+    const bool act = ml < ne_h;
+    const int i = h + (act ? ml : ne_h - 1) * 2 * h, a = i - h, b = i + h;
+    const bool hasb = base + b < nb;
+    if (work) {
+      double sl[3] = {0.0, 0.0, 0.0};
+      if (l == 0) {
+#pragma unroll
+        for (int t3 = 0; t3 < 3; ++t3) {
+          const int kk = e + 16 * t3, dd = kk >> 3, col = (base + a) * B + (kk & 7);
+          const bool in = kk < 40 && col + dd < M;
+          const double v = bm_src_load(A, in ? dd : 0, in ? col : 0, (long)M, 0);
+          sl[t3] = in ? v : ((dd == 0) ? 1.0 : 0.0);
+        }
+      }
+      bm_forward_node(l, i, a, base, act, hasb, BmLane{r, q, c, e, et, hi, lo}, Dl, El, xs, slab, sl, nullptr, ws + (size_t)base * BM_REC, bad, ld, updb, ybu);
+    }
+    bcr_lds_barrier();
+    if (work && act && hasb) {
+      Dl[(size_t)(b >> 1) * 16 + e] -= updb;
+      if (c == 0) xs[b * B + r] -= ybu;
+    }
+    bcr_lds_barrier();
+    stamp();
+  }
+  double* out = pre + (size_t)w * BMW_WG;
+  if (tid < BMW_LEFT) {
+    const int j = tid / BMW_SURV, k2 = tid - j * BMW_SURV, n = j * 8;
+    out[tid] = k2 < 16 ? Dl[(size_t)(n >> 1) * 16 + k2] : (k2 < 32 ? El[(size_t)(n >> 1) * 16 + k2 - 16] : xs[n * B + k2 - 32]);
+  } else if (tid < BMW_LEFT + 20) {
+    const int k2 = tid - BMW_LEFT;
+    out[tid] = k2 < 16 ? Dl[(size_t)(BMW_BLOCKS >> 1) * 16 + k2] : xs[BMW_BLOCKS * B + k2 - 16];
+  }
+  {
+    const double mine = (r == 0 && c == 0) ? (log(ld.m) + (double)ld.e * 0.6931471805599453094) : 0.0;
+    const double tot = wave_sum_dpp(mine);
+    int bm = bad ? bad : 0x7fffffff;
+#pragma unroll
+    for (int off = 32; off > 0; off >>= 1) { const int o = __shfl_xor(bm, off, 64); bm = o < bm ? o : bm; }
+    int* sbad = reinterpret_cast<int*>(red + 8);
+    if (lane == 0) { red[wv] = tot; sbad[wv] = bm; }
+    __syncthreads();
+    if (tid == 0) {
+      double s = 0.0;
+      int bmin = 0x7fffffff;
+      for (int w2 = 0; w2 < BMW_THREADS / 64; ++w2) { s += red[w2]; bmin = sbad[w2] < bmin ? sbad[w2] : bmin; }
+      out[BMW_LOGDET] = s;
+      out[BMW_BAD] = (double)bmin;
+    }
+  }
+  stamp();
+}
 
 __host__ __device__ inline size_t bcr_mfma_pre_ws_doubles(long nb) { return (size_t)nb * 96 + 64; }
 __host__ __device__ inline size_t bcr_mfma_pre_lds_doubles(long nb, int n_rec) {
diff --git a/asvgp_amd/csrc/elbo.hip b/asvgp_amd/csrc/elbo.hip
--- a/asvgp_amd/csrc/elbo.hip
+++ b/asvgp_amd/csrc/elbo.hip
@@ -13,7 +13,7 @@
 
 
 struct Ws {
-  double *Kuu, *dK, *P, *LK, *dLK, *LP, *SK, *dSK, *SP, *c, *alpha, *logdets, *fin, *bcrK, *bcrP;
+  double *Kuu, *dK, *P, *LK, *dLK, *LP, *SK, *dSK, *SP, *c, *alpha, *logdets, *fin, *bcrK, *bcrP, *pre;
 };
 static size_t bcr_ws_chain(int planes, int k, bool big) {
   long ns = 1024;
@@ -27,7 +27,7 @@
   return (a > c ? a : c) + 64;
 }
 static size_t bcr_ws_P(int k) { size_t a = bcr_ws_chain(1, k, false), b = bcr_ws_chain(1, k, true); return (a > b ? a : b) + 64; }
-static size_t bcr_ws_total(long M, int k) { return bcr_ws_K(k, M) + bcr_ws_P(k); }
+static size_t bcr_ws_total(long M, int k) { return bcr_ws_K(k, M) + bcr_ws_P(k) + bcr_mfma_wide_ws_doubles(); }
 static size_t ws_doubles(long M, int k, long D) {
   return (size_t)9 * (k + 1) * M + (size_t)2 * M * D + 64 + 32 + bcr_ws_total(M, k);
 }
@@ -41,7 +41,8 @@
   w.logdets = p; p += 64;
   w.fin = p; p += 32;
   w.bcrK = p; p += bcr_ws_K(k, M);
-  w.bcrP = p;
+  w.bcrP = p; p += bcr_ws_P(k);
+  w.pre = p;
   return w;
 }
 
@@ -76,6 +77,7 @@
   bool fused_fin;
   bool ahead_req, gpu_fwd, fwd_worker, defer_forward;
   bool no_split, plan_first;
+  bool no_presplit;
 };
 struct ChainPlan {
   int status; char msg[160];
@@ -87,6 +89,8 @@
   int grid, n_helpers, split;
   int fwd;
   bool scale_alpha, scale_c;
+  bool presplit; int pre_grid, pre_threads; size_t pre_lds_bytes;
+  int first_level;
 };
 
 template <int K, bool TANGENT>
@@ -146,6 +150,13 @@
     p.grid = 2 + p.split;
     p.fwd = in.ahead_req ? FWD_AHEAD : in.gpu_fwd ? FWD_GPU : in.plan_first ? FWD_HOST_BEFORE : in.fwd_worker ? FWD_WORKER
           : in.defer_forward ? FWD_DEFERRED : FWD_HOST_INLINE;
+    if (p.split && p.fwd != FWD_AHEAD && !in.no_presplit) {
+      p.presplit = true;
+      p.pre_grid = (int)((nb + BMW_BLOCKS - 1) / BMW_BLOCKS);
+      p.pre_threads = BMW_THREADS;
+      p.pre_lds_bytes = sizeof(double) * bcr_mfma_wide_lds_doubles();
+      p.first_level = BMW_LEVELS;
+    }
     return p;
   }
   if (in.ahead_req) return refuse(ASVGP_ERR_UNSUPPORTED, ahead_only);
@@ -444,6 +455,7 @@
   long D; int n_helpers; int finalize; int debug_no_assembly; int debug_stamps;
   double* mirror; unsigned long long mirror_seq;
   int split; double* xchg;
+  int first_level; const double* pre;
 };
 constexpr int FIN_GACC_PR = 21;
 __device__ __forceinline__ void assemble_band_slice(const double* __restrict__ S, const double* __restrict__ coef, const double* __restrict__ dcoef, int n_terms,
@@ -516,6 +528,30 @@
   __builtin_amdgcn_fence(__ATOMIC_ACQUIRE, "agent");
   elbo_finalize_body<K>((int)blockIdx.x - 2, fin.n_helpers, lds, fin.stats, Kuu, dK, nullptr, nullptr, SK, dSK, SP, nullptr, x, logdets, (long)M, fin.D,
                         fin.th, fin.alpha_scale, fin.gacc, fin.ticket, fin.arrived, fin.out);
+}
+
+template <int K>
+__global__ __launch_bounds__(BMW_THREADS) void p_chain_wide_kernel(KuuInterior ki, const double* A, const double* b, int M, double s, double* wsP, double* pre,
+                                                                   double* logdets, int debug_stamps) {
+  extern __shared__ double lds[];
+  static_assert(K == BM_B, "matrix-core chains: bandwidth 4");
+  static_assert(2 * PRIOR_BND_DIAGS * PRIOR_BND <= BMW_THREADS, "one boundary-table entry per thread");
+  const unsigned long long t_start = debug_stamps ? __builtin_amdgcn_s_memrealtime() : 0ull;
+  __shared__ double kdl[8];
+  __shared__ double bnd[2 * PRIOR_BND_DIAGS * PRIOR_BND];
+  if (threadIdx.x < 5) kdl[threadIdx.x] = ki.k[threadIdx.x];
+  {
+    const double* bnd_g = reinterpret_cast<const double*>((const char*)__builtin_amdgcn_kernarg_segment_ptr() + offsetof(KuuInterior, bnd));
+    if (threadIdx.x < 2 * PRIOR_BND_DIAGS * PRIOR_BND) bnd[threadIdx.x] = bnd_g[threadIdx.x];
+  }
+  __syncthreads();
+  bcr_mfma_wide<BandSumToep>(BandSumToep{A, 1.0 / s, (lds_cdouble_ptr)kdl, (lds_cdouble_ptr)bnd, ki.lo, ki.hi}, b, M, (int)blockIdx.x, wsP, pre, lds, 1,
+                             (debug_stamps && blockIdx.x == 0) ? pre + BMW_BAD + 1 : (double*)nullptr);
+  if (debug_stamps && threadIdx.x == 0 && (blockIdx.x == 0 || blockIdx.x == gridDim.x - 1)) {
+    const int o = blockIdx.x == 0 ? 20 : 22;
+    logdets[o] = (double)(t_start & 0xffffffffull);
+    logdets[o + 1] = (double)((__builtin_amdgcn_s_memrealtime() - t_start) & 0xffffffffull);
+  }
 }
 
 template <int K>
@@ -587,7 +623,8 @@
     BmSplit bsp;
     if (fin.split) { bsp.half = isPR ? 1 : 0; bsp.xchg = fin.xchg; bsp.spin_limit = spin_limit; bsp.gave_up = &gave_up; bsp.tag = seq << 8; }
     bcr_mfma_solve<BandSumToep>(BandSumToep{A, 1.0 / s_v, (lds_cdouble_ptr)kdl, (lds_cdouble_ptr)bnd, ki.lo, ki.hi}, b, M, wsP, lds, SP, x, logdets + 2, info + 1, 1,
-                                fin.debug_stamps ? (isPR ? fin.xchg + 128 : logdets + 32) : (double*)nullptr, bsp);
+                                fin.debug_stamps ? (isPR ? fin.xchg + 128 : logdets + 32) : (double*)nullptr, bsp,
+                                fin.first_level, fin.pre);
     rstamp(3);
     __syncthreads();
     if (gave_up) { if (threadIdx.x == 0) atomicExch(info + 1, -1); return; }
@@ -828,6 +865,8 @@
   ff.assembled = reinterpret_cast<unsigned*>(c.w.fin + 20);
   ff.debug_no_assembly = debug_env().no_assembly;
   ff.debug_stamps = debug_env().chain_stamps;
+  ff.first_level = p.first_level;
+  ff.pre = p.presplit ? c.w.pre : nullptr;
   return ff;
 }
 static void interior_dkuu(const PriorPlan* plan, const double* dc, double* dk, double* dkb) {
@@ -902,6 +941,9 @@
     set_pending_forward(h, c.cf, slot);
     handle_post_forward(h);
   }
+  if (p.presplit)
+    hipLaunchKernelGGL(p_chain_wide_kernel<K>, dim3(p.pre_grid), dim3(p.pre_threads), p.pre_lds_bytes, c.st, ki, c.A, c.b, (int)c.M, c.s, w.bcrP, w.pre,
+                       w.logdets, ff.debug_stamps);
   hipLaunchKernelGGL(kern, dim3(p.grid), dim3(BM_THREADS), p.lds_bytes, c.st, ki, c.S, c.cf, w.Kuu, w.dK, c.A, c.b, (int)c.M, w.bcrP, w.SP, w.alpha,
                      w.logdets, c.info, c.s, tab_k, n_rec, h->node_rec_dev, w.bcrK, w.SK, w.dSK, h->done_dev + slot.slot, slot.seq, ready, spin_limit, ff,
                      box_k);
@@ -1041,7 +1083,7 @@
   const bool have_plan = h->plan && prior_plan_M(h->plan) == M && prior_plan_k(h->plan) == K && prior_plan_terms(h->plan) == c.cf.n;
   p = plan_chains<K, TANGENT>(ChainPlanIn{h->band_algo, have_plan, have_plan ? prior_plan_nrec(h->plan) : 0, have_plan && prior_plan_interior(h->plan),
                                           M, D, part, fin != nullptr, h->ahead_req, h->prior_forward_gpu, h->fwd_worker, h->defer_forward,
-                                          debug_env().no_split != 0, debug_env().plan_first != 0});
+                                          debug_env().no_split != 0, debug_env().plan_first != 0, debug_env().no_presplit != 0});
   if (p.status) { set_error("%s", p.msg); return p.status; }
   if (p.nothing) return ASVGP_OK;
   switch (p.path) {
@@ -1517,7 +1559,7 @@
     return ASVGP_ERR_BAD_ARG;
   }
   const ChainPlanIn in{band_algorithm, have_plan != 0, n_rec, interior != 0, (long)M, (long)D, part, fused_finalize != 0, ahead != 0,
-                       prior_forward_gpu != 0, forward_worker != 0, defer_forward != 0, no_split != 0, plan_first != 0};
+                       prior_forward_gpu != 0, forward_worker != 0, defer_forward != 0, no_split != 0, plan_first != 0, false};
   ChainPlan p{};
   p.status = ASVGP_ERR_UNSUPPORTED;
   snprintf(p.msg, sizeof(p.msg), "elbo_launch_plan_host: bandwidth %d outside 1..%d", k, (int)ASVGP_MAX_ORDER);
@@ -1531,4 +1573,26 @@
   return p.status;
 }
 
+extern "C" int asvgp_elbo_presplit_plan_host(int band_algorithm, int have_plan, int n_rec, int interior, int64_t M, int k, int64_t D, int part, int tangent,
+                                             int fused_finalize, int ahead, int prior_forward_gpu, int forward_worker, int defer_forward, int no_split,
+                                             int plan_first, int no_presplit, int64_t* plan5_host) {
+  if (!plan5_host || M < 1 || D < 1 || part < 0 || part > 2 || band_algorithm < 0 || band_algorithm > 4) {
+    set_error("elbo_presplit_plan_host: bad argument");
+    return ASVGP_ERR_BAD_ARG;
+  }
+  const ChainPlanIn in{band_algorithm, have_plan != 0, n_rec, interior != 0, (long)M, (long)D, part, fused_finalize != 0, ahead != 0,
+                       prior_forward_gpu != 0, forward_worker != 0, defer_forward != 0, no_split != 0, plan_first != 0, no_presplit != 0};
+  ChainPlan p{};
+  p.status = ASVGP_ERR_UNSUPPORTED;
+  snprintf(p.msg, sizeof(p.msg), "elbo_presplit_plan_host: bandwidth %d outside 1..%d", k, (int)ASVGP_MAX_ORDER);
+  (void)for_bandwidth(k, [&](auto kk) {
+    p = tangent ? plan_chains<decltype(kk)::value, true>(in) : plan_chains<decltype(kk)::value, false>(in);
+    return 0;
+  });
+  const int64_t f[5] = {p.presplit, p.pre_grid, p.pre_threads, (int64_t)p.pre_lds_bytes, p.first_level};
+  for (int i = 0; i < 5; ++i) plan5_host[i] = f[i];
+  if (p.status) set_error("%s", p.msg);
+  return p.status;
+}
+
 #endif
diff --git a/asvgp_amd/csrc/handle.hip b/asvgp_amd/csrc/handle.hip
--- a/asvgp_amd/csrc/handle.hip
+++ b/asvgp_amd/csrc/handle.hip
@@ -22,6 +22,7 @@
   g_dbg.plan_first = getenv("ASVGP_PLAN_FIRST") ? 1 : 0;
   g_dbg.bcr_stamps = getenv("ASVGP_BCR_STAMPS") ? atoi(getenv("ASVGP_BCR_STAMPS")) : 0;
   g_dbg.no_split = getenv("ASVGP_NO_SPLIT") ? atoi(getenv("ASVGP_NO_SPLIT")) : 0;
+  g_dbg.no_presplit = getenv("ASVGP_NO_PRESPLIT") ? atoi(getenv("ASVGP_NO_PRESPLIT")) : 0;
 }
 const DebugEnv& debug_env() {
   std::call_once(g_dbg_once, debug_env_load);
diff --git a/asvgp_amd/csrc/handle.hpp b/asvgp_amd/csrc/handle.hpp
--- a/asvgp_amd/csrc/handle.hpp
+++ b/asvgp_amd/csrc/handle.hpp
@@ -67,7 +67,7 @@
 };
 constexpr size_t BOX_BYTES = 4096;
 
-struct DebugEnv { int no_assembly; int chain_stamps; long spin_limit; int host_times; int plan_first; int bcr_stamps; int no_split; };
+struct DebugEnv { int no_assembly; int chain_stamps; long spin_limit; int host_times; int plan_first; int bcr_stamps; int no_split; int no_presplit; };
 const DebugEnv& debug_env();
 
 Handle* as_handle(asvgp_handle_t h);
diff --git a/asvgp_amd/csrc/phi_launch.hpp b/asvgp_amd/csrc/phi_launch.hpp
--- a/asvgp_amd/csrc/phi_launch.hpp
+++ b/asvgp_amd/csrc/phi_launch.hpp
@@ -1,4 +1,5 @@
 #pragma once
+#include <mutex>
 #include <type_traits>
 
 namespace asvgp {
@@ -33,10 +34,27 @@
   hipLaunchKernelGGL(phi_reduce_kernel, dim3((E1 + 255) / 256, phi_reduce_split(G)), dim3(256), 0, st, partials, G, ncols, K, cell0, M, D, dcol, do_band, stats, ranges);
 }
 
+static int phi_grant_lds(int device, const void* kern, size_t lds_bytes) {
+  struct Granted { const void* kern; int device; size_t bytes; };
+  static Granted tab[64];
+  static int n_tab = 0;
+  static std::mutex mu;
+  std::lock_guard<std::mutex> lk(mu);
+  Granted* g = nullptr;
+  for (int i = 0; i < n_tab && !g; ++i)
+    if (tab[i].kern == kern && tab[i].device == device) g = tab + i;
+  if (g && lds_bytes <= g->bytes) return ASVGP_OK;
+  hipError_t e = hipFuncSetAttribute(kern, hipFuncAttributeMaxDynamicSharedMemorySize, (int)lds_bytes);
+  if (e != hipSuccess) { set_error("hipFuncSetAttribute(%zu B LDS): %s", lds_bytes, hipGetErrorString(e)); return ASVGP_ERR_LDS_CAPACITY; }
+  if (!g && n_tab < 64) { g = tab + n_tab++; g->kern = kern; g->device = device; g->bytes = 0; }
+  if (g) g->bytes = lds_bytes;
+  return ASVGP_OK;
+}
+
 template <class Kern, class... Args>
 static int phi_launch(Handle* h, hipStream_t st, Kern kern, int G, int threads, size_t lds_bytes, Args... args) {
-  hipError_t e = hipFuncSetAttribute(reinterpret_cast<const void*>(kern), hipFuncAttributeMaxDynamicSharedMemorySize, (int)lds_bytes);
-  if (e != hipSuccess) { set_error("hipFuncSetAttribute(%zu B LDS): %s", lds_bytes, hipGetErrorString(e)); return ASVGP_ERR_LDS_CAPACITY; }
+  const int rcg = phi_grant_lds(h->device, reinterpret_cast<const void*>(kern), lds_bytes);
+  if (rcg) return rcg;
   const bool prof = h->prof_on && h->prof_n < PROF_RING && (h->prof_calls++ % h->prof_every == 0);
   if (prof) (void)hipEventRecord(h->prof_ev[h->prof_n][0], st);
   hipLaunchKernelGGL(kern, dim3((unsigned)G), dim3(threads), lds_bytes, st, args...);
diff --git a/include/asvgp_hip.h b/include/asvgp_hip.h
--- a/include/asvgp_hip.h
+++ b/include/asvgp_hip.h
@@ -116,6 +116,9 @@
 int asvgp_elbo_launch_plan_host(int band_algorithm, int have_plan, int n_rec, int interior, int64_t M, int k, int64_t D, int part, int tangent,
                                 int fused_finalize, int ahead, int prior_forward_gpu, int forward_worker, int defer_forward, int no_split,
                                 int plan_first, int64_t* plan12_host);
+int asvgp_elbo_presplit_plan_host(int band_algorithm, int have_plan, int n_rec, int interior, int64_t M, int k, int64_t D, int part, int tangent,
+                                  int fused_finalize, int ahead, int prior_forward_gpu, int forward_worker, int defer_forward, int no_split,
+                                  int plan_first, int no_presplit, int64_t* plan5_host);
 int asvgp_prior_forward_stamps(asvgp_handle_t handle, const double* coef_host, const double* dcoef_dl_host, uint64_t* out64, void* stream);
 int asvgp_elbo_grad_1d(asvgp_handle_t handle, const double* stats, const double* static_bands, int kind, double variance,
                        double lengthscale, double noise_variance, int64_t N, int64_t M, int k, int64_t D,
```

Result: slower. 131,300 (-5.7%).
